# skyepurchase/MeatModeler

Measured on AMD Instinct MI355X. Metric: descriptor-match pairs/sec + BA residuals/sec, 500×1080p frames, 1/2/4/8 GPU, higher is better.
Workload: dtype u8/int32 (match), f64 (BA); 1 GPU; 500 frames 1920x1080, 4000 ORB kpts/frame, BF Hamming 2-NN + ratio, track linking, 2-view DLT, full BA (TRF, Schur, f64 MFMA Cholesky); frames=500, height=1080, width=1920, nfeatures=4000, parallelism=pairs/points x1

## Files before the change

include/meatmodeler.h:

```cpp
#ifndef MEATMODELER_H
#define MEATMODELER_H

#include <stddef.h>
#include <stdint.h>

#ifdef __cplusplus
extern "C" {
#endif

#define MM_OK 0
#define MM_ERR_ARG (-1)
#define MM_ERR_HIP (-2)
#define MM_ERR_WORKSPACE (-3)
#define MM_ERR_NUMERIC (-4)

typedef struct mm_ctx mm_ctx;

int mm_abi_version(void);
int mm_ctx_create(int device, void *hip_stream, mm_ctx **out);
void mm_ctx_destroy(mm_ctx *ctx);
const char *mm_last_error(mm_ctx *ctx);
int mm_ctx_sync(mm_ctx *ctx);
#define MM_CTL_CHOL_FORCE_ABANDON 1
#define MM_CTL_CHOL_LAST_PATH 2
#define MM_CTL_CHOL_RESERVED 3
#define MM_CTL_CU_COUNT 4
#define MM_CTL_CHOL_AVOID_FUSED 5
#define MM_CTL_LINK_LAST_VARIANT 6
#define MM_CTL_BATCH_LAST 7
long long mm_ctx_control(mm_ctx *ctx, int what, long long value);
int mm_timer_create(mm_ctx *ctx, void **timer_out);
int mm_timer_start(mm_ctx *ctx, void *timer);
int mm_timer_stop(mm_ctx *ctx, void *timer);
int mm_timer_elapsed_ms(mm_ctx *ctx, void *timer, float *ms_out);
void mm_timer_destroy(mm_ctx *ctx, void *timer);
int mm_profile_enable(mm_ctx *ctx, int on);
int mm_profile_select(mm_ctx *ctx, const char *name);
int mm_profile_report(mm_ctx *ctx, char *buf, size_t buf_len);

size_t mm_bf_workspace_bytes(int n_pairs, int nq_cap, int nt_cap);
int mm_bf_knn2_batched(mm_ctx *ctx, const uint8_t *q , const int32_t *nq , int nq_cap,
                       size_t q_set_stride, const uint8_t *t , const int32_t *nt , int nt_cap,
                       size_t t_set_stride, int n_pairs, int32_t *idx , int32_t *dist ,
                       void *ws , size_t ws_bytes);
int mm_bf_knn2_hamming(mm_ctx *ctx, const uint8_t *q , int nq, const uint8_t *t , int nt,
                       int32_t *idx , int32_t *dist , void *ws, size_t ws_bytes);
int mm_ratio_filter_batched(mm_ctx *ctx, const int32_t *idx , const int32_t *dist ,
                            const int32_t *nq , int nq_cap, int n_pairs, double threshold,
                            int32_t *pairs , int32_t *m_out );

typedef struct mm_orb_params {
    int32_t nfeatures;
    int32_t nlevels;
    int32_t edge_threshold;
    int32_t fast_threshold;
    float scale_factor;
    int32_t reserved;
} mm_orb_params;
size_t mm_orb_workspace_bytes(int batch, int height, int width, const mm_orb_params *prm);
int mm_orb_detect_compute(mm_ctx *ctx, const uint8_t *imgs , int batch, int height, int width, int stride,
                          const mm_orb_params *prm, const int8_t *pattern , void *ws , size_t ws_bytes,
                          float *kp_xy, int32_t *kp_meta, float *kp_resp, int32_t *kp_mom, uint8_t *desc,
                          int32_t *n_out);
int mm_orb_level_sizes(int height, int width, const mm_orb_params *prm, int32_t *lvl_w ,
                       int32_t *lvl_h , int32_t *lvl_n ,
                       float *lvl_scale );

int64_t mm_link_tracks_clip(int n_frames, int cap, const int32_t *kp_count, const float *kp_xy, int mcap,
                            const int32_t *match_count, const int32_t *matches, int64_t max_tracks,
                            int64_t max_obs, int64_t *track_ptr , int32_t *obs_frame,
                            int32_t *obs_kp, int64_t *n_obs_out);
size_t mm_link_workspace_bytes(int n_frames, int cap);
int mm_link_tracks_device(mm_ctx *ctx, int n_frames, int cap, const int32_t *kp_count, const float *kp_xy,
                          const int32_t *match_count, const int32_t *matches, void *ws, size_t ws_bytes,
                          int32_t *track_ptr, int32_t *obs_frame, int32_t *obs_kp, int64_t *counts );
int mm_flatten_offsets(mm_ctx *ctx, const int32_t *track_ptr, const int32_t *sel, int64_t n_sel, int64_t *out_ptr);
int mm_flatten_tracks(mm_ctx *ctx, const int32_t *track_ptr, const int32_t *obs_frame, const int32_t *obs_kp, const float *kp_xy,
                      int cap, const int32_t *sel , int t_lo, int64_t n_sel, const int64_t *out_ptr , int64_t n_obs,
                      int frame_offset, double *coords, int32_t *frame_indices, int32_t *point_indices);
int64_t mm_ba_build_pairs(int F, int P, int64_t O, const int32_t *fi, const int32_t *pi, const int32_t *pt_ptr,
                          const int32_t *pt_obs, const int32_t *cam_ptr, const int32_t *cam_obs, int span,
                          int64_t *seg_ptr, int32_t *pair_o, int32_t *pair_o2, int64_t max_pairs);
int mm_ba_build_index(int F, int P, int64_t O, const int32_t *fi, const int32_t *pi, int32_t *pt_ptr ,
                      int32_t *pt_obs , int32_t *cam_ptr , int32_t *cam_obs );

#define MM_VERIFY_TOO_FEW 1
#define MM_VERIFY_NO_MODEL 2
#define MM_VERIFY_WEAK 4
#define MM_VERIFY_MALFORMED 8
typedef struct mm_verify_params {
    int32_t n_hyp, min_matches, min_inliers, refit_iters;
    uint32_t seed, pair_base;
    int32_t on_fail, reserved;
    double threshold_px;
} mm_verify_params;
size_t mm_verify_workspace_bytes(int n_pairs, int n_hyp);
int mm_verify_matches(mm_ctx *ctx, const float *kp_xy , const int32_t *pairs ,
                      const int32_t *m , int n_pairs, int cap, const mm_verify_params *prm,
                      int32_t *pairs_out , int32_t *m_out , double *Fm ,
                      double *cost , int32_t *info , void *ws, size_t ws_bytes);

int mm_triangulate_dlt(mm_ctx *ctx, const double *proj , const int32_t *f0 , const int32_t *f1 ,
                       const double *x0 , const double *x1 , int64_t n,
                       double *X );
#define MM_TRI_BEHIND 1
#define MM_TRI_REPROJ 2
#define MM_TRI_PARALLAX 4
#define MM_TRI_DEGENERATE 8
typedef struct mm_tri_params {
    int32_t refine_iters, reserved;
    double max_reproj_px, max_cos_parallax, min_depth;
} mm_tri_params;
size_t mm_triangulate_tracks_workspace_bytes(int F);
int mm_triangulate_tracks(mm_ctx *ctx, const double *proj , int F, const int32_t *track_ptr , int64_t T,
                          const int32_t *obs_frame , const double *obs_xy , const mm_tri_params *prm,
                          double *X , double *quality , int32_t *flags , void *ws, size_t ws_bytes);

typedef struct mm_ba_problem {
    int32_t F, P;
    int64_t O;
    const double *K;
    const int32_t *fi, *pi;
    const double *obs;
    const int32_t *pt_ptr, *pt_obs;
    const int32_t *cam_ptr, *cam_obs;
    int32_t cam_span;
    int32_t reserved;
    int64_t n_seg;
    const int32_t *seg_ids;
    const int32_t *seg_chunk_ptr;
    int64_t n_chunks;
    const int32_t *chunk_seg;
    const int32_t *chunk_begin, *chunk_end;
    const int32_t *pair_o, *pair_o2;
    const int32_t *pair_p;
} mm_ba_problem;

int mm_ba_residual(mm_ctx *ctx, const mm_ba_problem *pb, const double *cams ,
                   const double *pts , double *res , double *cost2 ,
                   void *ws, size_t ws_bytes);
int mm_ba_jacobian(mm_ctx *ctx, const mm_ba_problem *pb, const double *cams, const double *pts, double *Jc,
                   double *Jp);
int mm_ba_normal_eq(mm_ctx *ctx, const mm_ba_problem *pb, const double *cams, const double *pts, double *B,
                    double *gc, double *C, double *gp);
int mm_ba_jvp(mm_ctx *ctx, const mm_ba_problem *pb, const double *cams, const double *pts, const double *wc,
              const double *wp, double *out);
size_t mm_ba_jvp_dots_workspace_bytes(const mm_ba_problem *pb);
int mm_ba_jvp_dots(mm_ctx *ctx, const mm_ba_problem *pb, const double *cams, const double *pts, const double *wc,
                   const double *wp, double *out, const double *other , double *rows ,
                   void *ws, size_t ws_bytes);
int mm_ba_schur(mm_ctx *ctx, const mm_ba_problem *pb, const double *cams, const double *pts, const double *Bd,
                const double *Cd, const double *gc, const double *gp, double *S, double *v, double *Cinv, void *ws,
                size_t ws_bytes);
size_t mm_ba_schur_workspace_bytes(const mm_ba_problem *pb);
int mm_ba_pairs_count(mm_ctx *ctx, const mm_ba_problem *pb, int32_t *cnt , int32_t *span_out );
int mm_ba_pairs_emit(mm_ctx *ctx, const mm_ba_problem *pb, const int64_t *offsets , int span,
                     int32_t *key , int32_t *pair_o , int32_t *pair_o2 );
size_t mm_multi_dot_workspace_bytes(void);
int mm_multi_dot(mm_ctx *ctx, int k, const double *const *a, const double *const *b, int64_t n, int64_t split,
                 double *out, void *ws, size_t ws_bytes);
int mm_trf_fused(mm_ctx *ctx, int op, const double *const *in, double *const *outv, const double *const *scalars,
                 double h0, double h1, int64_t n, int64_t split, double *out, void *ws, size_t ws_bytes);
int mm_trf_damping(mm_ctx *ctx, const double *gh2, const double *d11, double Delta, double min_damping, double *out);
size_t mm_ba_backsub_workspace_bytes(const mm_ba_problem *pb);
int mm_ba_backsub(mm_ctx *ctx, const mm_ba_problem *pb, const double *cams, const double *pts, const double *Cinv,
                  const double *gp, const double *dc , double *dp, void *ws , size_t ws_bytes);
int mm_ba_schur_solve(mm_ctx *ctx, const mm_ba_problem *pb, const double *cams, const double *pts, const double *Bd,
                      const double *Cd, const double *gc, const double *gp, double *S, double *v, double *Cinv,
                      int half_bandwidth, int32_t *info, void *ws_schur, size_t ws_schur_bytes, void *ws_chol,
                      size_t ws_chol_bytes, int n_slabs, int cams_per_slab, const int64_t *slab_seg_ptr,
                      const int64_t *slab_chunk_ptr);
int mm_ba_scale_update(mm_ctx *ctx, int F, int P, const double *B, const double *C, double *scale_inv , int first);
int mm_ba_damp(mm_ctx *ctx, int F, int P, const double *B, const double *C, const double *scale_inv, const double *reg ,
               double *Bd, double *Cd);
int mm_trf_step2d(mm_ctx *ctx, const double *r0, const double *d11, const double *r1, const double *r2, const double *r3,
                  const double *bs, const double *reg, const int32_t *info, double Delta, double *board );
typedef struct mm_trf_params {
    double ftol, xtol, gtol;
    double min_damping;
    int64_t max_nfev;
} mm_trf_params;
typedef struct mm_trf_row {
    int32_t iteration, nfev;
    double cost, reduction, step_norm, optimality;
} mm_trf_row;
typedef struct mm_trf_report {
    double cost0, cost, optimality, min_damping ;
    int32_t nfev, njev, status, iterations, log_rows;
    int32_t chol_fallbacks;
    int32_t collectives;
    int32_t reserved;
} mm_trf_report;
size_t mm_ba_trf_workspace_bytes(const mm_ba_problem *pb);
int mm_ba_trf(mm_ctx *ctx, const mm_ba_problem *pb, double *cams , double *pts ,
              const mm_trf_params *prm, mm_trf_report *report , mm_trf_row *log , int log_cap,
              void *ws , size_t ws_bytes);
typedef int (*mm_allreduce_fn)(void *user, double *buf , int64_t count);
typedef struct mm_dist {
    int32_t rank, world;
    int32_t half_bandwidth, band_exchange;
    mm_allreduce_fn allreduce;
    void *user;
} mm_dist;
size_t mm_ba_trf_dist_workspace_bytes(const mm_ba_problem *pb, int half_bandwidth);
int mm_ba_trf_dist(mm_ctx *ctx, const mm_ba_problem *pb, double *cams, double *pts, const mm_trf_params *prm,
                   mm_trf_report *report, mm_trf_row *log, int log_cap, void *ws, size_t ws_bytes, const mm_dist *dist);
size_t mm_ba_trf_batched_workspace_bytes(const mm_ba_problem *pb);
int mm_ba_trf_batched(mm_ctx *ctx, int n_prob, const mm_ba_problem *const *pbs, double *const *cams ,
                      double *const *pts , const mm_trf_params *prm, mm_trf_report *reports ,
                      void *const *ws , const size_t *ws_bytes, int32_t *solved_alone );
typedef struct mm_ba_fixed {
    int32_t F_fixed;
    int32_t reserved;
    const double *cams;
} mm_ba_fixed;
int mm_ba_residual_fixed(mm_ctx *ctx, const mm_ba_problem *pb, const mm_ba_fixed *fx, const double *cams ,
                         const double *pts , double *res , double *cost2 , void *ws,
                         size_t ws_bytes);
int mm_ba_normal_eq_fixed(mm_ctx *ctx, const mm_ba_problem *pb, const mm_ba_fixed *fx, const double *cams, const double *pts,
                          double *B, double *gc, double *C, double *gp);
size_t mm_ba_trf_fixed_workspace_bytes(const mm_ba_problem *pb, const mm_ba_fixed *fx);
int mm_ba_trf_fixed(mm_ctx *ctx, const mm_ba_problem *pb, const mm_ba_fixed *fx, double *cams ,
                    double *pts , const mm_trf_params *prm, mm_trf_report *report ,
                    mm_trf_row *log , int log_cap, void *ws , size_t ws_bytes);
size_t mm_chol_workspace_bytes(int n);
int mm_chol_solve_sym(mm_ctx *ctx, double *A , int n, double *b , int half_bandwidth, int both_triangles,
                      int32_t *info , void *ws, size_t ws_bytes);
int mm_chol_solve(mm_ctx *ctx, double *A , int n, double *b , int nrhs, int half_bandwidth,
                  int32_t *info , void *ws, size_t ws_bytes);

int mm_pyr_down(mm_ctx *ctx, const uint8_t *src , int w, int h, int src_pitch, uint8_t *dst , int dst_pitch);
int mm_lk_track(mm_ctx *ctx, const uint8_t *const *prev_levels, const uint8_t *const *next_levels, const int *w, const int *h,
                const int *pitch, int levels, const float *pts, int n, int win_w, int win_h, int max_count,
                double epsilon_sq, float *next_pts, uint8_t *status, float *err);
int mm_min_eig(mm_ctx *ctx, const uint8_t *img , int w, int h, int pitch, int block_size, double *eig );
int mm_corner_candidates(mm_ctx *ctx, const double *eig, int w, int h, double quality, unsigned long long *max_bits ,
                         long long *val_bits , int32_t *pos , int cap, int32_t *count );
int mm_gftt_select(const int32_t *pos , int64_t n, int w, int h, int max_corners, double min_distance,
                   float *out , int cap);
size_t mm_contrast_workspace_bytes(int batch, int w, int h, int tiles_x, int tiles_y);
int mm_increase_contrast(mm_ctx *ctx, const uint8_t *bgr, int batch, int w, int h, const uint16_t *gamma,
                         const uint16_t *cbrt_tab, const uint8_t *gamma_inv, double clip_limit, int tiles_x, int tiles_y,
                         uint8_t *out, uint8_t *grey , void *ws, size_t ws_bytes);
int mm_bgr_to_grey(mm_ctx *ctx, const uint8_t *bgr , size_t n_pixels, uint8_t *grey );
int mm_write_ply(const char *path, const double *xyz , int64_t n);

#ifdef __cplusplus
}
#endif
#endif
```

meatmodeler_amd/_lib.py:

```python
import ctypes as C
import os

_HERE = os.path.dirname(os.path.abspath(__file__))
LIB_PATH = os.path.join(_HERE, "libmeatmodeler_hip.so")

c_i32p = C.POINTER(C.c_int32)
c_i64p = C.POINTER(C.c_int64)
c_f32p = C.POINTER(C.c_float)
c_f64p = C.POINTER(C.c_double)
c_u8p = C.POINTER(C.c_uint8)
c_i8p = C.POINTER(C.c_int8)
vp = C.c_void_p


class MMError(RuntimeError):
    pass


class OrbParams(C.Structure):
    _fields_ = [("nfeatures", C.c_int32), ("nlevels", C.c_int32), ("edge_threshold", C.c_int32),
                ("fast_threshold", C.c_int32), ("scale_factor", C.c_float), ("reserved", C.c_int32)]


class BAProblem(C.Structure):
    _fields_ = [("F", C.c_int32), ("P", C.c_int32), ("O", C.c_int64), ("K", vp), ("fi", vp), ("pi", vp),
                ("obs", vp), ("pt_ptr", vp), ("pt_obs", vp), ("cam_ptr", vp), ("cam_obs", vp),
                ("cam_span", C.c_int32), ("reserved", C.c_int32), ("n_seg", C.c_int64), ("seg_ids", vp),
                ("seg_chunk_ptr", vp), ("n_chunks", C.c_int64), ("chunk_seg", vp), ("chunk_begin", vp),
                ("chunk_end", vp), ("pair_o", vp), ("pair_o2", vp), ("pair_p", vp)]


class BAFixed(C.Structure):
    _fields_ = [("F_fixed", C.c_int32), ("reserved", C.c_int32), ("cams", vp)]


class TrfParams(C.Structure):
    _fields_ = [("ftol", C.c_double), ("xtol", C.c_double), ("gtol", C.c_double), ("min_damping", C.c_double),
                ("max_nfev", C.c_int64)]


class TrfRow(C.Structure):
    _fields_ = [("iteration", C.c_int32), ("nfev", C.c_int32), ("cost", C.c_double), ("reduction", C.c_double),
                ("step_norm", C.c_double), ("optimality", C.c_double)]


class TriParams(C.Structure):
    _fields_ = [("refine_iters", C.c_int32), ("reserved", C.c_int32), ("max_reproj_px", C.c_double),
                ("max_cos_parallax", C.c_double), ("min_depth", C.c_double)]


class VerifyParams(C.Structure):
    _fields_ = [("n_hyp", C.c_int32), ("min_matches", C.c_int32), ("min_inliers", C.c_int32), ("refit_iters", C.c_int32),
                ("seed", C.c_uint32), ("pair_base", C.c_uint32), ("on_fail", C.c_int32), ("reserved", C.c_int32),
                ("threshold_px", C.c_double)]


ALLREDUCE_FN = C.CFUNCTYPE(C.c_int, vp, vp, C.c_int64)


class Dist(C.Structure):
    _fields_ = [("rank", C.c_int32), ("world", C.c_int32), ("half_bandwidth", C.c_int32), ("band_exchange", C.c_int32),
                ("allreduce", ALLREDUCE_FN), ("user", vp)]


class TrfReport(C.Structure):
    _fields_ = [("cost0", C.c_double), ("cost", C.c_double), ("optimality", C.c_double), ("min_damping", C.c_double),
                ("nfev", C.c_int32), ("njev", C.c_int32), ("status", C.c_int32), ("iterations", C.c_int32),
                ("log_rows", C.c_int32), ("chol_fallbacks", C.c_int32), ("collectives", C.c_int32), ("reserved", C.c_int32)]


SIGNATURES = {
    "mm_abi_version": (C.c_int, []),
    "mm_ctx_create": (C.c_int, [C.c_int, vp, C.POINTER(vp)]),
    "mm_ctx_destroy": (None, [vp]),
    "mm_ctx_control": (C.c_longlong, [vp, C.c_int, C.c_longlong]),
    "mm_last_error": (C.c_char_p, [vp]),
    "mm_ctx_sync": (C.c_int, [vp]),
    "mm_timer_create": (C.c_int, [vp, C.POINTER(vp)]),
    "mm_timer_start": (C.c_int, [vp, vp]),
    "mm_timer_stop": (C.c_int, [vp, vp]),
    "mm_timer_elapsed_ms": (C.c_int, [vp, vp, C.POINTER(C.c_float)]),
    "mm_timer_destroy": (None, [vp, vp]),
    "mm_profile_enable": (C.c_int, [vp, C.c_int]),
    "mm_profile_report": (C.c_int, [vp, C.c_char_p, C.c_size_t]),
    "mm_profile_select": (C.c_int, [vp, C.c_char_p]),
    "mm_bf_workspace_bytes": (C.c_size_t, [C.c_int, C.c_int, C.c_int]),
    "mm_bf_knn2_batched": (C.c_int, [vp, vp, vp, C.c_int, C.c_size_t, vp, vp, C.c_int, C.c_size_t, C.c_int, vp, vp,
                                     vp, C.c_size_t]),
    "mm_bf_knn2_hamming": (C.c_int, [vp, vp, C.c_int, vp, C.c_int, vp, vp, vp, C.c_size_t]),
    "mm_ratio_filter_batched": (C.c_int, [vp, vp, vp, vp, C.c_int, C.c_int, C.c_double, vp, vp]),
    "mm_orb_workspace_bytes": (C.c_size_t, [C.c_int, C.c_int, C.c_int, C.POINTER(OrbParams)]),
    "mm_orb_detect_compute": (C.c_int, [vp, vp, C.c_int, C.c_int, C.c_int, C.c_int, C.POINTER(OrbParams), vp, vp,
                                        C.c_size_t, vp, vp, vp, vp, vp, vp]),
    "mm_orb_level_sizes": (C.c_int, [C.c_int, C.c_int, C.POINTER(OrbParams), c_i32p, c_i32p, c_i32p, c_f32p]),
    "mm_link_tracks_clip": (C.c_int64, [C.c_int, C.c_int, c_i32p, c_f32p, C.c_int, c_i32p, c_i32p, C.c_int64,
                                        C.c_int64, c_i64p, c_i32p, c_i32p, c_i64p]),
    "mm_link_workspace_bytes": (C.c_size_t, [C.c_int, C.c_int]),
    "mm_link_tracks_device": (C.c_int, [vp, C.c_int, C.c_int, vp, vp, vp, vp, vp, C.c_size_t, vp, vp, vp, vp]),
    "mm_flatten_offsets": (C.c_int, [vp, vp, vp, C.c_int64, vp]),
    "mm_flatten_tracks": (C.c_int, [vp, vp, vp, vp, vp, C.c_int, vp, C.c_int, C.c_int64, vp, C.c_int64, C.c_int, vp, vp, vp]),
    "mm_ba_build_pairs": (C.c_int64, [C.c_int, C.c_int, C.c_int64, c_i32p, c_i32p, c_i32p, c_i32p, c_i32p, c_i32p, C.c_int,
                                      c_i64p, c_i32p, c_i32p, C.c_int64]),
    "mm_ba_build_index": (C.c_int, [C.c_int, C.c_int, C.c_int64, c_i32p, c_i32p, c_i32p, c_i32p, c_i32p, c_i32p]),
    "mm_verify_workspace_bytes": (C.c_size_t, [C.c_int, C.c_int]),
    "mm_verify_matches": (C.c_int, [vp, vp, vp, vp, C.c_int, C.c_int, C.POINTER(VerifyParams), vp, vp, vp, vp, vp, vp, C.c_size_t]),
    "mm_triangulate_dlt": (C.c_int, [vp, vp, vp, vp, vp, vp, C.c_int64, vp]),
    "mm_triangulate_tracks_workspace_bytes": (C.c_size_t, [C.c_int]),
    "mm_triangulate_tracks": (C.c_int, [vp, vp, C.c_int, vp, C.c_int64, vp, vp, C.POINTER(TriParams), vp, vp, vp, vp, C.c_size_t]),
    "mm_ba_residual": (C.c_int, [vp, C.POINTER(BAProblem), vp, vp, vp, vp, vp, C.c_size_t]),
    "mm_ba_jacobian": (C.c_int, [vp, C.POINTER(BAProblem), vp, vp, vp, vp]),
    "mm_ba_normal_eq": (C.c_int, [vp, C.POINTER(BAProblem), vp, vp, vp, vp, vp, vp]),
    "mm_ba_jvp": (C.c_int, [vp, C.POINTER(BAProblem), vp, vp, vp, vp, vp]),
    "mm_ba_schur": (C.c_int, [vp, C.POINTER(BAProblem), vp, vp, vp, vp, vp, vp, vp, vp, vp, vp, C.c_size_t]),
    "mm_ba_schur_workspace_bytes": (C.c_size_t, [C.POINTER(BAProblem)]),
    "mm_ba_pairs_count": (C.c_int, [vp, C.POINTER(BAProblem), vp, vp]),
    "mm_ba_pairs_emit": (C.c_int, [vp, C.POINTER(BAProblem), vp, C.c_int, vp, vp, vp]),
    "mm_ba_schur_solve": (C.c_int, [vp, C.POINTER(BAProblem), vp, vp, vp, vp, vp, vp, vp, vp, vp, C.c_int, vp, vp,
                                    C.c_size_t, vp, C.c_size_t, C.c_int, C.c_int, c_i64p, c_i64p]),
    "mm_multi_dot_workspace_bytes": (C.c_size_t, []),
    "mm_multi_dot": (C.c_int, [vp, C.c_int, C.POINTER(vp), C.POINTER(vp), C.c_int64, C.c_int64, vp, vp, C.c_size_t]),
    "mm_trf_fused": (C.c_int, [vp, C.c_int, C.POINTER(vp), C.POINTER(vp), C.POINTER(vp), C.c_double, C.c_double, C.c_int64,
                               C.c_int64, vp, vp, C.c_size_t]),
    "mm_trf_damping": (C.c_int, [vp, vp, vp, C.c_double, C.c_double, vp]),
    "mm_ba_backsub": (C.c_int, [vp, C.POINTER(BAProblem), vp, vp, vp, vp, vp, vp, vp, C.c_size_t]),
    "mm_ba_backsub_workspace_bytes": (C.c_size_t, [C.POINTER(BAProblem)]),
    "mm_chol_workspace_bytes": (C.c_size_t, [C.c_int]),
    "mm_chol_solve": (C.c_int, [vp, vp, C.c_int, vp, C.c_int, C.c_int, vp, vp, C.c_size_t]),
    "mm_ba_jvp_dots_workspace_bytes": (C.c_size_t, [C.POINTER(BAProblem)]),
    "mm_ba_jvp_dots": (C.c_int, [vp, C.POINTER(BAProblem), vp, vp, vp, vp, vp, vp, vp, vp, C.c_size_t]),
    "mm_ba_scale_update": (C.c_int, [vp, C.c_int, C.c_int, vp, vp, vp, C.c_int]),
    "mm_ba_damp": (C.c_int, [vp, C.c_int, C.c_int, vp, vp, vp, vp, vp, vp]),
    "mm_trf_step2d": (C.c_int, [vp, vp, vp, vp, vp, vp, vp, vp, vp, C.c_double, vp]),
    "mm_pyr_down": (C.c_int, [vp, vp, C.c_int, C.c_int, C.c_int, vp, C.c_int]),
    "mm_lk_track": (C.c_int, [vp, vp, vp, vp, vp, vp, C.c_int, vp, C.c_int, C.c_int, C.c_int, C.c_int, C.c_double, vp, vp, vp]),
    "mm_min_eig": (C.c_int, [vp, vp, C.c_int, C.c_int, C.c_int, C.c_int, vp]),
    "mm_corner_candidates": (C.c_int, [vp, vp, C.c_int, C.c_int, C.c_double, vp, vp, vp, C.c_int, vp]),
    "mm_gftt_select": (C.c_int, [vp, C.c_int64, C.c_int, C.c_int, C.c_int, C.c_double, vp, C.c_int]),
    "mm_contrast_workspace_bytes": (C.c_size_t, [C.c_int, C.c_int, C.c_int, C.c_int, C.c_int]),
    "mm_increase_contrast": (C.c_int, [vp, vp, C.c_int, C.c_int, C.c_int, vp, vp, vp, C.c_double, C.c_int, C.c_int, vp, vp, vp,
                                       C.c_size_t]),
    "mm_bgr_to_grey": (C.c_int, [vp, vp, C.c_size_t, vp]),
    "mm_write_ply": (C.c_int, [C.c_char_p, vp, C.c_int64]),
    "mm_chol_solve_sym": (C.c_int, [vp, vp, C.c_int, vp, C.c_int, C.c_int, vp, vp, C.c_size_t]),
    "mm_ba_trf_workspace_bytes": (C.c_size_t, [C.POINTER(BAProblem)]),
    "mm_ba_trf": (C.c_int, [vp, C.POINTER(BAProblem), vp, vp, C.POINTER(TrfParams), C.POINTER(TrfReport),
                            C.POINTER(TrfRow), C.c_int, vp, C.c_size_t]),
    "mm_ba_trf_batched_workspace_bytes": (C.c_size_t, [C.POINTER(BAProblem)]),
    "mm_ba_trf_batched": (C.c_int, [vp, C.c_int, C.POINTER(C.POINTER(BAProblem)), C.POINTER(vp), C.POINTER(vp),
                                    C.POINTER(TrfParams), C.POINTER(TrfReport), C.POINTER(vp), C.POINTER(C.c_size_t), c_i32p]),
    "mm_ba_residual_fixed": (C.c_int, [vp, C.POINTER(BAProblem), C.POINTER(BAFixed), vp, vp, vp, vp, vp, C.c_size_t]),
    "mm_ba_normal_eq_fixed": (C.c_int, [vp, C.POINTER(BAProblem), C.POINTER(BAFixed), vp, vp, vp, vp, vp, vp]),
    "mm_ba_trf_fixed_workspace_bytes": (C.c_size_t, [C.POINTER(BAProblem), C.POINTER(BAFixed)]),
    "mm_ba_trf_fixed": (C.c_int, [vp, C.POINTER(BAProblem), C.POINTER(BAFixed), vp, vp, C.POINTER(TrfParams),
                                  C.POINTER(TrfReport), C.POINTER(TrfRow), C.c_int, vp, C.c_size_t]),
    "mm_ba_trf_dist_workspace_bytes": (C.c_size_t, [C.POINTER(BAProblem), C.c_int]),
    "mm_ba_trf_dist": (C.c_int, [vp, C.POINTER(BAProblem), vp, vp, C.POINTER(TrfParams), C.POINTER(TrfReport),
                                 C.POINTER(TrfRow), C.c_int, vp, C.c_size_t, C.POINTER(Dist)]),
}


def _load():
    if not os.path.exists(LIB_PATH):
        raise ImportError(
            f"{LIB_PATH} is missing: the HIP extension has not been built "
            "(make -C meatmodeler_amd/csrc).  meatmodeler_amd has no CPU fallback.")
    lib = C.CDLL(LIB_PATH)
    for name, (res, args) in SIGNATURES.items():
        fn = getattr(lib, name)
        fn.restype = res
        fn.argtypes = args
    return lib


lib = _load()


def ptr(t):
    if t is None:
        return None
    if hasattr(t, "data_ptr"):
        return t.data_ptr()
    return t.ctypes.data


class Context:

    def __init__(self, device=None, stream=None):
        import torch
        if not torch.cuda.is_available():
            raise MMError("meatmodeler_amd needs an AMD GPU (torch.cuda.is_available() is False); "
                          "there is no CPU path")
        if device is None:
            device = torch.cuda.current_device()
        self.device = torch.device("cuda", device if isinstance(device, int) else device.index or 0)
        self.stream = stream if stream is not None else torch.cuda.current_stream(self.device)
        h = vp()
        rc = lib.mm_ctx_create(self.device.index, vp(self.stream.cuda_stream), C.byref(h))
        if rc != 0:
            raise MMError(f"mm_ctx_create failed ({rc})")
        self.h = h

    def check(self, rc, what=""):
        if rc != 0:
            msg = lib.mm_last_error(self.h)
            raise MMError(f"{what} failed ({rc}): {msg.decode() if msg else ''}")

    def sync(self):
        self.check(lib.mm_ctx_sync(self.h), "mm_ctx_sync")

    CTL_CHOL_FORCE_ABANDON, CTL_CHOL_LAST_PATH, CTL_CHOL_RESERVED, CTL_CU_COUNT, CTL_CHOL_AVOID_FUSED = 1, 2, 3, 4, 5
    CTL_LINK_LAST_VARIANT = 6
    CTL_BATCH_LAST = 7

    def control(self, what, value=0):
        r = int(lib.mm_ctx_control(self.h, int(what), int(value)))
        if r < -1 or (r == -1 and what not in (self.CTL_CHOL_LAST_PATH, self.CTL_LINK_LAST_VARIANT, self.CTL_BATCH_LAST)):
            self.check(r, "mm_ctx_control")
        return r

    def profile(self, level, only=None):
        if only is not None:
            self.check(lib.mm_profile_select(self.h, only.encode()), "mm_profile_select")
        self.check(lib.mm_profile_enable(self.h, int(level)), "mm_profile_enable")

    def profile_report(self):
        buf = C.create_string_buffer(1 << 16)
        n = lib.mm_profile_report(self.h, buf, len(buf))
        if n < 0:
            self.check(n, "mm_profile_report")
        out = {}
        for line in buf.value.decode().splitlines():
            name, cnt, ms = line.split()
            out[name] = (int(cnt), float(ms))
        return out

    def __del__(self):
        try:
            if getattr(self, "h", None):
                lib.mm_ctx_destroy(self.h)
                self.h = None
        except Exception:
            pass


class Timer:

    def __init__(self, ctx):
        self.ctx = ctx
        self.t = vp()
        ctx.check(lib.mm_timer_create(ctx.h, C.byref(self.t)), "mm_timer_create")

    def start(self):
        self.ctx.check(lib.mm_timer_start(self.ctx.h, self.t), "mm_timer_start")

    def stop(self):
        self.ctx.check(lib.mm_timer_stop(self.ctx.h, self.t), "mm_timer_stop")

    def elapsed_ms(self):
        ms = C.c_float()
        self.ctx.check(lib.mm_timer_elapsed_ms(self.ctx.h, self.t, C.byref(ms)), "mm_timer_elapsed_ms")
        return ms.value

    def __del__(self):
        try:
            lib.mm_timer_destroy(self.ctx.h, self.t)
        except Exception:
            pass


_default_ctx = {}


def default_context():
    import torch
    key = (torch.cuda.current_device(), torch.cuda.current_stream().cuda_stream)
    c = _default_ctx.get(key)
    if c is None:
        c = _default_ctx[key] = Context()
    return c
```

meatmodeler_amd/csrc/bf_match.hip:

```cpp
#include "mm_common.h"
#include <cstdlib>
#include <type_traits>

namespace {

constexpr int BF_THREADS = 256;
constexpr uint32_t BF_NONE = 0xFFFFFFFFu;
constexpr int BF_IDX_BITS = 20;

__device__ __forceinline__ uint32_t bcnt_acc(uint32_t x, uint32_t acc) {
    uint32_t r;
    asm("v_bcnt_u32_b32 %0, %1, %2" : "=v"(r) : "v"(x), "v"(acc));
    return r;
}

__device__ __forceinline__ uint32_t ham256(const uint32_t (&a)[8], const uint4 &t0, const uint4 &t1) {
    uint32_t d = bcnt_acc(a[0] ^ t0.x, 0u);
    d = bcnt_acc(a[1] ^ t0.y, d);
    d = bcnt_acc(a[2] ^ t0.z, d);
    d = bcnt_acc(a[3] ^ t0.w, d);
    d = bcnt_acc(a[4] ^ t1.x, d);
    d = bcnt_acc(a[5] ^ t1.y, d);
    d = bcnt_acc(a[6] ^ t1.z, d);
    d = bcnt_acc(a[7] ^ t1.w, d);
    return d;
}

__device__ __forceinline__ void top2_insert(uint32_t key, uint32_t &b0, uint32_t &b1) {
    uint32_t hi = max(b0, key);
    b0 = min(b0, key);
    b1 = min(b1, hi);
}

template <int BF_QPL, int BF_UNROLL>
__global__ __launch_bounds__(BF_THREADS) void bf_knn2_kernel(
    const uint8_t *__restrict__ q, const int32_t *__restrict__ nq_dev, int nq_cap, size_t q_stride,
    const uint8_t *__restrict__ t, const int32_t *__restrict__ nt_dev, int nt_cap, size_t t_stride, int n_splits,
    uint32_t *__restrict__ part, int32_t *__restrict__ idx, int32_t *__restrict__ dist) {
    const int pair = blockIdx.z;
    const int split = blockIdx.y;
    int nq = nq_dev ? min(nq_dev[pair], nq_cap) : nq_cap;
    int nt = nt_dev ? min(nt_dev[pair], nt_cap) : nt_cap;
    constexpr int BF_QTILE = BF_THREADS * BF_QPL;
    const int qbase = blockIdx.x * BF_QTILE;
    if (qbase >= nq) return;

    uint32_t qa[BF_QPL][8];
    const uint8_t *qp = q + (size_t)pair * q_stride;
#pragma unroll
    for (int u = 0; u < BF_QPL; ++u) {
        int qi = qbase + u * BF_THREADS + threadIdx.x;
        uint4 lo = make_uint4(0, 0, 0, 0), hi = lo;
        if (qi < nq) {
            const uint4 *p = reinterpret_cast<const uint4 *>(qp + (size_t)qi * 32);
            lo = p[0];
            hi = p[1];
        }
        qa[u][0] = lo.x; qa[u][1] = lo.y; qa[u][2] = lo.z; qa[u][3] = lo.w;
        qa[u][4] = hi.x; qa[u][5] = hi.y; qa[u][6] = hi.z; qa[u][7] = hi.w;
    }

    int chunk = (nt + n_splits - 1) / n_splits;
    chunk = (chunk + BF_UNROLL - 1) / BF_UNROLL * BF_UNROLL;
    const int j0 = split * chunk;
    const int j1 = min(nt, j0 + chunk);

    uint32_t b0[BF_QPL], b1[BF_QPL];
#pragma unroll
    for (int u = 0; u < BF_QPL; ++u) b0[u] = b1[u] = BF_NONE;

    const uint4 *__restrict__ tp = reinterpret_cast<const uint4 *>(t + (size_t)pair * t_stride);
    int j = j0;
    for (; j + BF_UNROLL <= j1; j += BF_UNROLL) {
        uint4 tv[2 * BF_UNROLL];
#pragma unroll
        for (int k = 0; k < 2 * BF_UNROLL; ++k) tv[k] = tp[2 * j + k];
#pragma unroll
        for (int k = 0; k < BF_UNROLL; ++k) {
#pragma unroll
            for (int u = 0; u < BF_QPL; ++u) {
                uint32_t d = ham256(qa[u], tv[2 * k], tv[2 * k + 1]);
                top2_insert((d << BF_IDX_BITS) | (uint32_t)(j + k), b0[u], b1[u]);
            }
        }
    }
    for (; j < j1; ++j) {
        uint4 t0 = tp[2 * j], t1 = tp[2 * j + 1];
#pragma unroll
        for (int u = 0; u < BF_QPL; ++u) {
            uint32_t d = ham256(qa[u], t0, t1);
            top2_insert((d << BF_IDX_BITS) | (uint32_t)j, b0[u], b1[u]);
        }
    }

#pragma unroll
    for (int u = 0; u < BF_QPL; ++u) {
        int qi = qbase + u * BF_THREADS + threadIdx.x;
        if (qi >= nq) continue;
        if (n_splits == 1) {
            size_t o = ((size_t)pair * nq_cap + qi) * 2;
            idx[o] = b0[u] == BF_NONE ? -1 : (int32_t)(b0[u] & ((1u << BF_IDX_BITS) - 1));
            idx[o + 1] = b1[u] == BF_NONE ? -1 : (int32_t)(b1[u] & ((1u << BF_IDX_BITS) - 1));
            dist[o] = b0[u] == BF_NONE ? -1 : (int32_t)(b0[u] >> BF_IDX_BITS);
            dist[o + 1] = b1[u] == BF_NONE ? -1 : (int32_t)(b1[u] >> BF_IDX_BITS);
        } else {
            size_t o = (((size_t)pair * n_splits + split) * nq_cap + qi) * 2;
            part[o] = b0[u];
            part[o + 1] = b1[u];
        }
    }
}

constexpr int BF_TCHUNK = 128;

__device__ __forceinline__ void top2_insert_med3(uint32_t key, uint32_t &b0, uint32_t &b1) {
    uint32_t m;
    asm("v_med3_u32 %0, %1, %2, %3" : "=v"(m) : "v"(b0), "v"(b1), "v"(key));
    b0 = min(b0, key);
    b1 = m;
}

template <int BF_QPL, int TCH = BF_TCHUNK>
__global__ __launch_bounds__(BF_THREADS) void bf_knn2_lds_kernel(
    const uint8_t *__restrict__ q, const int32_t *__restrict__ nq_dev, int nq_cap, size_t q_stride,
    const uint8_t *__restrict__ t, const int32_t *__restrict__ nt_dev, int nt_cap, size_t t_stride, int n_splits,
    uint32_t *__restrict__ part, int32_t *__restrict__ idx, int32_t *__restrict__ dist) {
    constexpr int NST = TCH / 128;
    __shared__ uint4 tl[2][TCH * 2];
    const int pair = blockIdx.z;
    const int split = blockIdx.y;
    int nq = nq_dev ? min(nq_dev[pair], nq_cap) : nq_cap;
    int nt = nt_dev ? min(nt_dev[pair], nt_cap) : nt_cap;
    constexpr int BF_QTILE = BF_THREADS * BF_QPL;
    const int qbase = blockIdx.x * BF_QTILE;
    if (qbase >= nq) return;

    uint32_t qa[BF_QPL][8];
    const uint8_t *qp = q + (size_t)pair * q_stride;
#pragma unroll
    for (int u = 0; u < BF_QPL; ++u) {
        int qi = qbase + u * BF_THREADS + threadIdx.x;
        uint4 lo = make_uint4(0, 0, 0, 0), hi = lo;
        if (qi < nq) {
            const uint4 *p = reinterpret_cast<const uint4 *>(qp + (size_t)qi * 32);
            lo = p[0];
            hi = p[1];
        }
        qa[u][0] = lo.x; qa[u][1] = lo.y; qa[u][2] = lo.z; qa[u][3] = lo.w;
        qa[u][4] = hi.x; qa[u][5] = hi.y; qa[u][6] = hi.z; qa[u][7] = hi.w;
    }
    int chunk = (nt + n_splits - 1) / n_splits;
    chunk = (chunk + 3) & ~3;
    const int j0 = split * chunk;
    const int j1 = min(nt, j0 + chunk);
    uint32_t b0[BF_QPL], b1[BF_QPL];
#pragma unroll
    for (int u = 0; u < BF_QPL; ++u) b0[u] = b1[u] = BF_NONE;

    const uint4 *__restrict__ tp = reinterpret_cast<const uint4 *>(t + (size_t)pair * t_stride);
    uint4 stage[NST];
#pragma unroll
    for (int z = 0; z < NST; ++z) {
        const int e = 2 * j0 + z * BF_THREADS + (int)threadIdx.x;
        stage[z] = e < 2 * j1 ? tp[e] : make_uint4(0, 0, 0, 0);
        tl[0][z * BF_THREADS + threadIdx.x] = stage[z];
    }
    __syncthreads();
    int buf = 0;
    for (int c0 = j0; c0 < j1; c0 += TCH) {
        const int cn = min(TCH, j1 - c0);
        const int nxt = c0 + TCH;
        if (nxt < j1) {
#pragma unroll
            for (int z = 0; z < NST; ++z) {
                const int e = 2 * nxt + z * BF_THREADS + (int)threadIdx.x;
                stage[z] = e < 2 * j1 ? tp[e] : make_uint4(0, 0, 0, 0);
            }
        }
        const uint4 *tb = tl[buf];
        int k = 0;
        for (; k + 4 <= cn; k += 4) {
            uint4 tv[8];
#pragma unroll
            for (int r = 0; r < 8; ++r) tv[r] = tb[2 * k + r];
            uint32_t d[4][BF_QPL];
            bool hit = false;
#pragma unroll
            for (int u = 0; u < BF_QPL; ++u) {
#pragma unroll
                for (int r = 0; r < 4; ++r) d[r][u] = ham256(qa[u], tv[2 * r], tv[2 * r + 1]);
                const uint32_t m = min(min(d[0][u], d[1][u]), min(d[2][u], d[3][u]));
                hit |= m < (b1[u] >> BF_IDX_BITS);
            }
            if (__builtin_amdgcn_ballot_w64(hit) != 0) {
#pragma unroll
                for (int r = 0; r < 4; ++r) {
#pragma unroll
                    for (int u = 0; u < BF_QPL; ++u)
                        top2_insert_med3((d[r][u] << BF_IDX_BITS) | (uint32_t)(c0 + k + r), b0[u], b1[u]);
                }
            }
        }
        for (; k < cn; ++k) {
            const uint4 t0 = tb[2 * k], t1 = tb[2 * k + 1];
#pragma unroll
            for (int u = 0; u < BF_QPL; ++u) {
                uint32_t d = ham256(qa[u], t0, t1);
                top2_insert_med3((d << BF_IDX_BITS) | (uint32_t)(c0 + k), b0[u], b1[u]);
            }
        }
        if (nxt < j1) {
#pragma unroll
            for (int z = 0; z < NST; ++z) tl[buf ^ 1][z * BF_THREADS + threadIdx.x] = stage[z];
            __syncthreads();
            buf ^= 1;
        }
    }
#pragma unroll
    for (int u = 0; u < BF_QPL; ++u) {
        int qi = qbase + u * BF_THREADS + threadIdx.x;
        if (qi >= nq) continue;
        if (n_splits == 1) {
            size_t o = ((size_t)pair * nq_cap + qi) * 2;
            idx[o] = b0[u] == BF_NONE ? -1 : (int32_t)(b0[u] & ((1u << BF_IDX_BITS) - 1));
            idx[o + 1] = b1[u] == BF_NONE ? -1 : (int32_t)(b1[u] & ((1u << BF_IDX_BITS) - 1));
            dist[o] = b0[u] == BF_NONE ? -1 : (int32_t)(b0[u] >> BF_IDX_BITS);
            dist[o + 1] = b1[u] == BF_NONE ? -1 : (int32_t)(b1[u] >> BF_IDX_BITS);
        } else {
            size_t o = (((size_t)pair * n_splits + split) * nq_cap + qi) * 2;
            part[o] = b0[u];
            part[o + 1] = b1[u];
        }
    }
}

__global__ __launch_bounds__(256) void bf_merge_kernel(const uint32_t *__restrict__ part,
                                                       const int32_t *__restrict__ nq_dev, int nq_cap, int n_splits,
                                                       int32_t *__restrict__ idx, int32_t *__restrict__ dist) {
    const int pair = blockIdx.y;
    const int qi = blockIdx.x * blockDim.x + threadIdx.x;
    int nq = nq_dev ? min(nq_dev[pair], nq_cap) : nq_cap;
    if (qi >= nq) return;
    uint32_t b0 = BF_NONE, b1 = BF_NONE;
    for (int s = 0; s < n_splits; ++s) {
        size_t o = (((size_t)pair * n_splits + s) * nq_cap + qi) * 2;
        top2_insert(part[o], b0, b1);
        top2_insert(part[o + 1], b0, b1);
    }
    size_t o = ((size_t)pair * nq_cap + qi) * 2;
    idx[o] = b0 == BF_NONE ? -1 : (int32_t)(b0 & ((1u << BF_IDX_BITS) - 1));
    idx[o + 1] = b1 == BF_NONE ? -1 : (int32_t)(b1 & ((1u << BF_IDX_BITS) - 1));
    dist[o] = b0 == BF_NONE ? -1 : (int32_t)(b0 >> BF_IDX_BITS);
    dist[o + 1] = b1 == BF_NONE ? -1 : (int32_t)(b1 >> BF_IDX_BITS);
}

__global__ __launch_bounds__(256) void ratio_filter_kernel(const int32_t *__restrict__ idx,
                                                           const int32_t *__restrict__ dist,
                                                           const int32_t *__restrict__ nq_dev, int nq_cap,
                                                           double threshold, int32_t *__restrict__ pairs,
                                                           int32_t *__restrict__ m_out) {
    __shared__ int wave_cnt[4];
    __shared__ int base_s;
    const int pair = blockIdx.x;
    int nq = nq_dev ? min(nq_dev[pair], nq_cap) : nq_cap;
    const int lane = threadIdx.x & 63, wave = threadIdx.x >> 6;
    if (threadIdx.x == 0) base_s = 0;
    __syncthreads();
    for (int q0 = 0; q0 < nq; q0 += 256) {
        int qi = q0 + threadIdx.x;
        bool keep = false;
        int ti = -1;
        if (qi < nq) {
            size_t o = ((size_t)pair * nq_cap + qi) * 2;
            int d0 = dist[o], d1 = dist[o + 1];
            ti = idx[o];
            keep = (d0 >= 0) && (d1 >= 0) && ((double)d0 < threshold * (double)d1);
        }
        unsigned long long m = __ballot(keep);
        int before = __builtin_popcountll(m & ((1ull << lane) - 1ull));
        if (lane == 0) wave_cnt[wave] = __builtin_popcountll(m);
        __syncthreads();
        int off = base_s;
        for (int w = 0; w < wave; ++w) off += wave_cnt[w];
        if (keep) {
            size_t o = ((size_t)pair * nq_cap + (off + before)) * 2;
            pairs[o] = qi;
            pairs[o + 1] = ti;
        }
        __syncthreads();
        if (threadIdx.x == 0) base_s += wave_cnt[0] + wave_cnt[1] + wave_cnt[2] + wave_cnt[3];
        __syncthreads();
    }
    if (threadIdx.x == 0) m_out[pair] = base_s;
}

typedef int bf_v4i __attribute__((ext_vector_type(4)));
typedef int bf_v16i __attribute__((ext_vector_type(16)));
constexpr int MF_TT = 32;
constexpr int MF_PITCH = 272;
constexpr int MF_SEG = 128;

__device__ __forceinline__ uint32_t bf_expand4(uint32_t nib) {
    const uint32_t x = (nib * 0x00204081u) & 0x01010101u;
    return ((x ^ 0x01010101u) * 0xFFu) | x;
}
__device__ __forceinline__ bf_v4i bf_expand16(uint32_t bits) {
    bf_v4i r;
    r[0] = (int)bf_expand4(bits & 15u);
    r[1] = (int)bf_expand4((bits >> 4) & 15u);
    r[2] = (int)bf_expand4((bits >> 8) & 15u);
    r[3] = (int)bf_expand4((bits >> 12) & 15u);
    return r;
}

__global__ __launch_bounds__(256) void bf_expand_kernel(const uint8_t *__restrict__ t, int nt_cap, size_t t_stride, int ntp,
                                                        int n_pairs, uint8_t *__restrict__ out) {
    const size_t g = (size_t)blockIdx.x * 256 + threadIdx.x;
    const size_t total = (size_t)n_pairs * ntp * 16;
    if (g >= total) return;
    const int chunk = (int)(g & 15);
    const size_t rowg = g >> 4;
    const int row = (int)(rowg % ntp), pair = (int)(rowg / ntp);
    uint32_t bits = 0;
    if (row < nt_cap) bits = reinterpret_cast<const uint16_t *>(t + (size_t)pair * t_stride + (size_t)row * 32)[chunk];
    reinterpret_cast<bf_v4i *>(out)[g] = bf_expand16(bits);
}

__device__ __forceinline__ uint32_t bf_pk_lo16(uint32_t hi_src, uint32_t lo_src) {
    return __builtin_amdgcn_perm(hi_src, lo_src, 0x05040100u);
}
typedef unsigned short bf_u16x2 __attribute__((ext_vector_type(2)));
__device__ __forceinline__ uint32_t bf_pk_mad(uint32_t a, uint32_t b, uint32_t c) {
    const bf_u16x2 r = __builtin_bit_cast(bf_u16x2, a) * __builtin_bit_cast(bf_u16x2, b) + __builtin_bit_cast(bf_u16x2, c);
    return __builtin_bit_cast(uint32_t, r);
}
__device__ __forceinline__ void bf_pk_top2(uint32_t key, uint32_t &b0, uint32_t &b1) {
    const bf_u16x2 k = __builtin_bit_cast(bf_u16x2, key), x0 = __builtin_bit_cast(bf_u16x2, b0), x1 = __builtin_bit_cast(bf_u16x2, b1);
    const bf_u16x2 hi = __builtin_elementwise_max(x0, k);
    b0 = __builtin_bit_cast(uint32_t, __builtin_elementwise_min(x0, k));
    b1 = __builtin_bit_cast(uint32_t, __builtin_elementwise_min(x1, hi));
}

__global__ __launch_bounds__(BF_THREADS) void bf_knn2_mfma_kernel(
    const uint8_t *__restrict__ q, const int32_t *__restrict__ nq_dev, int nq_cap, size_t q_stride,
    const uint8_t *__restrict__ tx, const int32_t *__restrict__ nt_dev, int nt_cap, int ntp,
    int32_t *__restrict__ idx, int32_t *__restrict__ dist) {
    __shared__ __attribute__((aligned(16))) uint8_t tile[2][MF_TT][MF_PITCH];
    const int pair = blockIdx.z;
    const int nq = nq_dev ? min(nq_dev[pair], nq_cap) : nq_cap;
    const int nt = nt_dev ? min(nt_dev[pair], nt_cap) : nt_cap;
    const int qbase = blockIdx.x * BF_THREADS;
    if (qbase >= nq) return;
    const int lane = threadIdx.x & 63, wv = threadIdx.x >> 6;
    const int c = lane & 31, h = lane >> 5;
    bf_v4i B[2][8];
    const uint8_t *qp = q + (size_t)pair * q_stride;
#pragma unroll
    for (int u = 0; u < 2; ++u) {
        const int qi = qbase + 64 * wv + 32 * u + c;
        uint4 lo = make_uint4(0, 0, 0, 0), hi = lo;
        if (qi < nq) {
            const uint4 *p = reinterpret_cast<const uint4 *>(qp + (size_t)qi * 32);
            lo = p[0];
            hi = p[1];
        }
        const uint32_t w[8] = {lo.x, lo.y, lo.z, lo.w, hi.x, hi.y, hi.z, hi.w};
#pragma unroll
        for (int j = 0; j < 8; ++j) B[u][j] = bf_expand16((w[j] >> (16 * h)) & 0xFFFFu);
    }
    uint32_t s0[2][8], s1[2][8];
#pragma unroll
    for (int u = 0; u < 2; ++u)
#pragma unroll
        for (int p = 0; p < 8; ++p) s0[u][p] = s1[u][p] = 0xFFFFFFFFu;
    uint32_t g0[2] = {BF_NONE, BF_NONE}, g1[2] = {BF_NONE, BF_NONE};
    const int ntiles = (nt + MF_TT - 1) / MF_TT;
    const uint8_t *txp = tx + (size_t)pair * ntp * 256;
    const int e0 = threadIdx.x, e1 = threadIdx.x + 256;
    bf_v4i a0, a1, b0_, b1_, c0_, c1_;
    auto fetch = [&](int tt, auto set) __attribute__((always_inline)) {
        constexpr int S = decltype(set)::value;
        if (tt < ntiles) {
            const bf_v4i *src = reinterpret_cast<const bf_v4i *>(txp + (size_t)tt * MF_TT * 256);
            const bf_v4i v0 = src[e0], v1 = src[e1];
            if constexpr (S == 0) { a0 = v0; a1 = v1; }
            if constexpr (S == 1) { b0_ = v0; b1_ = v1; }
            if constexpr (S == 2) { c0_ = v0; c1_ = v1; }
        }
    };
    auto commit = [&](int buf, auto set) __attribute__((always_inline)) {
        constexpr int S = decltype(set)::value;
        bf_v4i *d0 = reinterpret_cast<bf_v4i *>(&tile[buf][e0 >> 4][(e0 & 15) * 16]);
        bf_v4i *d1 = reinterpret_cast<bf_v4i *>(&tile[buf][e1 >> 4][(e1 & 15) * 16]);
        if constexpr (S == 0) { *d0 = a0; *d1 = a1; }
        if constexpr (S == 1) { *d0 = b0_; *d1 = b1_; }
        if constexpr (S == 2) { *d0 = c0_; *d1 = c1_; }
    };
    auto fold = [&](int seg) __attribute__((always_inline)) {
#pragma unroll
        for (int u = 0; u < 2; ++u)
#pragma unroll
            for (int p = 0; p < 8; ++p) {
                const int m = 8 * (p >> 1) + 4 * h + 2 * (p & 1);
#pragma unroll
                for (int x = 0; x < 2; ++x) {
#pragma unroll
                    for (int k = 0; k < 2; ++k) {
                        const uint32_t key16 = ((k == 0 ? s0[u][p] : s1[u][p]) >> (16 * x)) & 0xFFFFu;
                        if (key16 != 0xFFFFu) {
                            const uint32_t d = key16 >> 7, tno = key16 & 127u;
                            top2_insert((d << 16) | (uint32_t)((seg * MF_SEG + (int)tno) * MF_TT + m + x), g0[u], g1[u]);
                        }
                    }
                }
                s0[u][p] = s1[u][p] = 0xFFFFFFFFu;
            }
    };
    auto tile_step = [&](int tt, auto partial_tag) __attribute__((always_inline)) {
        constexpr bool PARTIAL = decltype(partial_tag)::value;
        const int buf = tt & 1;
        bf_v16i acc0 = {0, 0, 0, 0, 0, 0, 0, 0, 0, 0, 0, 0, 0, 0, 0, 0}, acc1 = acc0;
        bf_v4i A[8];
#pragma unroll
        for (int j = 0; j < 8; ++j) A[j] = *reinterpret_cast<const bf_v4i *>(&tile[buf][c][32 * j + 16 * h]);
        const uint32_t tno = (uint32_t)(tt & (MF_SEG - 1));
        const uint32_t base = (16384u + tno) * 0x00010001u;
        auto keys = [&](const bf_v16i &acc, int u, int p) __attribute__((always_inline)) {
            uint32_t k = bf_pk_mad(bf_pk_lo16((uint32_t)acc[2 * p + 1], (uint32_t)acc[2 * p]), 0xFFC0FFC0u, base);
            if constexpr (PARTIAL) {
                const int m = tt * MF_TT + 8 * (p >> 1) + 4 * h + 2 * (p & 1);
                k |= (m >= nt ? 0x0000FFFFu : 0u) | (m + 1 >= nt ? 0xFFFF0000u : 0u);
            }
            bf_pk_top2(k, s0[u][p], s1[u][p]);
        };
#pragma unroll
        for (int j = 0; j < 8; ++j) acc0 = __builtin_amdgcn_mfma_i32_32x32x32_i8(A[j], B[0][j], acc0, 0, 0, 0);
        __builtin_amdgcn_sched_barrier(0);
#pragma unroll
        for (int j = 0; j < 8; ++j) {
            acc1 = __builtin_amdgcn_mfma_i32_32x32x32_i8(A[j], B[1][j], acc1, 0, 0, 0);
            keys(acc0, 0, j);
            __builtin_amdgcn_sched_barrier(0);
        }
#pragma unroll
        for (int p = 0; p < 8; ++p) keys(acc1, 1, p);
    };
    using I0 = std::integral_constant<int, 0>;
    using I1 = std::integral_constant<int, 1>;
    using I2 = std::integral_constant<int, 2>;
    fetch(0, I0{});
    fetch(1, I1{});
    fetch(2, I2{});
    if (ntiles > 0) commit(0, I0{});
    fetch(3, I0{});
    __syncthreads();
    const int nfull = nt / MF_TT;
    auto iteration = [&](int tt, auto next_set) __attribute__((always_inline)) {
        tile_step(tt, std::false_type{});
        if ((tt & (MF_SEG - 1)) == MF_SEG - 1) fold(tt / MF_SEG);
        if (tt + 1 < ntiles) commit((tt & 1) ^ 1, next_set);
        fetch(tt + 4, next_set);
        __syncthreads();
    };
    int tt = 0;
    for (; tt + 3 <= nfull; tt += 3) {
        iteration(tt, I1{});
        iteration(tt + 1, I2{});
        iteration(tt + 2, I0{});
    }
    if (tt < nfull) {
        iteration(tt, I1{});
        if (tt + 1 < nfull) iteration(tt + 1, I2{});
    }
    if (nfull < ntiles) tile_step(nfull, std::true_type{});
    if (ntiles > 0) fold((ntiles - 1) / MF_SEG);
#pragma unroll
    for (int u = 0; u < 2; ++u) {
        const uint32_t o0 = __shfl_xor(g0[u], 32, 64), o1 = __shfl_xor(g1[u], 32, 64);
        top2_insert(o0, g0[u], g1[u]);
        top2_insert(o1, g0[u], g1[u]);
        const int qi = qbase + 64 * wv + 32 * u + c;
        if (h == 0 && qi < nq) {
            const size_t o = ((size_t)pair * nq_cap + qi) * 2;
            idx[o] = g0[u] == BF_NONE ? -1 : (int32_t)(g0[u] & 0xFFFFu);
            idx[o + 1] = g1[u] == BF_NONE ? -1 : (int32_t)(g1[u] & 0xFFFFu);
            dist[o] = g0[u] == BF_NONE ? -1 : (int32_t)(g0[u] >> 16);
            dist[o + 1] = g1[u] == BF_NONE ? -1 : (int32_t)(g1[u] >> 16);
        }
    }
}

typedef int bf_v8i __attribute__((ext_vector_type(8)));
typedef float bf_v16f __attribute__((ext_vector_type(16)));
constexpr int F4_PITCH = 144;

__device__ __forceinline__ uint32_t bf_fp4x8(uint32_t byte) {
    uint32_t x = byte;
    x = (x | (x << 12)) & 0x000F000Fu;
    x = (x | (x << 6)) & 0x03030303u;
    x = (x | (x << 3)) & 0x11111111u;
    return 0xAAAAAAAAu ^ (x << 3);
}
__device__ __forceinline__ bf_v4i bf_fp4x32(uint32_t bits) {
    bf_v4i r;
    r[0] = (int)bf_fp4x8(bits & 255u);
    r[1] = (int)bf_fp4x8((bits >> 8) & 255u);
    r[2] = (int)bf_fp4x8((bits >> 16) & 255u);
    r[3] = (int)bf_fp4x8(bits >> 24);
    return r;
}

__global__ __launch_bounds__(256) void bf_expand_fp4_kernel(const uint8_t *__restrict__ t, int nt_cap, size_t t_stride, int ntp,
                                                            int n_pairs, uint8_t *__restrict__ out) {
    const size_t g = (size_t)blockIdx.x * 256 + threadIdx.x;
    const size_t total = (size_t)n_pairs * ntp * 8;
    if (g >= total) return;
    const int chunk = (int)(g & 7);
    const size_t rowg = g >> 3;
    const int row = (int)(rowg % ntp), pair = (int)(rowg / ntp);
    uint32_t bits = 0;
    if (row < nt_cap) bits = reinterpret_cast<const uint32_t *>(t + (size_t)pair * t_stride + (size_t)row * 32)[chunk];
    reinterpret_cast<bf_v4i *>(out)[g] = bf_fp4x32(bits);
}

__global__ __launch_bounds__(BF_THREADS, 3) void bf_knn2_fp4_kernel(
    const uint8_t *__restrict__ q, const int32_t *__restrict__ nq_dev, int nq_cap, size_t q_stride,
    const uint8_t *__restrict__ tx, const int32_t *__restrict__ nt_dev, int nt_cap, int ntp,
    int32_t *__restrict__ idx, int32_t *__restrict__ dist) {
    __shared__ __attribute__((aligned(16))) uint8_t tile[2][MF_TT][F4_PITCH];
    const int pair = blockIdx.z;
    const int nq = nq_dev ? min(nq_dev[pair], nq_cap) : nq_cap;
    const int nt = nt_dev ? min(nt_dev[pair], nt_cap) : nt_cap;
    const int qbase = blockIdx.x * BF_THREADS;
    if (qbase >= nq) return;
    const int lane = threadIdx.x & 63, wv = threadIdx.x >> 6;
    const int c = lane & 31, h = lane >> 5;
    bf_v8i B[2][4];
    const uint8_t *qp = q + (size_t)pair * q_stride;
#pragma unroll
    for (int u = 0; u < 2; ++u) {
        const int qi = qbase + 64 * wv + 32 * u + c;
        uint4 lo = make_uint4(0, 0, 0, 0), hi = lo;
        if (qi < nq) {
            const uint4 *p = reinterpret_cast<const uint4 *>(qp + (size_t)qi * 32);
            lo = p[0];
            hi = p[1];
        }
        const uint32_t w[8] = {lo.x, lo.y, lo.z, lo.w, hi.x, hi.y, hi.z, hi.w};
#pragma unroll
        for (int j = 0; j < 4; ++j) {
            const bf_v4i e = bf_fp4x32(~(h ? w[2 * j + 1] : w[2 * j]));
            B[u][j] = bf_v8i{e[0], e[1], e[2], e[3], 0, 0, 0, 0};
        }
    }
    uint32_t s0[2][8], s1[2][8];
#pragma unroll
    for (int u = 0; u < 2; ++u)
#pragma unroll
        for (int p = 0; p < 8; ++p) s0[u][p] = s1[u][p] = 0xFFFFFFFFu;
    uint32_t g0[2] = {BF_NONE, BF_NONE}, g1[2] = {BF_NONE, BF_NONE};
    const int ntiles = (nt + MF_TT - 1) / MF_TT;
    const uint8_t *txp = tx + (size_t)pair * ntp * 128;
    const int e0 = threadIdx.x;
    bf_v4i ra, rb, rc;
    auto fetch = [&](int tt, auto set) __attribute__((always_inline)) {
        constexpr int S = decltype(set)::value;
        if (tt < ntiles) {
            const bf_v4i v = reinterpret_cast<const bf_v4i *>(txp + (size_t)tt * MF_TT * 128)[e0];
            if constexpr (S == 0) ra = v;
            if constexpr (S == 1) rb = v;
            if constexpr (S == 2) rc = v;
        }
    };
    auto commit = [&](int buf, auto set) __attribute__((always_inline)) {
        constexpr int S = decltype(set)::value;
        bf_v4i *d = reinterpret_cast<bf_v4i *>(&tile[buf][e0 >> 3][(e0 & 7) * 16]);
        if constexpr (S == 0) *d = ra;
        if constexpr (S == 1) *d = rb;
        if constexpr (S == 2) *d = rc;
    };
    auto fold = [&](int seg) __attribute__((always_inline)) {
#pragma unroll
        for (int u = 0; u < 2; ++u)
#pragma unroll
            for (int p = 0; p < 8; ++p) {
                const int m = 8 * (p >> 1) + 4 * h + 2 * (p & 1);
#pragma unroll
                for (int x = 0; x < 2; ++x) {
#pragma unroll
                    for (int k = 0; k < 2; ++k) {
                        const uint32_t key16 = ((k == 0 ? s0[u][p] : s1[u][p]) >> (16 * x)) & 0xFFFFu;
                        if (key16 != 0xFFFFu) {
                            const uint32_t d = key16 >> 7, tno = key16 & 127u;
                            top2_insert((d << 16) | (uint32_t)((seg * MF_SEG + (int)tno) * MF_TT + m + x), g0[u], g1[u]);
                        }
                    }
                }
                s0[u][p] = s1[u][p] = 0xFFFFFFFFu;
            }
    };
    auto keys = [&](const bf_v16f &acc, int u, int p, int dead_from) __attribute__((always_inline)) {
        const float f_hi = acc[2 * p + 1], f_lo = acc[2 * p];
        uint32_t k = bf_pk_lo16(__float_as_uint(f_hi), __float_as_uint(f_lo));
        if (dead_from >= 0) {
            const int m = 8 * (p >> 1) + 4 * h + 2 * (p & 1);
            k |= (m >= dead_from ? 0x0000FFFFu : 0u) | (m + 1 >= dead_from ? 0xFFFF0000u : 0u);
        }
        bf_pk_top2(k, s0[u][p], s1[u][p]);
    };
    bf_v16f acc1_prev;
    bool pending = false;
    auto tile_step = [&](int tt, auto first_tag) __attribute__((always_inline)) {
        constexpr bool HAVE_PREV = !decltype(first_tag)::value;
        const int buf = tt & 1;
        const uint32_t tno = (uint32_t)(tt & (MF_SEG - 1));
        const float init = 12582912.0f + 16384.0f + (float)tno;
        bf_v16f acc0 = {init, init, init, init, init, init, init, init, init, init, init, init, init, init, init, init};
        bf_v16f acc1 = acc0;
        bf_v8i A[4];
#pragma unroll
        for (int j = 0; j < 4; ++j) {
            const bf_v4i a = *reinterpret_cast<const bf_v4i *>(&tile[buf][c][32 * j + 16 * h]);
            A[j] = bf_v8i{a[0], a[1], a[2], a[3], 0, 0, 0, 0};
        }
#pragma unroll
        for (int j = 0; j < 4; ++j) {
            acc0 = __builtin_amdgcn_mfma_scale_f32_32x32x64_f8f6f4(A[j], B[0][j], acc0, 4, 4, 0, 133, 0, 127);
            if constexpr (HAVE_PREV) {
                keys(acc1_prev, 1, 2 * j, -1);
                keys(acc1_prev, 1, 2 * j + 1, -1);
            }
            __builtin_amdgcn_sched_barrier(0);
        }
        if (HAVE_PREV && ((tt - 1) & (MF_SEG - 1)) == MF_SEG - 1) fold((tt - 1) / MF_SEG);
#pragma unroll
        for (int j = 0; j < 4; ++j) {
            acc1 = __builtin_amdgcn_mfma_scale_f32_32x32x64_f8f6f4(A[j], B[1][j], acc1, 4, 4, 0, 133, 0, 127);
            keys(acc0, 0, 2 * j, -1);
            keys(acc0, 0, 2 * j + 1, -1);
            __builtin_amdgcn_sched_barrier(0);
        }
        acc1_prev = acc1;
    };
    using I0 = std::integral_constant<int, 0>;
    using I1 = std::integral_constant<int, 1>;
    using I2 = std::integral_constant<int, 2>;
    fetch(0, I0{});
    fetch(1, I1{});
    fetch(2, I2{});
    if (ntiles > 0) commit(0, I0{});
    fetch(3, I0{});
    __syncthreads();
    const int nfull = nt / MF_TT;
    auto iteration = [&](int tt, auto next_set, auto first_tag) __attribute__((always_inline)) {
        tile_step(tt, first_tag);
        if (tt + 1 < ntiles) commit((tt & 1) ^ 1, next_set);
        fetch(tt + 4, next_set);
        __syncthreads();
    };
    int tt = 0;
    if (nfull > 0) {
        iteration(0, I1{}, std::true_type{});
        pending = true;
        tt = 1;
        if (tt < nfull) { iteration(tt, I2{}, std::false_type{}); ++tt; }
        if (tt < nfull) { iteration(tt, I0{}, std::false_type{}); ++tt; }
    }
    for (; tt + 3 <= nfull; tt += 3) {
        iteration(tt, I1{}, std::false_type{});
        iteration(tt + 1, I2{}, std::false_type{});
        iteration(tt + 2, I0{}, std::false_type{});
    }
    if (tt < nfull) {
        iteration(tt, I1{}, std::false_type{});
        if (tt + 1 < nfull) iteration(tt + 1, I2{}, std::false_type{});
    }
    if (pending) {
#pragma unroll
        for (int p = 0; p < 8; ++p) keys(acc1_prev, 1, p, -1);
        if (((nfull - 1) & (MF_SEG - 1)) == MF_SEG - 1) fold((nfull - 1) / MF_SEG);
    }
    if (nfull < ntiles) {
        const int buf = nfull & 1;
        const float init = 12582912.0f + 16384.0f + (float)(nfull & (MF_SEG - 1));
        bf_v16f acc0 = {init, init, init, init, init, init, init, init, init, init, init, init, init, init, init, init};
        bf_v16f acc1 = acc0;
#pragma unroll
        for (int j = 0; j < 4; ++j) {
            const bf_v4i a = *reinterpret_cast<const bf_v4i *>(&tile[buf][c][32 * j + 16 * h]);
            const bf_v8i A = bf_v8i{a[0], a[1], a[2], a[3], 0, 0, 0, 0};
            acc0 = __builtin_amdgcn_mfma_scale_f32_32x32x64_f8f6f4(A, B[0][j], acc0, 4, 4, 0, 133, 0, 127);
            acc1 = __builtin_amdgcn_mfma_scale_f32_32x32x64_f8f6f4(A, B[1][j], acc1, 4, 4, 0, 133, 0, 127);
        }
        const int dead_from = nt - nfull * MF_TT;
#pragma unroll
        for (int p = 0; p < 8; ++p) {
            keys(acc0, 0, p, dead_from);
            keys(acc1, 1, p, dead_from);
        }
    }
    if (ntiles > 0) fold((ntiles - 1) / MF_SEG);
#pragma unroll
    for (int u = 0; u < 2; ++u) {
        const uint32_t o0 = __shfl_xor(g0[u], 32, 64), o1 = __shfl_xor(g1[u], 32, 64);
        top2_insert(o0, g0[u], g1[u]);
        top2_insert(o1, g0[u], g1[u]);
        const int qi = qbase + 64 * wv + 32 * u + c;
        if (h == 0 && qi < nq) {
            const size_t o = ((size_t)pair * nq_cap + qi) * 2;
            idx[o] = g0[u] == BF_NONE ? -1 : (int32_t)(g0[u] & 0xFFFFu);
            idx[o + 1] = g1[u] == BF_NONE ? -1 : (int32_t)(g1[u] & 0xFFFFu);
            dist[o] = g0[u] == BF_NONE ? -1 : (int32_t)(g0[u] >> 16);
            dist[o + 1] = g1[u] == BF_NONE ? -1 : (int32_t)(g1[u] >> 16);
        }
    }
}


struct F4mState {
    uint32_t m[5], last, n0, n1, key;
};
template <bool PARTIAL>
__device__ __forceinline__ void f4m_chunk0(const bf_v16f &acc, F4mState &st, int h, int dead_from) {
    uint32_t v[16];
#pragma unroll
    for (int i = 0; i < 16; ++i) {
        const float f = acc[i];
        v[i] = __float_as_uint(f);
        if constexpr (PARTIAL) {
            const int m = 8 * (i >> 2) + 4 * h + (i & 3);
            if (m >= dead_from) v[i] = 0xFFFFFFFFu;
        }
    }
#pragma unroll
    for (int g = 0; g < 5; ++g) st.m[g] = min(min(v[3 * g], v[3 * g + 1]), v[3 * g + 2]);
    st.last = v[15];
}
__device__ __forceinline__ void f4m_chunk1(F4mState &st) {
    st.n0 = min(min(st.m[0], st.m[1]), st.m[2]);
    st.n1 = min(min(st.m[3], st.m[4]), st.last);
    st.n0 = min(st.n0, st.n1);
}
template <bool PARTIAL>
__device__ __forceinline__ void f4m_chunk2(F4mState &st, uint32_t tile32) {
    const uint32_t m = st.n0;
    uint32_t k = ((m & 0x003FFFE0u) << 11) + tile32;
    k = (m & 31u) | k;
    if constexpr (PARTIAL) k = m == 0xFFFFFFFFu ? BF_NONE : k;
    st.key = k;
}
__device__ __forceinline__ void f4m_update(uint32_t k, uint32_t &b0, uint32_t &b1) {
    asm("v_med3_u32 %0, %1, %2, %3" : "=v"(b1) : "v"(b0), "v"(b1), "v"(k));
    b0 = min(b0, k);
}

#ifdef MM_BF_CLOCK
__device__ long long g_bf_clock[2 * 4096];
#endif
template <int WAVES, bool PIPE>
__global__ __launch_bounds__(BF_THREADS, WAVES) void bf_knn2_fp4min_kernel(
    const uint8_t *__restrict__ q, const int32_t *__restrict__ nq_dev, int nq_cap, size_t q_stride,
    const uint8_t *__restrict__ tx, const uint8_t *__restrict__ tpk, size_t t_stride, const int32_t *__restrict__ nt_dev,
    int nt_cap, int ntp, int32_t *__restrict__ idx, int32_t *__restrict__ dist, int qtiles, int n_pairs) {
    __shared__ __attribute__((aligned(16))) uint8_t tile[3][MF_TT][F4_PITCH];
    const int xcd = blockIdx.x & 7, slot = blockIdx.x >> 3;
    const int grp = slot / qtiles;
    const int pair = grp * 8 + xcd;
    if (pair >= n_pairs) return;
    const int nq = nq_dev ? min(nq_dev[pair], nq_cap) : nq_cap;
    const int nt = nt_dev ? min(nt_dev[pair], nt_cap) : nt_cap;
    const int qbase = (slot - grp * qtiles) * BF_THREADS;
    if (qbase >= nq) return;
    const int lane = threadIdx.x & 63, wv = threadIdx.x >> 6;
    const int c = lane & 31, h = lane >> 5;
#ifdef MM_BF_CLOCK
    const long long clk_t0 = __builtin_readcyclecounter();
    const unsigned long long clk_r0 = __builtin_amdgcn_s_memrealtime();
#endif
    bf_v4i B4[2][4];
    const uint8_t *qp = q + (size_t)pair * q_stride;
#pragma unroll
    for (int u = 0; u < 2; ++u) {
        const int qi = qbase + 64 * wv + 32 * u + c;
        uint4 lo = make_uint4(0, 0, 0, 0), hi = lo;
        if (qi < nq) {
            const uint4 *p = reinterpret_cast<const uint4 *>(qp + (size_t)qi * 32);
            lo = p[0];
            hi = p[1];
        }
        const uint32_t w[8] = {lo.x, lo.y, lo.z, lo.w, hi.x, hi.y, hi.z, hi.w};
#pragma unroll
        for (int j = 0; j < 4; ++j) {
            const bf_v4i e = bf_fp4x32(~(h ? w[2 * j + 1] : w[2 * j]));
            B4[u][j] = e;
        }
    }
    bf_v16f cinit;
#pragma unroll
    for (int i = 0; i < 16; ++i) cinit[i] = 12582912.0f + 262144.0f + (float)(8 * (i >> 2) + 4 * h + (i & 3));
    uint32_t b0[2] = {BF_NONE, BF_NONE}, b1[2] = {BF_NONE, BF_NONE};
    const int ntiles = (nt + MF_TT - 1) / MF_TT;
    const uint8_t *txp = tx + (size_t)pair * ntp * 128;
    const int e0 = threadIdx.x;
    bf_v4i ra, rb, rc;
    auto fetch = [&](int tt, auto set) __attribute__((always_inline)) {
        constexpr int S = decltype(set)::value;
        if (tt < ntiles) {
            const bf_v4i v = reinterpret_cast<const bf_v4i *>(txp + (size_t)tt * MF_TT * 128)[e0];
            if constexpr (S == 0) ra = v;
            if constexpr (S == 1) rb = v;
            if constexpr (S == 2) rc = v;
        }
    };
    auto commit = [&](int buf, auto set) __attribute__((always_inline)) {
        constexpr int S = decltype(set)::value;
        bf_v4i *d = reinterpret_cast<bf_v4i *>(&tile[buf][e0 >> 3][(e0 & 7) * 16]);
        if constexpr (S == 0) *d = ra;
        if constexpr (S == 1) *d = rb;
        if constexpr (S == 2) *d = rc;
    };
    bf_v16f acc1_prev;
    bf_v4i A4[4];
    auto read_a = [&](int buf, int j) __attribute__((always_inline)) {
        A4[j] = *reinterpret_cast<const bf_v4i *>(&tile[buf][c][32 * j + 16 * h]);
    };
#define F4M_A(j) (bf_v8i{A4[j][0], A4[j][1], A4[j][2], A4[j][3], 0, 0, 0, 0})
#define F4M_B(u, j) (bf_v8i{B4[u][j][0], B4[u][j][1], B4[u][j][2], B4[u][j][3], 0, 0, 0, 0})
    const bool wave_active = __builtin_amdgcn_readfirstlane(qbase + 64 * wv) < nq;
    auto tile_step = [&](int tt, auto first_tag, int nxt, bool have_next) __attribute__((always_inline)) {
        constexpr bool HAVE_PREV = !decltype(first_tag)::value;
        if (!wave_active) return;
        if constexpr (!PIPE) {
#pragma unroll
            for (int j = 0; j < 4; ++j) read_a((nxt + 2) % 3, j);
        }
        F4mState st;
        bf_v16f acc0 = __builtin_amdgcn_mfma_scale_f32_32x32x64_f8f6f4(F4M_A(0), F4M_B(0, 0), cinit, 4, 4, 0, 137, 0, 127);
        if constexpr (HAVE_PREV) f4m_chunk0<false>(acc1_prev, st, h, 0);
        __builtin_amdgcn_sched_barrier(0);
        acc0 = __builtin_amdgcn_mfma_scale_f32_32x32x64_f8f6f4(F4M_A(1), F4M_B(0, 1), acc0, 4, 4, 0, 137, 0, 127);
        if constexpr (HAVE_PREV) f4m_chunk1(st);
        __builtin_amdgcn_sched_barrier(0);
        acc0 = __builtin_amdgcn_mfma_scale_f32_32x32x64_f8f6f4(F4M_A(2), F4M_B(0, 2), acc0, 4, 4, 0, 137, 0, 127);
        if constexpr (HAVE_PREV) f4m_chunk2<false>(st, (uint32_t)(tt - 1) * MF_TT);
        __builtin_amdgcn_sched_barrier(0);
        acc0 = __builtin_amdgcn_mfma_scale_f32_32x32x64_f8f6f4(F4M_A(3), F4M_B(0, 3), acc0, 4, 4, 0, 137, 0, 127);
        if constexpr (HAVE_PREV) f4m_update(st.key, b0[1], b1[1]);
        __builtin_amdgcn_sched_barrier(0);
        bf_v16f acc1 = __builtin_amdgcn_mfma_scale_f32_32x32x64_f8f6f4(F4M_A(0), F4M_B(1, 0), cinit, 4, 4, 0, 137, 0, 127);
        if (PIPE && have_next) read_a(nxt, 0);
        f4m_chunk0<false>(acc0, st, h, 0);
        __builtin_amdgcn_sched_barrier(0);
        acc1 = __builtin_amdgcn_mfma_scale_f32_32x32x64_f8f6f4(F4M_A(1), F4M_B(1, 1), acc1, 4, 4, 0, 137, 0, 127);
        if (PIPE && have_next) read_a(nxt, 1);
        f4m_chunk1(st);
        __builtin_amdgcn_sched_barrier(0);
        acc1 = __builtin_amdgcn_mfma_scale_f32_32x32x64_f8f6f4(F4M_A(2), F4M_B(1, 2), acc1, 4, 4, 0, 137, 0, 127);
        if (PIPE && have_next) read_a(nxt, 2);
        f4m_chunk2<false>(st, (uint32_t)tt * MF_TT);
        __builtin_amdgcn_sched_barrier(0);
        acc1 = __builtin_amdgcn_mfma_scale_f32_32x32x64_f8f6f4(F4M_A(3), F4M_B(1, 3), acc1, 4, 4, 0, 137, 0, 127);
        if (PIPE && have_next) read_a(nxt, 3);
        f4m_update(st.key, b0[0], b1[0]);
        __builtin_amdgcn_sched_barrier(0);
        acc1_prev = acc1;
    };
    using I0 = std::integral_constant<int, 0>;
    using I1 = std::integral_constant<int, 1>;
    using I2 = std::integral_constant<int, 2>;
    fetch(0, I0{});
    fetch(1, I1{});
    fetch(2, I2{});
    if (ntiles > 0) commit(0, I0{});
    fetch(3, I0{});
    if (ntiles > 1) commit(1, I1{});
    fetch(4, I1{});
    __syncthreads();
    if constexpr (PIPE) {
#pragma unroll
        for (int j = 0; j < 4; ++j) read_a(0, j);
    }
    const int nfull = nt / MF_TT;
    auto iteration = [&](int tt, auto cur_tag, auto first_tag) __attribute__((always_inline)) {
        constexpr int CUR = decltype(cur_tag)::value, NXT = (CUR + 1) % 3, C2 = (CUR + 2) % 3;
        tile_step(tt, first_tag, NXT, tt + 1 < ntiles);
        if (tt + 2 < ntiles) commit(C2, std::integral_constant<int, C2>{});
        fetch(tt + 5, std::integral_constant<int, C2>{});
        __syncthreads();
    };
    int tt = 0;
    if (nfull > 0) {
        iteration(0, I0{}, std::true_type{});
        tt = 1;
        if (tt < nfull) { iteration(tt, I1{}, std::false_type{}); ++tt; }
        if (tt < nfull) { iteration(tt, I2{}, std::false_type{}); ++tt; }
    }
    for (; tt + 3 <= nfull; tt += 3) {
        iteration(tt, I0{}, std::false_type{});
        iteration(tt + 1, I1{}, std::false_type{});
        iteration(tt + 2, I2{}, std::false_type{});
    }
    if (tt < nfull) {
        iteration(tt, I0{}, std::false_type{});
        if (tt + 1 < nfull) iteration(tt + 1, I1{}, std::false_type{});
    }
    auto book = [&](const bf_v16f &acc, uint32_t tile32, int u, auto partial_tag, int dead_from) __attribute__((always_inline)) {
        constexpr bool PARTIAL = decltype(partial_tag)::value;
        F4mState st;
        f4m_chunk0<PARTIAL>(acc, st, h, dead_from);
        f4m_chunk1(st);
        f4m_chunk2<PARTIAL>(st, tile32);
        f4m_update(st.key, b0[u], b1[u]);
    };
    if (!wave_active) return;
    if (nfull > 0) book(acc1_prev, (uint32_t)(nfull - 1) * MF_TT, 1, std::false_type{}, 0);
    if (nfull < ntiles) {
        bf_v16f acc0 = cinit, acc1 = cinit;
#pragma unroll
        for (int j = 0; j < 4; ++j) {
            if constexpr (!PIPE) read_a(nfull % 3, j);
            acc0 = __builtin_amdgcn_mfma_scale_f32_32x32x64_f8f6f4(F4M_A(j), F4M_B(0, j), acc0, 4, 4, 0, 137, 0, 127);
            acc1 = __builtin_amdgcn_mfma_scale_f32_32x32x64_f8f6f4(F4M_A(j), F4M_B(1, j), acc1, 4, 4, 0, 137, 0, 127);
        }
        const int dead_from = nt - nfull * MF_TT;
        book(acc0, (uint32_t)nfull * MF_TT, 0, std::true_type{}, dead_from);
        book(acc1, (uint32_t)nfull * MF_TT, 1, std::true_type{}, dead_from);
    }
    const uint8_t *tp = tpk + (size_t)pair * t_stride;
#pragma unroll
    for (int u = 0; u < 2; ++u) {
        const int qi = qbase + 64 * wv + 32 * u + c;
        {
            const uint4 *p = reinterpret_cast<const uint4 *>(qp + (size_t)min(qi, nq - 1) * 32);
            const uint4 lo = p[0], hi = p[1];
            const uint32_t a[8] = {lo.x, lo.y, lo.z, lo.w, hi.x, hi.y, hi.z, hi.w};
            const bool have = b0[u] != BF_NONE;
            const uint32_t best_idx = have ? (b0[u] & 0xFFFFu) : 0u, t0 = best_idx & ~31u;
            const uint32_t last = (uint32_t)max(nt - 1, 0);
            uint32_t c2 = BF_NONE;
#pragma unroll
            for (int part = 0; part < 4; ++part) {
                uint4 r0[4], r1[4];
#pragma unroll
                for (int i = 0; i < 4; ++i) {
                    const int ii = 4 * part + i;
                    const uint32_t ti = t0 + (uint32_t)(8 * (ii >> 2) + 4 * h + (ii & 3));
                    const uint4 *r = reinterpret_cast<const uint4 *>(tp + (size_t)min(ti, last) * 32);
                    r0[i] = r[0];
                    r1[i] = r[1];
                }
#pragma unroll
                for (int i = 0; i < 4; ++i) {
                    const int ii = 4 * part + i;
                    const uint32_t ti = t0 + (uint32_t)(8 * (ii >> 2) + 4 * h + (ii & 3));
                    const uint32_t key = (ham256(a, r0[i], r1[i]) << 22) | ti;
                    c2 = (have && ti != best_idx && ti < (uint32_t)nt) ? min(c2, key) : c2;
                }
            }
            b1[u] = min(b1[u], c2);
        }
        const uint32_t o0 = __shfl_xor(b0[u], 32, 64), o1 = __shfl_xor(b1[u], 32, 64);
        top2_insert(o0, b0[u], b1[u]);
        top2_insert(o1, b0[u], b1[u]);
        if (h == 0 && qi < nq) {
            const size_t o = ((size_t)pair * nq_cap + qi) * 2;
            idx[o] = b0[u] == BF_NONE ? -1 : (int32_t)(b0[u] & 0xFFFFu);
            idx[o + 1] = b1[u] == BF_NONE ? -1 : (int32_t)(b1[u] & 0xFFFFu);
            dist[o] = b0[u] == BF_NONE ? -1 : (int32_t)(b0[u] >> 22);
            dist[o + 1] = b1[u] == BF_NONE ? -1 : (int32_t)(b1[u] >> 22);
        }
    }
#ifdef MM_BF_CLOCK
    if (threadIdx.x == 0) {
        const unsigned w = blockIdx.x & 4095u;
        g_bf_clock[2 * w] = __builtin_readcyclecounter() - clk_t0;
        g_bf_clock[2 * w + 1] = (long long)(__builtin_amdgcn_s_memrealtime() - clk_r0);
    }
#endif
}

#undef F4M_B
#undef F4M_A
int bf_variant(int n_pairs, int nq_cap) {
    const char *e = getenv("MM_BF_VARIANT");
    const int forced = e ? atoi(e) : 0;
    if (forced) return forced;
    return 314;
}

bool bf_use_mfma(int n_pairs, int nq_cap, int nt_cap) {
    const int v = bf_variant(n_pairs, nq_cap);
    return (v == 200 || v == 300 || v == 310 || v == 314) && nt_cap >= 64 && nt_cap < 65536;
}
int bf_ntp(int nt_cap) { return (nt_cap + MF_TT - 1) / MF_TT * MF_TT; }

int bf_choose_splits(int n_pairs, int nq_cap, int nt_cap) {
    if (bf_use_mfma(n_pairs, nq_cap, nt_cap)) return 1;
    int var = bf_variant(n_pairs, nq_cap);
    if (var == 200 || var >= 300) var = 114;
    const int BF_QTILE = BF_THREADS * ((var / 10) % 10);
    long waves = (long)n_pairs * ((nq_cap + BF_QTILE - 1) / BF_QTILE) * (BF_THREADS / 64);
    if (waves <= 0) return 1;
    long s = (2048 + waves - 1) / waves;
    long smax = (nt_cap + 127) / 128;
    if (s > smax) s = smax;
    if (s > 64) s = 64;
    if (s < 1) s = 1;
    return (int)s;
}

}

#ifdef MM_BF_CLOCK
extern "C" int mm_debug_bf_clock(long long *host ) {
    return (int)hipMemcpyFromSymbol(host, HIP_SYMBOL(g_bf_clock), sizeof(g_bf_clock));
}
#endif

extern "C" {

size_t mm_bf_workspace_bytes(int n_pairs, int nq_cap, int nt_cap) {
    if (n_pairs > 0 && nq_cap > 0 && bf_use_mfma(n_pairs, nq_cap, nt_cap))
        return mm_align_up((size_t)n_pairs * bf_ntp(nt_cap) * (bf_variant(n_pairs, nq_cap) >= 300 ? 128 : 256), 256);
    int s = bf_choose_splits(n_pairs, nq_cap, nt_cap);
    if (s == 1) return 256;
    return mm_align_up((size_t)n_pairs * s * nq_cap * 2 * sizeof(uint32_t), 256);
}

int mm_bf_knn2_batched(mm_ctx *ctx, const uint8_t *q, const int32_t *nq, int nq_cap, size_t q_set_stride,
                       const uint8_t *t, const int32_t *nt, int nt_cap, size_t t_set_stride, int n_pairs,
                       int32_t *idx, int32_t *dist, void *ws, size_t ws_bytes) {
    if (!ctx) return MM_ERR_ARG;
    if (n_pairs == 0 || nq_cap == 0) return MM_OK;
    if (!q || (!t && nt_cap > 0) || !idx || !dist || n_pairs < 0 || nq_cap < 0 || nt_cap < 0)
        return mm_fail(ctx, MM_ERR_ARG, "mm_bf_knn2_batched: bad argument");
    if (nt_cap >= (1 << BF_IDX_BITS)) return mm_fail(ctx, MM_ERR_ARG, "mm_bf_knn2_batched: nt_cap must be < 2^20");
    if (((uintptr_t)q | (uintptr_t)t | q_set_stride | t_set_stride) & 15)
        return mm_fail(ctx, MM_ERR_ARG, "mm_bf_knn2_batched: descriptors must be 16-byte aligned");
    if (n_pairs > 65535) return mm_fail(ctx, MM_ERR_ARG, "mm_bf_knn2_batched: at most 65535 pairs per call");
    int s = bf_choose_splits(n_pairs, nq_cap, nt_cap);
    if (s > 1 && (!ws || ws_bytes < mm_bf_workspace_bytes(n_pairs, nq_cap, nt_cap)))
        return mm_fail(ctx, MM_ERR_WORKSPACE, "mm_bf_knn2_batched: workspace too small");
    if (bf_use_mfma(n_pairs, nq_cap, nt_cap)) {
        if (!ws || ws_bytes < mm_bf_workspace_bytes(n_pairs, nq_cap, nt_cap) || ((uintptr_t)ws & 15))
            return mm_fail(ctx, MM_ERR_WORKSPACE, "mm_bf_knn2_batched: workspace too small or misaligned");
        const int ntp = bf_ntp(nt_cap);
        const dim3 grid((nq_cap + BF_THREADS - 1) / BF_THREADS, 1, n_pairs);
        if (bf_variant(n_pairs, nq_cap) >= 300) {
            const size_t chunks = (size_t)n_pairs * ntp * 8;
            MM_LAUNCH(ctx, "bf_expand_kernel", bf_expand_fp4_kernel, dim3((unsigned)((chunks + 255) / 256)), dim3(256), 0, t, nt_cap,
                      t_set_stride, ntp, n_pairs, (uint8_t *)ws);
            const int qtiles = (int)grid.x;
            const dim3 grid_x(8u * (unsigned)((n_pairs + 7) / 8) * grid.x);
            if (bf_variant(n_pairs, nq_cap) == 310) {
                MM_LAUNCH(ctx, "bf_knn2_fp4min_kernel", (bf_knn2_fp4min_kernel<3, true>), grid_x, dim3(BF_THREADS), 0, q, nq, nq_cap, q_set_stride,
                          (const uint8_t *)ws, t, t_set_stride, nt, nt_cap, ntp, idx, dist, qtiles, n_pairs);
                return MM_OK;
            }
            if (bf_variant(n_pairs, nq_cap) == 314) {
                MM_LAUNCH(ctx, "bf_knn2_fp4min_kernel", (bf_knn2_fp4min_kernel<4, false>), grid_x, dim3(BF_THREADS), 0, q, nq, nq_cap, q_set_stride,
                          (const uint8_t *)ws, t, t_set_stride, nt, nt_cap, ntp, idx, dist, qtiles, n_pairs);
                return MM_OK;
            }
            MM_LAUNCH(ctx, "bf_knn2_fp4_kernel", bf_knn2_fp4_kernel, grid, dim3(BF_THREADS), 0, q, nq, nq_cap, q_set_stride,
                      (const uint8_t *)ws, nt, nt_cap, ntp, idx, dist);
            return MM_OK;
        }
        const size_t chunks = (size_t)n_pairs * ntp * 16;
        MM_LAUNCH(ctx, "bf_expand_kernel", bf_expand_kernel, dim3((unsigned)((chunks + 255) / 256)), dim3(256), 0, t, nt_cap,
                  t_set_stride, ntp, n_pairs, (uint8_t *)ws);
        MM_LAUNCH(ctx, "bf_knn2_mfma_kernel", bf_knn2_mfma_kernel, grid, dim3(BF_THREADS), 0, q, nq, nq_cap, q_set_stride,
                  (const uint8_t *)ws, nt, nt_cap, ntp, idx, dist);
        return MM_OK;
    }
    int var = bf_variant(n_pairs, nq_cap);
    if (var == 200 || var >= 300) var = 114;
    const int qtile = BF_THREADS * ((var / 10) % 10);
    dim3 grid((nq_cap + qtile - 1) / qtile, s, n_pairs);
#define BF_GO(Q, U)                                                                                              \
    MM_LAUNCH(ctx, "bf_knn2_kernel", (bf_knn2_kernel<Q, U>), grid, dim3(BF_THREADS), 0, q, nq, nq_cap, q_set_stride, t, \
              nt, nt_cap, t_set_stride, s, (uint32_t *)ws, idx, dist)
    switch (var) {
        case 14: BF_GO(1, 4); break;
        case 18: BF_GO(1, 8); break;
        case 24: BF_GO(2, 4); break;
        case 28: BF_GO(2, 8); break;
        case 34: BF_GO(3, 4); break;
        case 44: BF_GO(4, 4); break;
        case 48: BF_GO(4, 8); break;
#define BF_GO_LDS(Q)                                                                                             \
    MM_LAUNCH(ctx, "bf_knn2_lds_kernel", (bf_knn2_lds_kernel<Q>), grid, dim3(BF_THREADS), 0, q, nq, nq_cap, q_set_stride, t, \
              nt, nt_cap, t_set_stride, s, (uint32_t *)ws, idx, dist)
        case 114: BF_GO_LDS(1); break;
        case 115:
            MM_LAUNCH(ctx, "bf_knn2_lds_kernel", (bf_knn2_lds_kernel<1, 512>), grid, dim3(BF_THREADS), 0, q, nq, nq_cap, q_set_stride,
                      t, nt, nt_cap, t_set_stride, s, (uint32_t *)ws, idx, dist);
            break;
        case 125:
            MM_LAUNCH(ctx, "bf_knn2_lds_kernel", (bf_knn2_lds_kernel<2, 512>), grid, dim3(BF_THREADS), 0, q, nq, nq_cap, q_set_stride,
                      t, nt, nt_cap, t_set_stride, s, (uint32_t *)ws, idx, dist);
            break;
        case 124: BF_GO_LDS(2); break;
        case 134: BF_GO_LDS(3); break;
        case 144: BF_GO_LDS(4); break;
#undef BF_GO_LDS
        default: return mm_fail(ctx, MM_ERR_ARG, "mm_bf_knn2_batched: unknown MM_BF_VARIANT %d", var);
    }
#undef BF_GO
    if (s > 1) {
        dim3 g2((nq_cap + 255) / 256, n_pairs);
        MM_LAUNCH(ctx, "bf_merge_kernel", bf_merge_kernel, g2, dim3(256), 0, (const uint32_t *)ws, nq, nq_cap, s, idx, dist);
    }
    return MM_OK;
}

int mm_bf_knn2_hamming(mm_ctx *ctx, const uint8_t *q, int nq, const uint8_t *t, int nt, int32_t *idx, int32_t *dist,
                       void *ws, size_t ws_bytes) {
    return mm_bf_knn2_batched(ctx, q, nullptr, nq, 0, t, nullptr, nt, 0, 1, idx, dist, ws, ws_bytes);
}

int mm_ratio_filter_batched(mm_ctx *ctx, const int32_t *idx, const int32_t *dist, const int32_t *nq, int nq_cap,
                            int n_pairs, double threshold, int32_t *pairs, int32_t *m_out) {
    if (!ctx) return MM_ERR_ARG;
    if (n_pairs == 0) return MM_OK;
    if (!idx || !dist || !pairs || !m_out || n_pairs < 0 || nq_cap < 0)
        return mm_fail(ctx, MM_ERR_ARG, "mm_ratio_filter_batched: bad argument");
    MM_LAUNCH(ctx, "ratio_filter_kernel", ratio_filter_kernel, dim3(n_pairs), dim3(256), 0, idx, dist, nq, nq_cap, threshold, pairs, m_out);
    return MM_OK;
}

}
```

meatmodeler_amd/ops.py:

```python
import ctypes as C
import math
import os

import numpy as np
import torch

from . import _lib
from ._lib import lib, ptr, vp, OrbParams, BAProblem, default_context


def _i32(t):
    assert t.dtype == torch.int32 and t.is_contiguous()
    return t



def bf_knn2_batched(q, t, nq=None, nt=None, ctx=None):
    ctx = ctx or default_context()
    assert q.dtype == torch.uint8 and t.dtype == torch.uint8 and q.shape[-1] == 32 and t.shape[-1] == 32
    assert q.stride(-1) == 1 and q.stride(-2) == 32 and t.stride(-1) == 1 and t.stride(-2) == 32
    n_pairs, nq_cap, nt_cap = q.shape[0], q.shape[1], t.shape[1]
    assert t.shape[0] == n_pairs
    both = torch.full((2, n_pairs, nq_cap, 2), -1, dtype=torch.int32, device=q.device)
    idx, dist = both[0], both[1]
    if n_pairs == 0 or nq_cap == 0:
        return idx, dist
    wsb = lib.mm_bf_workspace_bytes(n_pairs, nq_cap, nt_cap)
    ws = torch.empty(wsb, dtype=torch.uint8, device=q.device)
    qs = q.stride(0) if n_pairs > 1 else 0
    ts = t.stride(0) if n_pairs > 1 else 0
    ctx.check(lib.mm_bf_knn2_batched(ctx.h, ptr(q), ptr(nq), nq_cap, qs, ptr(t), ptr(nt), nt_cap, ts, n_pairs,
                                     ptr(idx), ptr(dist), ptr(ws), wsb), "mm_bf_knn2_batched")
    return idx, dist


def bf_knn2(q, t, ctx=None):
    ctx = ctx or default_context()
    assert q.dtype == torch.uint8 and t.dtype == torch.uint8 and q.is_contiguous() and t.is_contiguous()
    nq, nt = q.shape[0], t.shape[0]
    idx = torch.full((nq, 2), -1, dtype=torch.int32, device=q.device)
    dist = torch.full((nq, 2), -1, dtype=torch.int32, device=q.device)
    if nq == 0:
        return idx, dist
    wsb = lib.mm_bf_workspace_bytes(1, nq, nt)
    ws = torch.empty(wsb, dtype=torch.uint8, device=q.device)
    ctx.check(lib.mm_bf_knn2_hamming(ctx.h, ptr(q), nq, ptr(t), nt, ptr(idx), ptr(dist), ptr(ws), wsb),
              "mm_bf_knn2_hamming")
    return idx, dist


def ratio_filter_batched(idx, dist, threshold=0.75, nq=None, ctx=None):
    ctx = ctx or default_context()
    n_pairs, nq_cap = idx.shape[0], idx.shape[1]
    pairs = torch.full((n_pairs, nq_cap, 2), -1, dtype=torch.int32, device=idx.device)
    m = torch.zeros(n_pairs, dtype=torch.int32, device=idx.device)
    if n_pairs == 0:
        return pairs, m
    ctx.check(lib.mm_ratio_filter_batched(ctx.h, ptr(_i32(idx)), ptr(_i32(dist)), ptr(nq), nq_cap, n_pairs,
                                          float(threshold), ptr(pairs), ptr(m)), "mm_ratio_filter_batched")
    return pairs, m


VERIFY_TOO_FEW, VERIFY_NO_MODEL, VERIFY_WEAK, VERIFY_MALFORMED = 1, 2, 4, 8


def verify_matches(kp_xy, pairs, m, n_hyp=256, threshold_px=2.0, min_matches=16, min_inliers=16, refit_iters=2, seed=0,
                   pair_base=0, on_fail="keep", ctx=None):
    if on_fail not in ("keep", "drop"):
        raise ValueError("verify_matches: on_fail must be 'keep' or 'drop'")
    if not 1 <= int(n_hyp) <= 4096:
        raise ValueError("verify_matches: n_hyp must be in 1 .. 4096")
    if not float(threshold_px) >= 0:
        raise ValueError("verify_matches: threshold_px must not be negative")
    if not 0 <= int(refit_iters) <= 1000 or int(min_inliers) < 0:
        raise ValueError("verify_matches: refit_iters must be in 0 .. 1000 and min_inliers not negative")
    if pairs.dim() != 3 or pairs.shape[2] != 2 or kp_xy.dim() != 3 or tuple(kp_xy.shape) != (pairs.shape[0] + 1, pairs.shape[1], 2) \
            or tuple(m.shape) != (pairs.shape[0],):
        raise ValueError("verify_matches: kp_xy [n_pairs+1, cap, 2], pairs [n_pairs, cap, 2] and m [n_pairs] expected")
    ctx = ctx or default_context()
    d = pairs.device
    n_pairs, cap = pairs.shape[0], pairs.shape[1]
    pairs_out = torch.full((n_pairs, cap, 2), -1, dtype=torch.int32, device=d)
    m_out = torch.zeros(n_pairs, dtype=torch.int32, device=d)
    F = torch.full((n_pairs, 9), math.nan, dtype=torch.float64, device=d)
    cost = torch.full((n_pairs,), math.nan, dtype=torch.float64, device=d)
    info = torch.zeros((n_pairs, 4), dtype=torch.int32, device=d)
    if n_pairs == 0 or cap == 0:
        return pairs_out, m_out, F, cost, info
    prm = _lib.VerifyParams(int(n_hyp), int(min_matches), int(min_inliers), int(refit_iters), int(seed) & 0xFFFFFFFF,
                            int(pair_base) & 0xFFFFFFFF, 1 if on_fail == "drop" else 0, 0, float(threshold_px))
    wsb = lib.mm_verify_workspace_bytes(n_pairs, int(n_hyp))
    ws = torch.empty(wsb, dtype=torch.uint8, device=d)
    assert kp_xy.dtype == torch.float32
    ctx.check(lib.mm_verify_matches(ctx.h, ptr(kp_xy.contiguous()), ptr(_i32(pairs.contiguous())), ptr(_i32(m.contiguous())),
                                    n_pairs, cap, C.byref(prm), ptr(pairs_out), ptr(m_out), ptr(F), ptr(cost), ptr(info),
                                    ptr(ws), wsb), "mm_verify_matches")
    return pairs_out, m_out, F, cost, info



def orb_params(nfeatures, nlevels=8, scale_factor=1.2, edge_threshold=31, fast_threshold=20):
    return OrbParams(int(nfeatures), int(nlevels), int(edge_threshold), int(fast_threshold), float(scale_factor), 0)


def orb_level_sizes(H, W, prm):
    L = prm.nlevels
    w = (C.c_int32 * L)()
    h = (C.c_int32 * L)()
    n = (C.c_int32 * L)()
    s = (C.c_float * L)()
    rc = lib.mm_orb_level_sizes(H, W, C.byref(prm), w, h, n, s)
    if rc != 0:
        raise _lib.MMError(f"mm_orb_level_sizes failed ({rc})")
    return np.array(w), np.array(h), np.array(n), np.array(s, np.float32)


class OrbWorkspace:

    def __init__(self, batch, H, W, prm, device, pattern):
        self.batch, self.H, self.W, self.prm = batch, H, W, prm
        nb = lib.mm_orb_workspace_bytes(batch, H, W, C.byref(prm))
        if nb == 0:
            raise _lib.MMError("mm_orb_workspace_bytes: unsupported geometry")
        self.nbytes = nb
        self.ws = torch.empty(nb, dtype=torch.uint8, device=device)
        self.pattern = torch.as_tensor(np.ascontiguousarray(pattern, np.int8)).to(device)
        cap = prm.nfeatures
        self.xy = torch.zeros((batch, cap, 2), dtype=torch.float32, device=device)
        self.meta = torch.zeros((batch, cap, 4), dtype=torch.int32, device=device)
        self.resp = torch.zeros((batch, cap), dtype=torch.float32, device=device)
        self.mom = torch.zeros((batch, cap, 2), dtype=torch.int32, device=device)
        self.desc = torch.zeros((batch, cap, 32), dtype=torch.uint8, device=device)
        self.n = torch.zeros(batch, dtype=torch.int32, device=device)


def orb_detect_compute(imgs, wsp, ctx=None, out=None):
    ctx = ctx or default_context()
    assert imgs.dtype == torch.uint8 and imgs.dim() == 3 and imgs.stride(2) == 1
    B, H, W = imgs.shape
    assert B <= wsp.batch and H == wsp.H and W == wsp.W and imgs.stride(0) == H * imgs.stride(1)
    xy, meta, resp, mom, desc, n = out if out is not None else (wsp.xy, wsp.meta, wsp.resp, wsp.mom, wsp.desc, wsp.n)
    ctx.check(lib.mm_orb_detect_compute(ctx.h, ptr(imgs), B, H, W, imgs.stride(1), C.byref(wsp.prm), ptr(wsp.pattern),
                                        ptr(wsp.ws), wsp.nbytes, ptr(xy), ptr(meta), ptr(resp), ptr(mom), ptr(desc),
                                        ptr(n)), "mm_orb_detect_compute")
    return xy, meta, resp, mom, desc, n



def triangulate_dlt(proj, f0, f1, x0, x1, ctx=None):
    ctx = ctx or default_context()
    n = f0.shape[0]
    X = torch.empty((n, 3), dtype=torch.float64, device=proj.device)
    if n:
        lim = torch.stack([f0.min(), f1.min(), f0.max(), f1.max()]).tolist()
        if min(lim[:2]) < 0 or max(lim[2:]) >= proj.shape[0]:
            raise IndexError("triangulate_dlt: frame index outside the projection table")
        ctx.check(lib.mm_triangulate_dlt(ctx.h, ptr(proj.contiguous()), ptr(_i32(f0)), ptr(_i32(f1)),
                                         ptr(x0.contiguous()), ptr(x1.contiguous()), n, ptr(X)), "mm_triangulate_dlt")
    return X


TRI_BEHIND, TRI_REPROJ, TRI_PARALLAX, TRI_DEGENERATE = 1, 2, 4, 8


def triangulate_tracks(proj, track_ptr, obs_frame, obs_xy, refine_iters=8, max_reproj_px=math.inf, min_angle_deg=0,
                       min_depth=-math.inf, ctx=None):
    if proj.dim() != 3 or tuple(proj.shape[1:]) != (3, 4):
        raise ValueError("triangulate_tracks: proj must be [F,3,4]")
    if not 0 <= int(refine_iters) <= 1000:
        raise ValueError("triangulate_tracks: refine_iters must be in 0 .. 1000")
    if not min_angle_deg >= 0:
        raise ValueError("triangulate_tracks: min_angle_deg must not be negative")
    ctx = ctx or default_context()
    d = proj.device
    F = proj.shape[0]
    tp = _i32(track_ptr.to(torch.int32).contiguous())
    of_ = _i32(obs_frame.to(torch.int32).contiguous())
    xy = obs_xy.to(torch.float64).contiguous()
    T, O = tp.numel() - 1, of_.numel()
    if T < 0 or xy.shape != (O, 2):
        raise ValueError("triangulate_tracks: track_ptr [T+1], obs_frame [O] and obs_xy [O,2] expected")
    X = torch.empty((T, 3), dtype=torch.float64, device=d)
    quality = torch.empty((T, 4), dtype=torch.float64, device=d)
    flags = torch.empty(T, dtype=torch.int32, device=d)
    if T == 0:
        return X, quality, flags
    lim = [tp[0], tp[-1], (tp[1:] - tp[:-1]).min()] + ([of_.min(), of_.max()] if O else [])
    lim = torch.stack([v.long() for v in lim]).tolist()
    if lim[0] < 0 or lim[1] > O or lim[2] < 0:
        raise ValueError("triangulate_tracks: track_ptr is not a CSR over the observations")
    if O and (lim[3] < 0 or lim[4] >= F):
        raise IndexError("triangulate_tracks: frame index outside the projection table")
    max_cos = math.cos(math.radians(min_angle_deg)) if min_angle_deg > 0 else 2.0
    prm = _lib.TriParams(int(refine_iters), 0, float(max_reproj_px), max_cos, float(min_depth))
    ws = torch.empty(max(lib.mm_triangulate_tracks_workspace_bytes(F), 256), dtype=torch.uint8, device=d)
    if O == 0:
        of_ = torch.zeros(1, dtype=torch.int32, device=d)
        xy = torch.zeros((1, 2), dtype=torch.float64, device=d)
    ctx.check(lib.mm_triangulate_tracks(ctx.h, ptr(proj.to(torch.float64).contiguous()), F, ptr(tp), T, ptr(of_), ptr(xy),
                                        C.byref(prm), ptr(X), ptr(quality), ptr(flags), ptr(ws), ws.numel()),
              "mm_triangulate_tracks")
    return X, quality, flags



def link_tracks_device(kp_count, kp_xy, match_count, matches, ctx=None):
    ctx = ctx or default_context()
    F, cap = kp_xy.shape[0], kp_xy.shape[1]
    d = kp_xy.device
    npairs = max(F - 1, 0)
    if matches.shape[0] != npairs or (npairs and matches.shape[1] != cap) or match_count.shape[0] != npairs:
        raise ValueError("link_tracks_device: matches must be [F-1, cap, 2] with match_count [F-1]")
    track_ptr = torch.empty(npairs * cap + 1, dtype=torch.int32, device=d)
    obs_frame = torch.empty(max(2 * npairs * cap, 1), dtype=torch.int32, device=d)
    obs_kp = torch.empty_like(obs_frame)
    counts = torch.zeros(3, dtype=torch.int64, device=d)
    wsb = lib.mm_link_workspace_bytes(F, cap)
    ws = torch.empty(max(wsb, 256), dtype=torch.uint8, device=d)
    ctx.check(lib.mm_link_tracks_device(ctx.h, F, cap, ptr(_i32(kp_count)), ptr(kp_xy.contiguous()),
                                        ptr(_i32(match_count)), ptr(_i32(matches)), ptr(ws), ws.numel(), ptr(track_ptr),
                                        ptr(obs_frame), ptr(obs_kp), ptr(counts)), "mm_link_tracks_device")
    nt, no, bad = (int(v) for v in counts.cpu())
    return track_ptr[:nt + 1], obs_frame[:no], obs_kp[:no], bool(bad)


def flatten_tracks(track_ptr, obs_frame, obs_kp, kp_xy, sel=None, t_lo=0, n_sel=None, frame_offset=0, ctx=None):
    ctx = ctx or default_context()
    d = kp_xy.device
    cap = kp_xy.shape[1]
    tp = track_ptr.to(torch.int32).contiguous()
    T = tp.numel() - 1
    out_ptr = None
    if sel is None:
        n_sel = T - t_lo if n_sel is None else int(n_sel)
        if n_sel < 0 or t_lo < 0 or t_lo + n_sel > T:
            raise ValueError("flatten_tracks: range outside the track list")
        n_obs = int((tp[t_lo + n_sel] - tp[t_lo]).item()) if n_sel else 0
        sel_t = None
    else:
        sel_t = sel.to(torch.int32).contiguous()
        n_sel = sel_t.numel()
        out_ptr = torch.empty(n_sel + 1, dtype=torch.int64, device=d)
        ctx.check(lib.mm_flatten_offsets(ctx.h, ptr(tp), ptr(sel_t) if n_sel else None, n_sel, ptr(out_ptr)), "mm_flatten_offsets")
        n_obs = int(out_ptr[n_sel].item())
    coords = torch.empty((n_obs, 2), dtype=torch.float64, device=d)
    fi = torch.empty(n_obs, dtype=torch.int32, device=d)
    pi = torch.empty(n_obs, dtype=torch.int32, device=d)
    if n_obs:
        ctx.check(lib.mm_flatten_tracks(ctx.h, ptr(tp), ptr(obs_frame.to(torch.int32).contiguous()), ptr(obs_kp.to(torch.int32).contiguous()),
                                        ptr(kp_xy.contiguous()), cap,
                                        ptr(sel_t) if sel_t is not None else None, int(t_lo), n_sel,
                                        ptr(out_ptr) if out_ptr is not None else None, n_obs, int(frame_offset), ptr(coords),
                                        ptr(fi), ptr(pi)), "mm_flatten_tracks")
    return coords, fi, pi



def ba_build_index(F, P, fi, pi):
    fi = np.ascontiguousarray(fi, np.int32)
    pi = np.ascontiguousarray(pi, np.int32)
    O = fi.size
    pt_ptr = np.zeros(P + 1, np.int32)
    cam_ptr = np.zeros(F + 1, np.int32)
    pt_obs = np.zeros(max(O, 1), np.int32)
    cam_obs = np.zeros(max(O, 1), np.int32)
    i32p = _lib.c_i32p
    rc = lib.mm_ba_build_index(F, P, O, fi.ctypes.data_as(i32p), pi.ctypes.data_as(i32p), pt_ptr.ctypes.data_as(i32p),
                               pt_obs.ctypes.data_as(i32p), cam_ptr.ctypes.data_as(i32p), cam_obs.ctypes.data_as(i32p))
    if rc != 0:
        raise ValueError(f"mm_ba_build_index failed ({rc}): frame/point index out of range")
    return pt_ptr, pt_obs[:O], cam_ptr, cam_obs[:O]


class BADevice:

    def __init__(self, K, fi, pi, obs, F, P, device, ctx=None, pairs=True, max_band_span=192, fixed_cams=None):
        self.ctx = ctx or default_context()
        self._mdot = None
        dev = device
        self.device = dev
        self.F, self.P, self.O = int(F), int(P), int(len(fi))
        F, P, O = self.F, self.P, self.O

        def to_dev(a, dtype):
            if isinstance(a, torch.Tensor):
                return a.to(device=dev, dtype=dtype).contiguous()
            return torch.as_tensor(np.ascontiguousarray(a)).to(device=dev, dtype=dtype).contiguous()

        self.K = to_dev(np.asarray(K, np.float64).reshape(9), torch.float64)
        self.fi = to_dev(fi, torch.int32).reshape(-1)
        self.pi = to_dev(pi, torch.int32).reshape(-1)
        self.obs = to_dev(obs, torch.float64).reshape(-1, 2)
        self.fixed_cams, self.F_fixed, self.fx = None, 0, None
        if fixed_cams is not None:
            assert (isinstance(fixed_cams, torch.Tensor) and fixed_cams.dtype == torch.float64 and fixed_cams.device == dev
                    and fixed_cams.dim() == 2 and fixed_cams.shape[1] == 6), "fixed_cams: [F_fixed, 6] f64 device tensor"
            self.F_fixed = int(fixed_cams.shape[0])
            if self.F_fixed:
                self.fixed_cams = fixed_cams.contiguous()
                self.fx = _lib.BAFixed(self.F_fixed, 0, ptr(self.fixed_cams))
        F_all = F + self.F_fixed
        i64 = dict(dtype=torch.int64, device=dev)
        if O:
            lim = torch.stack([self.fi.min(), self.fi.max(), self.pi.min(), self.pi.max(),
                               (self.pi[1:] >= self.pi[:-1]).all().to(torch.int32)]).tolist()
            if lim[0] < 0 or lim[1] >= F_all or lim[2] < 0 or lim[3] >= P:
                raise ValueError("frame / point index out of range")
            point_major = bool(lim[4])
        else:
            point_major = True
        if point_major:
            self.pt_obs = torch.arange(O, dtype=torch.int32, device=dev)
        else:
            self.pt_obs = torch.sort(self.pi, stable=True)[1].to(torch.int32)
        self.pt_ptr = torch.zeros(P + 1, dtype=torch.int32, device=dev)
        self.cam_ptr = torch.zeros(F + 1, dtype=torch.int32, device=dev)
        if O and self.F_fixed:
            self.pt_ptr[1:] = torch.cumsum(torch.bincount(self.pi, minlength=P), 0).to(torch.int32)
            self.cam_ptr[1:] = torch.cumsum(torch.bincount(self.fi, minlength=F_all)[:F], 0).to(torch.int32)
            n_free = int(self.cam_ptr[-1].item())
            self.cam_obs = torch.sort(self.fi, stable=True)[1][:n_free].to(torch.int32).contiguous()
        elif O:
            self.pt_ptr[1:] = torch.cumsum(torch.bincount(self.pi, minlength=P), 0).to(torch.int32)
            self.cam_ptr[1:] = torch.cumsum(torch.bincount(self.fi, minlength=F), 0).to(torch.int32)
            self.cam_obs = torch.sort(self.fi, stable=True)[1].to(torch.int32)
        else:
            self.cam_obs = torch.zeros(0, dtype=torch.int32, device=dev)
        self.cam_span = 0
        self.max_band_span = int(max_band_span)
        self.slabs = None
        self.overlap = os.environ.get("MM_SCHUR_OVERLAP", "0") != "0"
        self.pb = BAProblem(F, P, O, ptr(self.K), ptr(self.fi), ptr(self.pi), ptr(self.obs),
                            ptr(self.pt_ptr), ptr(self.pt_obs), ptr(self.cam_ptr), ptr(self.cam_obs),
                            0, 0, 0, None, None, 0, None, None, None, None, None, None)
        self.n_pairs = 0
        pair_pb, free_idx, O_pairs = self.pb, None, O
        if O and self.F_fixed:
            free_idx = torch.nonzero(self.fi < F).reshape(-1)
            O_pairs = int(free_idx.numel())
            fi_f, pi_f = self.fi[free_idx].contiguous(), self.pi[free_idx].contiguous()
            pt_ptr_f = torch.zeros(P + 1, dtype=torch.int32, device=dev)
            pt_ptr_f[1:] = torch.cumsum(torch.bincount(pi_f, minlength=P), 0).to(torch.int32)
            pt_obs_f = (torch.arange(O_pairs, dtype=torch.int32, device=dev) if point_major
                        else torch.sort(pi_f, stable=True)[1].to(torch.int32))
            self._pair_src = (fi_f, pi_f, pt_ptr_f, pt_obs_f)
            pair_pb = BAProblem(F, P, O_pairs, ptr(self.K), ptr(fi_f), ptr(pi_f), ptr(self.obs), ptr(pt_ptr_f),
                                ptr(pt_obs_f), ptr(self.cam_ptr), ptr(self.cam_obs),
                                0, 0, 0, None, None, 0, None, None, None, None, None, None)
        if O_pairs:
            cnt = torch.empty(O_pairs, dtype=torch.int32, device=dev)
            span_t = torch.zeros(1, dtype=torch.int32, device=dev)
            self.ctx.check(lib.mm_ba_pairs_count(self.ctx.h, C.byref(pair_pb), ptr(cnt), ptr(span_t)),
                           "mm_ba_pairs_count")
            offs = torch.cumsum(cnt, 0, dtype=torch.int64)
            span, n = torch.stack([span_t[0].to(torch.int64), offs[-1]]).tolist()
            self.cam_span = int(span)
            self.pb.cam_span = self.cam_span
            if pairs and self.cam_span <= max_band_span and self.cam_span < F and F * (self.cam_span + 1) < 2 ** 31:
                key = torch.empty(n, dtype=torch.int32, device=dev)
                po = torch.empty(n, dtype=torch.int32, device=dev)
                po2 = torch.empty(n, dtype=torch.int32, device=dev)
                offs_ex = (offs - cnt).contiguous()
                self.ctx.check(lib.mm_ba_pairs_emit(self.ctx.h, C.byref(pair_pb), ptr(offs_ex), self.cam_span, ptr(key),
                                                    ptr(po), ptr(po2)), "mm_ba_pairs_emit")
                key_s, perm = torch.sort(key, stable=True)
                self.pair_o, self.pair_o2 = po[perm].contiguous(), po2[perm].contiguous()
                if free_idx is not None:
                    self.pair_o = free_idx[self.pair_o.long()].to(torch.int32).contiguous()
                    self.pair_o2 = free_idx[self.pair_o2.long()].to(torch.int32).contiguous()
                seg_ids, counts = torch.unique_consecutive(key_s, return_counts=True)
                seg_hi = torch.cumsum(counts, 0)
                seg_lo = seg_hi - counts
                CH = max(64, int(os.environ.get("MM_SCHUR_CHUNK", "512")) // 64 * 64)
                cntc = (counts + (CH - 1)) // CH
                first_hi = torch.cumsum(cntc, 0)
                first = first_hi - cntc
                nchunks = int(first_hi[-1].item())
                chunk_seg = torch.repeat_interleave(torch.arange(len(seg_ids), **i64), cntc, output_size=nchunks)
                chunk_begin = seg_lo[chunk_seg] + CH * (torch.arange(nchunks, **i64) - first[chunk_seg])
                chunk_end = torch.minimum(chunk_begin + CH, seg_hi[chunk_seg])
                i32 = lambda t: t.to(torch.int32).contiguous()
                self.seg_ids = i32(seg_ids)
                self.seg_chunk_ptr = i32(torch.cat([first, first_hi[-1:]]))
                self.chunk_seg, self.chunk_begin, self.chunk_end = i32(chunk_seg), i32(chunk_begin), i32(chunk_end)
                self.n_pairs = int(n)
                self.pb.n_seg = len(seg_ids)
                self.pb.n_chunks = nchunks
                self.pb.seg_ids, self.pb.seg_chunk_ptr = ptr(self.seg_ids), ptr(self.seg_chunk_ptr)
                self.pb.chunk_seg, self.pb.chunk_begin, self.pb.chunk_end = ptr(self.chunk_seg), ptr(self.chunk_begin), ptr(self.chunk_end)
                self.pb.pair_o, self.pb.pair_o2 = ptr(self.pair_o), ptr(self.pair_o2)
                self.pair_p = self.pi[self.pair_o.long()].contiguous()
                self.pb.pair_p = ptr(self.pair_p)
                n_slabs = 8
                cps = -(-F // n_slabs)
                if cps >= 16:
                    seg_cam = seg_ids.to(torch.int64) // (self.cam_span + 1)
                    bounds = torch.arange(n_slabs + 1, **i64) * cps
                    sseg = torch.searchsorted(seg_cam, bounds)
                    schunk = torch.cat([first, first_hi[-1:]])[sseg]
                    self.slabs = (n_slabs, cps, np.ascontiguousarray(sseg.cpu().numpy(), np.int64),
                                  np.ascontiguousarray(schunk.cpu().numpy(), np.int64))
        self._ws = torch.empty(2048 * 8, dtype=torch.uint8, device=dev)
        self._cost2 = torch.zeros(1, dtype=torch.float64, device=dev)
        self._S = None
        self._schur_ws = None
        self._chol_ws = None

    def residual(self, cams, pts, want_res=False, cost_out=None):
        res = torch.empty((self.O, 2), dtype=torch.float64, device=self.device) if want_res else None
        cost2 = cost_out if cost_out is not None else torch.empty(1, dtype=torch.float64, device=self.device)
        if self.fx is not None:
            self.ctx.check(lib.mm_ba_residual_fixed(self.ctx.h, C.byref(self.pb), C.byref(self.fx), ptr(cams), ptr(pts),
                                                    ptr(res), ptr(cost2), ptr(self._ws), self._ws.numel()),
                           "mm_ba_residual_fixed")
            return cost2, res
        self.ctx.check(lib.mm_ba_residual(self.ctx.h, C.byref(self.pb), ptr(cams), ptr(pts), ptr(res), ptr(cost2),
                                          ptr(self._ws), self._ws.numel()), "mm_ba_residual")
        return cost2, res

    def _no_fixed(self, what):
        if self.fx is not None:
            raise NotImplementedError(f"BADevice.{what}: no fixed-camera form (residual, normal_eq and trf_solve have one)")

    def jacobian(self, cams, pts):
        self._no_fixed("jacobian")
        Jc = torch.empty((self.O, 2, 6), dtype=torch.float64, device=self.device)
        Jp = torch.empty((self.O, 2, 3), dtype=torch.float64, device=self.device)
        self.ctx.check(lib.mm_ba_jacobian(self.ctx.h, C.byref(self.pb), ptr(cams), ptr(pts), ptr(Jc), ptr(Jp)),
                       "mm_ba_jacobian")
        return Jc, Jp

    def normal_eq(self, cams, pts, want_cams=True, want_pts=True, out=None):
        d = self.device
        if out is not None:
            B, gc, Cb, gp = out
            for t_ in out:
                assert t_ is None or (t_.dtype == torch.float64 and t_.is_contiguous())
        else:
            B = torch.empty((self.F, 6, 6), dtype=torch.float64, device=d) if want_cams else None
            gc = torch.empty((self.F, 6), dtype=torch.float64, device=d) if want_cams else None
            Cb = torch.empty((self.P, 6), dtype=torch.float64, device=d) if want_pts else None
            gp = torch.empty((self.P, 3), dtype=torch.float64, device=d) if want_pts else None
        if self.fx is not None:
            self.ctx.check(lib.mm_ba_normal_eq_fixed(self.ctx.h, C.byref(self.pb), C.byref(self.fx), ptr(cams), ptr(pts),
                                                     ptr(B), ptr(gc), ptr(Cb), ptr(gp)), "mm_ba_normal_eq_fixed")
            return B, gc, Cb, gp
        self.ctx.check(lib.mm_ba_normal_eq(self.ctx.h, C.byref(self.pb), ptr(cams), ptr(pts), ptr(B), ptr(gc), ptr(Cb),
                                           ptr(gp)), "mm_ba_normal_eq")
        return B, gc, Cb, gp

    def jvp(self, cams, pts, wc, wp):
        self._no_fixed("jvp")
        out = torch.empty((self.O, 2), dtype=torch.float64, device=self.device)
        self.ctx.check(lib.mm_ba_jvp(self.ctx.h, C.byref(self.pb), ptr(cams), ptr(pts), ptr(wc), ptr(wp), ptr(out)),
                       "mm_ba_jvp")
        return out

    def jvp_dots(self, cams, pts, wc, wp, other=None):
        self._no_fixed("jvp_dots")
        out = torch.empty((self.O, 2), dtype=torch.float64, device=self.device)
        rows = torch.empty((2, 3), dtype=torch.float64, device=self.device)
        if getattr(self, "_jvp_ws", None) is None:
            self._jvp_ws = torch.zeros(lib.mm_ba_jvp_dots_workspace_bytes(C.byref(self.pb)), dtype=torch.uint8,
                                       device=self.device)
        self.ctx.check(lib.mm_ba_jvp_dots(self.ctx.h, C.byref(self.pb), ptr(cams), ptr(pts), ptr(wc), ptr(wp), ptr(out),
                                          ptr(other), ptr(rows), ptr(self._jvp_ws), self._jvp_ws.numel()), "mm_ba_jvp_dots")
        return out, rows

    def schur(self, cams, pts, Bd, Cd, gc, gp):
        self._no_fixed("schur")
        n = 6 * self.F
        if self._S is None:
            self._alloc_S(n)
        S = self._S
        v = torch.empty(n, dtype=torch.float64, device=self.device)
        Cinv = torch.empty((self.P, 6), dtype=torch.float64, device=self.device)
        if self._schur_ws is None:
            nb = lib.mm_ba_schur_workspace_bytes(C.byref(self.pb))
            self._schur_ws = torch.empty(max(nb, 256), dtype=torch.uint8, device=self.device)
        self.ctx.check(lib.mm_ba_schur(self.ctx.h, C.byref(self.pb), ptr(cams), ptr(pts), ptr(Bd), ptr(Cd), ptr(gc),
                                       ptr(gp), ptr(S), ptr(v), ptr(Cinv), ptr(self._schur_ws),
                                       self._schur_ws.numel()), "mm_ba_schur")
        return S, v, Cinv

    def _alloc_S(self, n):
        self._S_storage = torch.zeros(2 * n * n, dtype=torch.float64, device=self.device)
        self._S = self._S_storage[:n * n].view(n, n)

    def band_view(self, half_bandwidth):
        n = 6 * self.F
        hb = int(min(half_bandwidth, n - 1))
        return torch.as_strided(self._S_storage, (n, hb + 1), (n + 1, n))

    def schur_solve(self, cams, pts, Bd, Cd, gc, gp, half_bandwidth):
        self._no_fixed("schur_solve")
        n = 6 * self.F
        if self._S is None:
            self._alloc_S(n)
        v = torch.empty(n, dtype=torch.float64, device=self.device)
        Cinv = torch.empty((self.P, 6), dtype=torch.float64, device=self.device)
        info = torch.zeros(1, dtype=torch.int32, device=self.device)
        if self._schur_ws is None:
            nb = lib.mm_ba_schur_workspace_bytes(C.byref(self.pb))
            self._schur_ws = torch.empty(max(nb, 256), dtype=torch.uint8, device=self.device)
        if self._chol_ws is None:
            self._chol_ws = torch.empty(lib.mm_chol_workspace_bytes(n), dtype=torch.uint8, device=self.device)
        hb = int(min(half_bandwidth, n))
        if self.slabs is not None and self.overlap:
            ns, cps, sseg, schunk = self.slabs
            a_seg, a_chunk = sseg.ctypes.data_as(_lib.c_i64p), schunk.ctypes.data_as(_lib.c_i64p)
        else:
            ns, cps, a_seg, a_chunk = 0, 0, None, None
        self.ctx.check(lib.mm_ba_schur_solve(self.ctx.h, C.byref(self.pb), ptr(cams), ptr(pts), ptr(Bd), ptr(Cd), ptr(gc),
                                             ptr(gp), ptr(self._S), ptr(v), ptr(Cinv), hb, ptr(info), ptr(self._schur_ws),
                                             self._schur_ws.numel(), ptr(self._chol_ws), self._chol_ws.numel(), ns, cps,
                                             a_seg, a_chunk), "mm_ba_schur_solve")
        return info, v, Cinv

    def multi_dot(self, pairs, split=0):
        if self._mdot is None:
            self._mdot = MultiDot(self.device, self.ctx)
        return self._mdot(pairs, split)

    _FUSED_ROWS = (2, 3, 2, 6, 0, 0)

    def trf_fused(self, op, ins, outs, scalars=(), h0=0.0, h1=0.0, split=0):
        if self._mdot is None:
            self._mdot = MultiDot(self.device, self.ctx)
        ws = self._mdot.ws
        n = outs[0].numel()
        for t in list(ins) + list(outs) + list(scalars):
            assert t.dtype == torch.float64 and t.is_contiguous()
        pin = (C.c_void_p * len(ins))(*[t.data_ptr() for t in ins])
        pout = (C.c_void_p * len(outs))(*[t.data_ptr() for t in outs])
        psc = (C.c_void_p * max(len(scalars), 1))(*[t.data_ptr() for t in scalars]) if scalars else None
        rows = self._FUSED_ROWS[op]
        if n == 0:
            return torch.zeros((max(rows, 1), 3), dtype=torch.float64, device=self.device)
        res = torch.empty((max(rows, 1), 3), dtype=torch.float64, device=self.device)
        self.ctx.check(lib.mm_trf_fused(self.ctx.h, op, pin, pout, psc, float(h0), float(h1), n, int(split), ptr(res), ptr(ws),
                                        ws.numel()), "mm_trf_fused")
        return res

    def trf_step2d(self, r0, d11, r1, r2, r3, bs, reg, info, Delta, board):
        self.ctx.check(lib.mm_trf_step2d(self.ctx.h, ptr(r0), ptr(d11), ptr(r1), ptr(r2), ptr(r3), ptr(bs), ptr(reg),
                                         ptr(info), float(Delta), ptr(board)), "mm_trf_step2d")

    def trf_damping(self, gh2, d11, Delta, min_damping):
        return trf_damping(gh2, d11, Delta, min_damping, self.ctx)

    def chol_solve(self, S, v, half_bandwidth=None):
        return chol_solve(S, v, self.ctx, half_bandwidth=half_bandwidth)

    def scale_update(self, B, Cb, si, first):
        self.ctx.check(lib.mm_ba_scale_update(self.ctx.h, self.F, self.P, ptr(B), ptr(Cb), ptr(si), 1 if first else 0),
                       "mm_ba_scale_update")
        return si

    def damp(self, B, Cb, si, reg, Bd, Cd):
        assert reg.dtype == torch.float64 and reg.numel() == 1
        self.ctx.check(lib.mm_ba_damp(self.ctx.h, self.F, self.P, ptr(B), ptr(Cb), ptr(si), ptr(reg), ptr(Bd), ptr(Cd)),
                       "mm_ba_damp")
        return Bd, Cd

    def chol_solve_sym(self, S, v, half_bandwidth, both_triangles):
        return chol_solve_sym(S, v, self.ctx, half_bandwidth, both_triangles)

    def trf_solve(self, cams, pts, ftol, xtol, gtol, max_nfev=None, min_damping=1e-9, log_cap=0):
        for t in (cams, pts):
            assert t.dtype == torch.float64 and t.is_contiguous() and t.device == self.device
        if getattr(self, "_trf_ws", None) is None:
            nb = (lib.mm_ba_trf_fixed_workspace_bytes(C.byref(self.pb), C.byref(self.fx)) if self.fx is not None
                  else lib.mm_ba_trf_workspace_bytes(C.byref(self.pb)))
            self._trf_ws = torch.empty(nb, dtype=torch.uint8, device=self.device)
        prm = _lib.TrfParams(ftol, xtol, gtol, min_damping, int(max_nfev) if max_nfev else 0)
        rep = _lib.TrfReport()
        log = (_lib.TrfRow * max(log_cap, 1))()
        if self.fx is not None:
            name = "mm_ba_trf_fixed"
            rc = lib.mm_ba_trf_fixed(self.ctx.h, C.byref(self.pb), C.byref(self.fx), ptr(cams), ptr(pts), C.byref(prm),
                                     C.byref(rep), log, int(log_cap), ptr(self._trf_ws), self._trf_ws.numel())
        else:
            name = "mm_ba_trf"
            rc = lib.mm_ba_trf(self.ctx.h, C.byref(self.pb), ptr(cams), ptr(pts), C.byref(prm), C.byref(rep), log,
                               int(log_cap), ptr(self._trf_ws), self._trf_ws.numel())
        if rc and rep.status == -2:
            raise ValueError("Residuals are not finite in the initial point.")
        self.ctx.check(rc, name)
        rows = [(r.iteration, r.nfev, r.cost, r.reduction, r.step_norm, r.optimality)
                for r in log[:min(rep.log_rows, log_cap)]]
        return rep, rows

    def trf_solve_dist(self, cams, pts, ftol, xtol, gtol, allreduce, half_bandwidth, band_exchange, max_nfev=None,
                       min_damping=1e-9, log_cap=0):
        self._no_fixed("trf_solve_dist")
        for t in (cams, pts):
            assert t.dtype == torch.float64 and t.is_contiguous() and t.device == self.device
        need = lib.mm_ba_trf_dist_workspace_bytes(C.byref(self.pb), int(half_bandwidth))
        if getattr(self, "_trf_ws_dist", None) is None or self._trf_ws_dist.numel() < need:
            self._trf_ws_dist = torch.empty(need, dtype=torch.uint8, device=self.device)
        ws = self._trf_ws_dist
        base = ws.data_ptr()
        err = []

        def _cb(user, buf, count):
            try:
                off = int(buf) - base
                with torch.cuda.stream(self.ctx.stream):
                    allreduce(ws[off:off + 8 * int(count)].view(torch.float64))
                return 0
            except BaseException as e:
                err.append(e)
                return 1
        cb = _lib.ALLREDUCE_FN(_cb)
        d = _lib.Dist(int(getattr(allreduce, "rank", 0)), int(getattr(allreduce, "world_size", 1)), int(half_bandwidth),
                      1 if band_exchange else 0, cb, None)
        prm = _lib.TrfParams(ftol, xtol, gtol, min_damping, int(max_nfev) if max_nfev else 0)
        rep = _lib.TrfReport()
        log = (_lib.TrfRow * max(log_cap, 1))()
        rc = lib.mm_ba_trf_dist(self.ctx.h, C.byref(self.pb), ptr(cams), ptr(pts), C.byref(prm), C.byref(rep), log,
                                int(log_cap), ptr(ws), ws.numel(), C.byref(d))
        if err:
            raise err[0]
        if rc and rep.status == -2:
            raise ValueError("Residuals are not finite in the initial point.")
        self.ctx.check(rc, "mm_ba_trf_dist")
        rows = [(r.iteration, r.nfev, r.cost, r.reduction, r.step_norm, r.optimality)
                for r in log[:min(rep.log_rows, log_cap)]]
        return rep, rows

    def backsub(self, cams, pts, Cinv, gp, dc):
        self._no_fixed("backsub")
        dp = torch.empty((self.P, 3), dtype=torch.float64, device=self.device)
        if getattr(self, "_backsub_ws", None) is None:
            self._backsub_ws = torch.empty(lib.mm_ba_backsub_workspace_bytes(C.byref(self.pb)), dtype=torch.uint8,
                                           device=self.device)
        self.ctx.check(lib.mm_ba_backsub(self.ctx.h, C.byref(self.pb), ptr(cams), ptr(pts), ptr(Cinv), ptr(gp), ptr(dc),
                                         ptr(dp), ptr(self._backsub_ws), self._backsub_ws.numel()), "mm_ba_backsub")
        return dp


def trf_solve_batched(problems, cams_list, pts_list, ftol, xtol, gtol, max_nfev=None, min_damping=1e-9, ctx=None):
    n = len(problems)
    if n == 0:
        return [], []
    ctx = ctx or problems[0].ctx
    dev = problems[0].device
    pbs = (C.POINTER(_lib.BAProblem) * n)()
    cams_p, pts_p, ws_p = (C.c_void_p * n)(), (C.c_void_p * n)(), (C.c_void_p * n)()
    ws_b = (C.c_size_t * n)()
    keep = []
    for k, (pb, cm, pt) in enumerate(zip(problems, cams_list, pts_list)):
        for t in (cm, pt):
            assert t.dtype == torch.float64 and t.is_contiguous() and t.device == dev
        assert pb.device == dev
        need = lib.mm_ba_trf_batched_workspace_bytes(C.byref(pb.pb))
        if getattr(pb, "_trf_ws", None) is None or pb._trf_ws.numel() < need:
            pb._trf_ws = torch.empty(need, dtype=torch.uint8, device=dev)
        pbs[k] = C.pointer(pb.pb)
        cams_p[k], pts_p[k], ws_p[k], ws_b[k] = cm.data_ptr(), pt.data_ptr(), pb._trf_ws.data_ptr(), pb._trf_ws.numel()
        keep.append(pb._trf_ws)
    prm = _lib.TrfParams(ftol, xtol, gtol, min_damping, int(max_nfev) if max_nfev else 0)
    reps = (_lib.TrfReport * n)()
    alone = (C.c_int32 * n)()
    rc = lib.mm_ba_trf_batched(ctx.h, n, pbs, cams_p, pts_p, C.byref(prm), reps, ws_p, ws_b, alone)
    if rc and any(r.status == -2 for r in reps):
        raise ValueError("Residuals are not finite in the initial point.")
    ctx.check(rc, "mm_ba_trf_batched")
    return list(reps), [bool(a) for a in alone]


class MultiDot:

    def __init__(self, device, ctx=None):
        self.ctx = ctx or default_context()
        self.ws = torch.zeros(lib.mm_multi_dot_workspace_bytes(), dtype=torch.uint8, device=device)

    def __call__(self, pairs, split=0):
        out_all = []
        for i0 in range(0, len(pairs), 8):
            chunk = pairs[i0:i0 + 8]
            k = len(chunk)
            n = chunk[0][0].numel()
            if n == 0:
                out_all.append(torch.zeros((k, 3), dtype=torch.float64, device=self.ws.device))
                continue
            for a, b in chunk:
                assert a.dtype == torch.float64 and b.dtype == torch.float64 and a.is_contiguous() and b.is_contiguous()
                assert a.numel() == n and b.numel() == n
            pa = (C.c_void_p * k)(*[a.data_ptr() for a, _ in chunk])
            pb_ = (C.c_void_p * k)(*[b.data_ptr() for _, b in chunk])
            out = torch.empty((k, 3), dtype=torch.float64, device=self.ws.device)
            self.ctx.check(lib.mm_multi_dot(self.ctx.h, k, pa, pb_, n, int(split), ptr(out), ptr(self.ws), self.ws.numel()),
                           "mm_multi_dot")
            out_all.append(out)
        return out_all[0] if len(out_all) == 1 else torch.cat(out_all)


def trf_damping(gh2, d11, Delta, min_damping, ctx=None):
    ctx = ctx or default_context()
    out = torch.empty(2, dtype=torch.float64, device=gh2.device)
    ctx.check(lib.mm_trf_damping(ctx.h, ptr(gh2), ptr(d11), float(Delta), float(min_damping), ptr(out)), "mm_trf_damping")
    return out


def chol_solve(A, b, ctx=None, half_bandwidth=None):
    ctx = ctx or default_context()
    n = A.shape[0]
    assert A.dtype == torch.float64 and A.is_contiguous() and b.is_contiguous() and b.shape[-1] == n
    nrhs = 1 if b.dim() == 1 else b.shape[0]
    info = torch.zeros(1, dtype=torch.int32, device=A.device)
    wsb = lib.mm_chol_workspace_bytes(n)
    ws = torch.empty(wsb, dtype=torch.uint8, device=A.device)
    hb = n if half_bandwidth is None else int(min(half_bandwidth, n))
    ctx.check(lib.mm_chol_solve(ctx.h, ptr(A), n, ptr(b), nrhs, hb, ptr(info), ptr(ws), wsb), "mm_chol_solve")
    return info


def chol_solve_sym(A, b, ctx=None, half_bandwidth=None, both_triangles=True):
    ctx = ctx or default_context()
    n = A.shape[0]
    assert A.dtype == torch.float64 and A.is_contiguous() and b.is_contiguous() and b.dim() == 1 and b.shape[0] == n
    info = torch.zeros(1, dtype=torch.int32, device=A.device)
    wsb = lib.mm_chol_workspace_bytes(n)
    ws = torch.empty(wsb, dtype=torch.uint8, device=A.device)
    hb = n if half_bandwidth is None else int(min(half_bandwidth, n))
    ctx.check(lib.mm_chol_solve_sym(ctx.h, ptr(A), n, ptr(b), hb, 1 if both_triangles else 0, ptr(info), ptr(ws), wsb),
              "mm_chol_solve_sym")
    return info



def pyramid(img, max_level, ctx=None):
    ctx = ctx or default_context()
    assert img.dtype == torch.uint8 and img.dim() == 2 and img.is_contiguous()
    levels = [img]
    for _ in range(int(max_level)):
        s = levels[-1]
        h, w = s.shape
        d = torch.empty(((h + 1) // 2, (w + 1) // 2), dtype=torch.uint8, device=s.device)
        ctx.check(lib.mm_pyr_down(ctx.h, ptr(s), w, h, s.stride(0), ptr(d), d.stride(0)), "mm_pyr_down")
        levels.append(d)
    return levels


def lk_track(prev_levels, next_levels, pts, win=(21, 21), max_count=30, epsilon=0.01, ctx=None):
    ctx = ctx or default_context()
    L = len(prev_levels)
    assert len(next_levels) == L and pts.dtype == torch.float32 and pts.is_contiguous() and pts.shape[-1] == 2
    n = pts.shape[0]
    d = pts.device
    out = torch.empty((n, 2), dtype=torch.float32, device=d)
    st = torch.empty(n, dtype=torch.uint8, device=d)
    err = torch.empty(n, dtype=torch.float32, device=d)
    if n == 0:
        return out, st, err
    arr_p = (C.c_void_p * L)(*[t.data_ptr() for t in prev_levels])
    arr_n = (C.c_void_p * L)(*[t.data_ptr() for t in next_levels])
    ws = (C.c_int * L)(*[t.shape[1] for t in prev_levels])
    hs = (C.c_int * L)(*[t.shape[0] for t in prev_levels])
    ps = (C.c_int * L)(*[t.stride(0) for t in prev_levels])
    for a, b in zip(prev_levels, next_levels):
        assert a.shape == b.shape and a.stride(0) == b.stride(0)
    eps = min(max(float(epsilon), 0.0), 10.0) ** 2
    ctx.check(lib.mm_lk_track(ctx.h, arr_p, arr_n, ws, hs, ps, L, ptr(pts), n, int(win[0]), int(win[1]),
                              min(max(int(max_count), 0), 100), eps, ptr(out), ptr(st), ptr(err)), "mm_lk_track")
    return out, st, err


def min_eig(img, block_size=3, ctx=None):
    ctx = ctx or default_context()
    assert img.dtype == torch.uint8 and img.dim() == 2 and img.stride(1) == 1
    h, w = img.shape
    eig = torch.empty((h, w), dtype=torch.float64, device=img.device)
    ctx.check(lib.mm_min_eig(ctx.h, ptr(img), w, h, img.stride(0), int(block_size), ptr(eig)), "mm_min_eig")
    return eig


def good_features(img, max_corners, quality, min_distance, block_size=3, ctx=None):
    ctx = ctx or default_context()
    h, w = img.shape
    if h < 3 or w < 3:
        return np.zeros((0, 2), np.float32)
    eig = min_eig(img, block_size, ctx)
    cap = h * w
    d = img.device
    mx = torch.zeros(1, dtype=torch.int64, device=d)
    vb = torch.empty(cap, dtype=torch.int64, device=d)
    pos = torch.empty(cap, dtype=torch.int32, device=d)
    cnt = torch.zeros(1, dtype=torch.int32, device=d)
    ctx.check(lib.mm_corner_candidates(ctx.h, ptr(eig), w, h, float(quality), ptr(mx), ptr(vb), ptr(pos), cap, ptr(cnt)),
              "mm_corner_candidates")
    n = min(int(cnt.item()), cap)
    if n == 0:
        return np.zeros((0, 2), np.float32)
    pos_s, o1 = torch.sort(pos[:n], stable=True)
    _, o2 = torch.sort(vb[:n][o1], descending=True, stable=True)
    pos_h = np.ascontiguousarray(pos_s[o2].cpu().numpy(), np.int32)
    out_cap = int(max_corners) if max_corners and max_corners > 0 else n
    out = np.zeros((max(out_cap, 1), 2), np.float32)
    m = lib.mm_gftt_select(pos_h.ctypes.data_as(C.c_void_p), n, w, h, int(max_corners or 0), float(min_distance),
                           out.ctypes.data_as(C.c_void_p), out_cap)
    if m < 0:
        raise _lib.MMError(f"mm_gftt_select failed ({m})")
    return out[:m]


_LAB_TABLES = {}


def increase_contrast(bgr, clip_limit=3.5, tiles=(8, 8), want_grey=False, ctx=None):
# ... 25 lines not shown
```

meatmodeler_amd/pipeline.py:

```python
import ctypes as C
import queue
import time
from concurrent.futures import ThreadPoolExecutor

import numpy as np
import torch

from . import _lib, ops, parallel
from ._lib import lib, default_context, c_i32p, c_i64p, c_f32p, MMError
from .bundleAdjuster import SchurTRF, frameParameters
from .orb_pattern import brief_pattern


VERIFY_KEYS = ("n_hyp", "threshold_px", "min_matches", "min_inliers", "refit_iters", "seed", "on_fail")


def verify_options(verify):
    if verify is None:
        return None
    if not isinstance(verify, dict):
        raise ValueError("verify must be None or a dict of " + ", ".join(VERIFY_KEYS))
    unknown = set(verify) - set(VERIFY_KEYS)
    if unknown:
        raise ValueError(f"verify takes {', '.join(VERIFY_KEYS)}; not {sorted(unknown)}")
    return dict(verify)


class ClipPipeline:
    def __init__(self, height, width, nfeatures, batch=32, ratio=0.75, device=None, ctx=None, nlevels=8):
        self.ctx = ctx or default_context()
        self.device = device or self.ctx.device
        self.H, self.W = height, width
        self.prm = ops.orb_params(nfeatures, nlevels=nlevels)
        self.cap = nfeatures
        self.batch = batch
        self.ratio = ratio
        self.wsp = ops.OrbWorkspace(batch, height, width, self.prm, self.device, brief_pattern())
        self.scales = ops.orb_level_sizes(height, width, self.prm)[3]

    def detect(self, frames):
        F = frames.shape[0]
        d = self.device
        out = dict(xy=torch.zeros((F, self.cap, 2), dtype=torch.float32, device=d),
                   meta=torch.zeros((F, self.cap, 4), dtype=torch.int32, device=d),
                   resp=torch.zeros((F, self.cap), dtype=torch.float32, device=d),
                   mom=torch.zeros((F, self.cap, 2), dtype=torch.int32, device=d),
                   desc=torch.zeros((F, self.cap, 32), dtype=torch.uint8, device=d),
                   n=torch.zeros(F, dtype=torch.int32, device=d))
        for b0 in range(0, F, self.batch):
            b1 = min(F, b0 + self.batch)
            ops.orb_detect_compute(frames[b0:b1], self.wsp, self.ctx,
                                   out=(out["xy"][b0:b1], out["meta"][b0:b1], out["resp"][b0:b1], out["mom"][b0:b1],
                                        out["desc"][b0:b1], out["n"][b0:b1]))
        return out

    def match(self, det, pair_lo=0, pair_hi=None):
        F = det["desc"].shape[0]
        if pair_hi is None:
            pair_hi = F - 1
        npairs = max(pair_hi - pair_lo, 0)
        desc, n = det["desc"], det["n"]
        if npairs == 0:
            return (torch.zeros((0, self.cap, 2), dtype=torch.int32, device=self.device),
                    torch.zeros(0, dtype=torch.int32, device=self.device))
        q = desc[pair_lo:pair_hi]
        t = desc[pair_lo + 1:pair_hi + 1]
        idx, dist = ops.bf_knn2_batched(q, t, n[pair_lo:pair_hi].contiguous(), n[pair_lo + 1:pair_hi + 1].contiguous(),
                                        self.ctx)
        return ops.ratio_filter_batched(idx, dist, self.ratio, n[pair_lo:pair_hi].contiguous(), self.ctx)

    def verify(self, det, pairs, m, pair_lo=0, **params):
        n = pairs.shape[0]
        return ops.verify_matches(det["xy"][:n + 1], pairs, m, pair_base=pair_lo, ctx=self.ctx, **params)

    def link(self, kp_count, kp_xy, match_count, matches):
        kp_count = np.ascontiguousarray(kp_count, np.int32)
        kp_xy = np.ascontiguousarray(kp_xy, np.float32)
        match_count = np.ascontiguousarray(match_count, np.int32)
        matches = np.ascontiguousarray(matches, np.int32)
        F = len(kp_count)
        cap = kp_xy.shape[1] if kp_xy.ndim == 3 else 0
        mcap = matches.shape[1] if matches.ndim == 3 else 0
        total = int(match_count.sum())
        track_ptr = np.zeros(total + 2, np.int64)
        obs_frame = np.zeros(2 * total + 2, np.int32)
        obs_kp = np.zeros(2 * total + 2, np.int32)
        n_obs = C.c_int64(0)
        nt = lib.mm_link_tracks_clip(F, cap, kp_count.ctypes.data_as(c_i32p), kp_xy.ctypes.data_as(c_f32p), mcap,
                                     match_count.ctypes.data_as(c_i32p), matches.ctypes.data_as(c_i32p), total + 1,
                                     2 * total + 1, track_ptr.ctypes.data_as(c_i64p), obs_frame.ctypes.data_as(c_i32p),
                                     obs_kp.ctypes.data_as(c_i32p), C.byref(n_obs))
        if nt < 0:
            raise MMError(f"mm_link_tracks_clip failed ({nt})")
        return track_ptr[:nt + 1], obs_frame[:n_obs.value], obs_kp[:n_obs.value]

    def triangulate(self, track_ptr, obs_frame, obs_kp, kp_xy_dev, projections):
        d = self.device
        track_ptr, obs_frame, obs_kp = (t if torch.is_tensor(t) else torch.as_tensor(np.ascontiguousarray(t)).to(d)
                                        for t in (track_ptr, obs_frame, obs_kp))
        T = track_ptr.shape[0] - 1
        if T <= 0:
            return torch.zeros((0, 3), dtype=torch.float64, device=d)
        first = track_ptr[:-1].long()
        last = track_ptr[1:].long() - 1
        f0, f1 = obs_frame[first].int(), obs_frame[last].int()
        x0 = kp_xy_dev[f0.long(), obs_kp[first].long()].to(torch.float64)
        x1 = kp_xy_dev[f1.long(), obs_kp[last].long()].to(torch.float64)
        proj = torch.as_tensor(np.ascontiguousarray(projections, np.float64)).to(d)
        return ops.triangulate_dlt(proj, f0.contiguous(), f1.contiguous(), x0, x1, self.ctx)

    def triangulate_multi_view(self, track_ptr, obs_frame, obs_kp, kp_xy_dev, projections, **thresholds):
        coords, of_, _ = ops.flatten_tracks(track_ptr, obs_frame, obs_kp, kp_xy_dev, ctx=self.ctx)
        proj = torch.as_tensor(np.ascontiguousarray(projections, np.float64)).to(self.device)
        return ops.triangulate_tracks(proj, track_ptr, of_, coords, ctx=self.ctx, **thresholds)

    @staticmethod
    def flatten(track_ptr, obs_frame, obs_kp, kp_xy_host):
        lens = np.diff(track_ptr).astype(np.int64)
        pi = np.repeat(np.arange(len(lens), dtype=np.int32), lens)
        coords = kp_xy_host[obs_frame, obs_kp].astype(np.float64)
        return coords, obs_frame.astype(np.int32), pi

    @staticmethod
    def window_selection(first_frame, last_frame, lo, hi, n_frames):
        inside = (first_frame >= lo) & (last_frame < hi)
        if hi >= n_frames:
            return inside
        return inside & (last_frame <= hi - 2)

    @staticmethod
    def window_selection_anchored(first_frame, last_frame, lo, hi, n_frames):
        del first_frame
        sel = (last_frame >= lo) & (last_frame < hi)
        if hi >= n_frames:
            return sel
        return sel & (last_frame <= hi - 2)

    def adjust_windows(self, out, K, extrinsics, window=50, stride=25, ftol=1e-4, verbose=0, timers=None, dist=None,
                       order="sequential", streams=1, batched=False, max_nfev=None, boundary="inside"):
        d = self.device
        world = dist.get_world_size() if dist is not None else 1
        rank = dist.get_rank() if dist is not None else 0
        if order not in ("sequential", "wavefront"):
            raise ValueError("order must be 'sequential' or 'wavefront'")
        if boundary not in ("inside", "anchored"):
            raise ValueError("boundary must be 'inside' or 'anchored'")
        if boundary == "anchored":
            if order != "sequential" or batched or int(streams) > 1 or dist is not None:
                raise ValueError("boundary='anchored' needs order='sequential' on one rank and one stream (no batched): "
                                 "its windows read the cameras earlier windows settled")
            return self._adjust_windows_anchored(out, K, extrinsics, window, stride, ftol, verbose, timers, max_nfev)
        allreduce = parallel.AllReduce() if world > 1 else None
        if order == "wavefront":
            return self._adjust_windows_wavefront(out, K, extrinsics, window, stride, ftol, verbose, timers, allreduce,
                                                  world, rank, streams, batched, max_nfev)
        F = int(np.asarray(extrinsics).shape[0])
        tp, of_, ok = out["track_ptr_dev"], out["obs_frame_dev"], out["obs_kp_dev"]
        xy = out["xy_dev"]
        T = tp.shape[0] - 1
        with np.errstate(all="ignore"):
            cams = torch.as_tensor(frameParameters(np.asarray(extrinsics, float)[:, :3, :]).reshape(F, 6)).to(d)
        pts = out["points0"].clone()
        stats = []
        if T == 0:
            return dict(cams=cams, points=pts, windows=stats)
        tp64 = tp.long()
        first_f, last_f = of_[tp64[:-1]], of_[tp64[1:] - 1]
        lens_all = tp64[1:] - tp64[:-1]
        window = max(2, min(int(window), F))
        his = list(range(window, F, max(1, int(stride)))) + [F]
        t0 = time.perf_counter()
        for hi in his:
            lo = max(0, hi - window)
            sel = torch.nonzero(self.window_selection(first_f, last_f, lo, hi, F)).reshape(-1)
            P = int(sel.numel())
            if P == 0:
                continue
            lens = lens_all[sel]
            P_all, p_lo, p_hi = P, 0, P
            if world > 1 and P >= 4 * world:
                cum = torch.cat([torch.zeros(1, dtype=torch.int64, device=d), torch.cumsum(lens, 0)])
                bounds = parallel.split_by_weight(cum, world)
                p_lo, p_hi = bounds[rank], bounds[rank + 1]
                sel_all, sel = sel, sel[p_lo:p_hi]
                lens = lens[p_lo:p_hi]
                P = p_hi - p_lo
            sharded = world > 1 and P_all >= 4 * world
            coords, fi, pi = ops.flatten_tracks(tp, of_, ok, xy, sel=sel, frame_offset=lo, ctx=self.ctx)
            O = int(fi.numel())
            pb = ops.BADevice(K, fi, pi, coords, hi - lo, P, d, self.ctx)
            res = SchurTRF(pb, allreduce=allreduce if sharded else None).solve(
                cams[lo:hi].contiguous(), pts[sel].contiguous(), ftol=ftol, max_nfev=max_nfev, verbose=verbose if rank == 0 else 0)
            cams[lo:hi] = res.cams
            if sharded:
                buf = torch.zeros((P_all, 3), dtype=torch.float64, device=d)
                buf[p_lo:p_hi] = res.pts
                allreduce(buf)
                pts[sel_all] = buf
                O_all = torch.tensor([float(O)], dtype=torch.float64, device=d)
                allreduce(O_all)
                O = int(O_all.item())
            else:
                pts[sel] = res.pts
            stats.append(dict(lo=lo, hi=hi, points=P_all, observations=O, nfev=res.nfev, cost=res.cost,
                              status=res.status))
        self.ctx.sync()
        if timers is not None:
            timers["ba_windows"] = timers.get("ba_windows", 0.0) + (time.perf_counter() - t0) * 1e3
        return dict(cams=cams, points=pts, windows=stats)

    def _adjust_windows_anchored(self, out, K, extrinsics, window, stride, ftol, verbose, timers, max_nfev):
        d = self.device
        F = int(np.asarray(extrinsics).shape[0])
        tp, of_, ok = out["track_ptr_dev"], out["obs_frame_dev"], out["obs_kp_dev"]
        xy = out["xy_dev"]
        T = tp.shape[0] - 1
        with np.errstate(all="ignore"):
            cams = torch.as_tensor(frameParameters(np.asarray(extrinsics, float)[:, :3, :]).reshape(F, 6)).to(d)
        pts = out["points0"].clone()
        stats = []
        if T == 0:
            return dict(cams=cams, points=pts, windows=stats)
        tp64 = tp.long()
        first_f, last_f = of_[tp64[:-1]], of_[tp64[1:] - 1]
        window = max(2, min(int(window), F))
        his = list(range(window, F, max(1, int(stride)))) + [F]
        t0 = time.perf_counter()
        for hi in his:
            lo = max(0, hi - window)
            W = hi - lo
            sel = torch.nonzero(self.window_selection_anchored(first_f, last_f, lo, hi, F)).reshape(-1)
            P = int(sel.numel())
            if P == 0:
                continue
            coords, fi, pi = ops.flatten_tracks(tp, of_, ok, xy, sel=sel, frame_offset=lo, ctx=self.ctx)
            O = int(fi.numel())
            n_fixed = 0
            if lo > 0:
                fi = torch.where(fi < 0, fi + (lo + W), fi).contiguous()
                n_fixed = int(torch.unique(fi[fi >= W]).numel())
                pb = ops.BADevice(K, fi, pi, coords, W, P, d, self.ctx, fixed_cams=cams[:lo].clone())
            else:
                pb = ops.BADevice(K, fi, pi, coords, W, P, d, self.ctx)
            res = SchurTRF(pb).solve(cams[lo:hi].contiguous(), pts[sel].contiguous(), ftol=ftol, max_nfev=max_nfev,
                                     verbose=verbose)
            cams[lo:hi] = res.cams
            pts[sel] = res.pts
            stats.append(dict(lo=lo, hi=hi, points=P, observations=O, fixed_cameras=n_fixed, nfev=res.nfev, cost=res.cost,
                              status=res.status))
        self.ctx.sync()
        if timers is not None:
            timers["ba_windows"] = timers.get("ba_windows", 0.0) + (time.perf_counter() - t0) * 1e3
        return dict(cams=cams, points=pts, windows=stats)

    def _window_problem(self, out, first_f, last_f, lens_all, tp64, lo, hi, F, ctx=None):
        d = self.device
        of_, ok, xy = out["obs_frame_dev"], out["obs_kp_dev"], out["xy_dev"]
        sel = torch.nonzero(self.window_selection(first_f, last_f, lo, hi, F)).reshape(-1)
        P = int(sel.numel())
        if P == 0:
            return sel, None, None, None, 0, 0
        coords, fi, pi = ops.flatten_tracks(out["track_ptr_dev"], of_, ok, xy, sel=sel, frame_offset=lo, ctx=ctx or self.ctx)
        return sel, fi, pi, coords, P, int(fi.numel())

    def _adjust_windows_wavefront(self, out, K, extrinsics, window, stride, ftol, verbose, timers, allreduce, world, rank,
                                  streams=1, batched=False, max_nfev=None):
        d = self.device
        F = int(np.asarray(extrinsics).shape[0])
        tp, of_ = out["track_ptr_dev"], out["obs_frame_dev"]
        T = tp.shape[0] - 1
        with np.errstate(all="ignore"):
            cams = torch.as_tensor(frameParameters(np.asarray(extrinsics, float)[:, :3, :]).reshape(F, 6)).to(d)
        pts = out["points0"].clone()
        if T == 0:
            return dict(cams=cams, points=pts, windows=[])
        tp64 = tp.long()
        first_f, last_f = of_[tp64[:-1]], of_[tp64[1:] - 1]
        lens_all = tp64[1:] - tp64[:-1]
        window = max(2, min(int(window), F))
        his = list(range(window, F, max(1, int(stride)))) + [F]
        wins = [(max(0, hi - window), hi) for hi in his]
        colour_end, colours = [], []
        for lo, hi in wins:
            c = next((k for k, e in enumerate(colour_end) if e <= lo), len(colour_end))
            if c == len(colour_end):
                colour_end.append(hi)
            else:
                colour_end[c] = hi
            colours.append(c)
        t0 = time.perf_counter()
        table = torch.zeros((len(wins), 5), dtype=torch.float64, device=d)
        n_streams = max(1, int(streams))
        slots = queue.SimpleQueue()
        if n_streams > 1:
            for _ in range(n_streams):
                st = torch.cuda.Stream(device=d)
                slots.put((st, _lib.Context(d, st)))

        def solve_window(k, ctx, cams, pts, cams_upd, cam_mask, pts_upd, pt_mask):
            lo, hi = wins[k]
            sel, fi, pi, coords, P, O = self._window_problem(out, first_f, last_f, lens_all, tp64, lo, hi, F, ctx)
            if P == 0:
                return
            pb = ops.BADevice(K, fi, pi, coords, hi - lo, P, d, ctx)
            res = SchurTRF(pb).solve(cams[lo:hi].contiguous(), pts[sel].contiguous(), ftol=ftol, max_nfev=max_nfev,
                                     verbose=verbose if rank == 0 and n_streams == 1 else 0)
            cams_upd[lo:hi] = res.cams
            cam_mask[lo:hi] = 1.0
            pts_upd[sel] = res.pts
            pt_mask[sel] = 1.0
            table[k] = torch.tensor([P, O, res.nfev, res.status, res.cost], dtype=torch.float64, device=d)

        def solve_window_on_slot(k, *state):
            slot = slots.get()
            try:
                with torch.cuda.stream(slot[0]):
                    solve_window(k, slot[1], *state)
                    slot[0].synchronize()
            finally:
                slots.put(slot)

        for c in range(len(colour_end)):
            mine = [k for j, k in enumerate(k for k, cc in enumerate(colours) if cc == c) if j % world == rank]
            cams_upd, pts_upd = torch.zeros_like(cams), torch.zeros_like(pts)
            cam_mask = torch.zeros(F, dtype=torch.float64, device=d)
            pt_mask = torch.zeros(T, dtype=torch.float64, device=d)
            state = (cams, pts, cams_upd, cam_mask, pts_upd, pt_mask)
            if batched and len(mine) > 1:
                items = []
                for k in mine:
                    lo, hi = wins[k]
                    sel, fi, pi, coords, P, O = self._window_problem(out, first_f, last_f, lens_all, tp64, lo, hi, F)
                    if P == 0:
                        continue
                    pb = ops.BADevice(K, fi, pi, coords, hi - lo, P, d, self.ctx)
                    items.append((k, sel, pb, cams[lo:hi].contiguous(), pts[sel].contiguous(), P, O))
                reps, _ = ops.trf_solve_batched([it[2] for it in items], [it[3] for it in items], [it[4] for it in items],
                                                ftol, 1e-8, 1e-8, max_nfev=max_nfev, ctx=self.ctx)
                rows, ks = [], []
                for (k, sel, pb, cw, pw, P, O), rep in zip(items, reps):
                    lo, hi = wins[k]
                    cams_upd[lo:hi] = cw
                    cam_mask[lo:hi] = 1.0
                    pts_upd[sel] = pw
                    pt_mask[sel] = 1.0
                    rows.append([P, O, rep.nfev, rep.status, rep.cost])
                    ks.append(k)
                if ks:
                    table[torch.tensor(ks, device=d)] = torch.tensor(rows, dtype=torch.float64, device=d)
            elif n_streams > 1 and len(mine) > 1:
                torch.cuda.current_stream(d).synchronize()
                with ThreadPoolExecutor(max_workers=n_streams) as pool:
                    for f_ in [pool.submit(solve_window_on_slot, k, *state) for k in mine]:
                        f_.result()
            else:
                for k in mine:
                    solve_window(k, self.ctx, *state)
            if allreduce is not None:
                for t_ in (cams_upd, cam_mask, pts_upd, pt_mask):
                    allreduce(t_)
            cams = torch.where(cam_mask[:, None] > 0, cams_upd, cams)
            pts = torch.where(pt_mask[:, None] > 0, pts_upd, pts)
        if allreduce is not None:
            allreduce(table)
        self.ctx.sync()
        if timers is not None:
            timers["ba_windows"] = timers.get("ba_windows", 0.0) + (time.perf_counter() - t0) * 1e3
        tab = table.cpu().numpy()
        stats = [dict(lo=wins[k][0], hi=wins[k][1], points=int(r[0]), observations=int(r[1]), nfev=int(r[2]), status=int(r[3]),
                      cost=float(r[4]), colour=colours[k]) for k, r in enumerate(tab) if r[0] > 0]
        return dict(cams=cams, points=pts, windows=stats)

# ... 133 lines not shown
```

Baseline: 8556 billion descriptor pairs/s (match stage).

## Fuse brute-force kNN with ratio filter and build BA index natively on GPU

Matching now calls a single fused kernel that does the Hamming 2-NN search and the ratio test together. This avoids writing and re-reading the intermediate idx/dist arrays and saves one launch. Separately, a native HIP index builder using rocprim sorts, scans and run-length encoding replaces the torch-based BA index construction, which cuts host-side torch op overhead. Together these add a large amount of new native code and a second matching path that has to stay in agreement with the old two-step one.

```diff
diff --git a/include/meatmodeler.h b/include/meatmodeler.h
--- a/include/meatmodeler.h
+++ b/include/meatmodeler.h
@@ -48,6 +48,12 @@
 int mm_ratio_filter_batched(mm_ctx *ctx, const int32_t *idx , const int32_t *dist ,
                             const int32_t *nq , int nq_cap, int n_pairs, double threshold,
                             int32_t *pairs , int32_t *m_out );
+size_t mm_bf_match_ratio_workspace_bytes(int n_pairs, int nq_cap, int nt_cap);
+int mm_bf_match_ratio_batched(mm_ctx *ctx, const uint8_t *q , const int32_t *nq , int nq_cap,
+                              size_t q_set_stride, const uint8_t *t , const int32_t *nt , int nt_cap,
+                              size_t t_set_stride, int n_pairs, double threshold,
+                              int32_t *pairs , int32_t *m_out ,
+                              void *ws , size_t ws_bytes);
 
 typedef struct mm_orb_params {
     int32_t nfeatures;
@@ -156,6 +162,22 @@
 int mm_ba_pairs_count(mm_ctx *ctx, const mm_ba_problem *pb, int32_t *cnt , int32_t *span_out );
 int mm_ba_pairs_emit(mm_ctx *ctx, const mm_ba_problem *pb, const int64_t *offsets , int span,
                      int32_t *key , int32_t *pair_o , int32_t *pair_o2 );
+typedef struct mm_ba_index {
+    int32_t F, P;
+    int64_t O;
+    const int32_t *fi, *pi;
+    int32_t *pt_ptr, *pt_obs, *cam_ptr, *cam_obs;
+    int64_t *head;
+    int32_t cam_span, chunk;
+    int64_t n_pairs;
+    int32_t *pair_o, *pair_o2, *pair_p;
+    int32_t *seg_ids, *seg_chunk_ptr;
+    int32_t *chunk_seg, *chunk_begin, *chunk_end;
+} mm_ba_index;
+int mm_ba_index_bounds(int F, int cam_span, int64_t n_pairs, int chunk, int64_t *seg_cap, int64_t *chunk_cap);
+size_t mm_ba_index_workspace_bytes(mm_ctx *ctx, const mm_ba_index *ix, int stage);
+int mm_ba_index_build(mm_ctx *ctx, const mm_ba_index *ix, int stage, void *ws0 , size_t ws0_bytes,
+                      void *ws1 , size_t ws1_bytes);
 size_t mm_multi_dot_workspace_bytes(void);
 int mm_multi_dot(mm_ctx *ctx, int k, const double *const *a, const double *const *b, int64_t n, int64_t split,
                  double *out, void *ws, size_t ws_bytes);
diff --git a/meatmodeler_amd/_lib.py b/meatmodeler_amd/_lib.py
--- a/meatmodeler_amd/_lib.py
+++ b/meatmodeler_amd/_lib.py
@@ -28,6 +28,14 @@
                 ("cam_span", C.c_int32), ("reserved", C.c_int32), ("n_seg", C.c_int64), ("seg_ids", vp),
                 ("seg_chunk_ptr", vp), ("n_chunks", C.c_int64), ("chunk_seg", vp), ("chunk_begin", vp),
                 ("chunk_end", vp), ("pair_o", vp), ("pair_o2", vp), ("pair_p", vp)]
+
+
+class BAIndex(C.Structure):
+    _fields_ = [("F", C.c_int32), ("P", C.c_int32), ("O", C.c_int64), ("fi", vp), ("pi", vp),
+                ("pt_ptr", vp), ("pt_obs", vp), ("cam_ptr", vp), ("cam_obs", vp), ("head", vp),
+                ("cam_span", C.c_int32), ("chunk", C.c_int32), ("n_pairs", C.c_int64),
+                ("pair_o", vp), ("pair_o2", vp), ("pair_p", vp), ("seg_ids", vp), ("seg_chunk_ptr", vp),
+                ("chunk_seg", vp), ("chunk_begin", vp), ("chunk_end", vp)]
 
 
 class BAFixed(C.Structure):
@@ -89,6 +97,9 @@
                                      vp, C.c_size_t]),
     "mm_bf_knn2_hamming": (C.c_int, [vp, vp, C.c_int, vp, C.c_int, vp, vp, vp, C.c_size_t]),
     "mm_ratio_filter_batched": (C.c_int, [vp, vp, vp, vp, C.c_int, C.c_int, C.c_double, vp, vp]),
+    "mm_bf_match_ratio_workspace_bytes": (C.c_size_t, [C.c_int, C.c_int, C.c_int]),
+    "mm_bf_match_ratio_batched": (C.c_int, [vp, vp, vp, C.c_int, C.c_size_t, vp, vp, C.c_int, C.c_size_t, C.c_int,
+                                            C.c_double, vp, vp, vp, C.c_size_t]),
     "mm_orb_workspace_bytes": (C.c_size_t, [C.c_int, C.c_int, C.c_int, C.POINTER(OrbParams)]),
     "mm_orb_detect_compute": (C.c_int, [vp, vp, C.c_int, C.c_int, C.c_int, C.c_int, C.POINTER(OrbParams), vp, vp,
                                         C.c_size_t, vp, vp, vp, vp, vp, vp]),
@@ -115,6 +126,9 @@
     "mm_ba_schur_workspace_bytes": (C.c_size_t, [C.POINTER(BAProblem)]),
     "mm_ba_pairs_count": (C.c_int, [vp, C.POINTER(BAProblem), vp, vp]),
     "mm_ba_pairs_emit": (C.c_int, [vp, C.POINTER(BAProblem), vp, C.c_int, vp, vp, vp]),
+    "mm_ba_index_bounds": (C.c_int, [C.c_int, C.c_int, C.c_int64, C.c_int, c_i64p, c_i64p]),
+    "mm_ba_index_workspace_bytes": (C.c_size_t, [vp, C.POINTER(BAIndex), C.c_int]),
+    "mm_ba_index_build": (C.c_int, [vp, C.POINTER(BAIndex), C.c_int, vp, C.c_size_t, vp, C.c_size_t]),
     "mm_ba_schur_solve": (C.c_int, [vp, C.POINTER(BAProblem), vp, vp, vp, vp, vp, vp, vp, vp, vp, C.c_int, vp, vp,
                                     C.c_size_t, vp, C.c_size_t, C.c_int, C.c_int, c_i64p, c_i64p]),
     "mm_multi_dot_workspace_bytes": (C.c_size_t, []),
diff --git a/meatmodeler_amd/csrc/ba_index.hip b/meatmodeler_amd/csrc/ba_index.hip
--- /dev/null
+++ b/meatmodeler_amd/csrc/ba_index.hip
@@ -0,0 +1,307 @@
+#include <cstring>
+#include "mm_common.h"
+#include <rocprim/rocprim.hpp>
+
+namespace {
+
+constexpr int HEAD_SPAN = 0, HEAD_PAIRS = 1, HEAD_BAD_RANGE = 2, HEAD_NOT_POINT_MAJOR = 3, HEAD_SEG = 4, HEAD_CHUNKS = 5;
+
+__device__ __forceinline__ bool idx_ok(const int64_t *head) { return head[HEAD_BAD_RANGE] == 0 && head[HEAD_NOT_POINT_MAJOR] == 0; }
+
+__global__ __launch_bounds__(256) void idx_validate_kernel(const int32_t *__restrict__ fi, const int32_t *__restrict__ pi,
+                                                           int64_t O, int F, int P, int64_t *__restrict__ head) {
+    const int64_t o = (int64_t)blockIdx.x * 256 + threadIdx.x;
+    bool bad = false, unsorted = false;
+    if (o < O) {
+        const int f = fi[o], p = pi[o];
+        bad = f < 0 || f >= F || p < 0 || p >= P;
+        unsorted = o > 0 && pi[o - 1] > p;
+    }
+    if (__ballot(bad) != 0 && (threadIdx.x & 63) == 0) head[HEAD_BAD_RANGE] = 1;
+    if (__ballot(unsorted) != 0 && (threadIdx.x & 63) == 0) head[HEAD_NOT_POINT_MAJOR] = 1;
+}
+
+__global__ __launch_bounds__(256) void idx_ptr_kernel(const int32_t *__restrict__ keys, int64_t n, int nbins,
+                                                      int32_t *__restrict__ ptr, int32_t *__restrict__ identity,
+                                                      const int64_t *__restrict__ head) {
+    if (!idx_ok(head)) return;
+    const int64_t i = (int64_t)blockIdx.x * 256 + threadIdx.x;
+    if (i >= n) return;
+    const int k = keys[i];
+    const int lo = i == 0 ? 0 : keys[i - 1] + 1;
+    for (int b = lo; b <= k; ++b) ptr[b] = (int32_t)i;
+    if (i == n - 1)
+        for (int b = k + 1; b <= nbins; ++b) ptr[b] = (int32_t)n;
+    if (identity) identity[i] = (int32_t)i;
+}
+
+__global__ __launch_bounds__(256) void idx_count_kernel(const int32_t *__restrict__ fi, const int32_t *__restrict__ pi,
+                                                        const int32_t *__restrict__ pt_ptr, int64_t O,
+                                                        int32_t *__restrict__ cnt, int32_t *__restrict__ span_out,
+                                                        const int64_t *__restrict__ head) {
+    if (!idx_ok(head)) return;
+    const int64_t o = (int64_t)blockIdx.x * 256 + threadIdx.x;
+    int dmax = 0;
+    if (o < O) {
+        const int f = fi[o], p = pi[o];
+        int c = 0;
+        for (int e = pt_ptr[p]; e < pt_ptr[p + 1]; ++e) {
+            const int d = f - fi[e];
+            c += d >= 0;
+            dmax = max(dmax, d);
+        }
+        cnt[o] = c;
+    }
+    for (int off = 32; off > 0; off >>= 1) dmax = max(dmax, __shfl_down(dmax, off, 64));
+    if ((threadIdx.x & 63) == 0 && dmax > __hip_atomic_load(span_out, __ATOMIC_RELAXED, __HIP_MEMORY_SCOPE_AGENT)) atomicMax(span_out, dmax);
+}
+
+__global__ void idx_head0_kernel(const int32_t *__restrict__ cnt, const int64_t *__restrict__ offs, int64_t O,
+                                 const int32_t *__restrict__ span, int64_t *__restrict__ head) {
+    if (!idx_ok(head)) return;
+    head[HEAD_SPAN] = *span;
+    head[HEAD_PAIRS] = offs[O - 1] + cnt[O - 1];
+}
+
+__global__ __launch_bounds__(256) void idx_emit_kernel(const int32_t *__restrict__ fi, const int32_t *__restrict__ pi,
+                                                       const int32_t *__restrict__ pt_ptr, int64_t O,
+                                                       const int64_t *__restrict__ offs, int span, int64_t n_pairs,
+                                                       int32_t *__restrict__ key, uint64_t *__restrict__ val,
+                                                       const int64_t *__restrict__ head) {
+    if (!idx_ok(head)) return;
+    const int64_t o = (int64_t)blockIdx.x * 256 + threadIdx.x;
+    if (o >= O) return;
+    const int f = fi[o], p = pi[o];
+    int64_t w = offs[o];
+    for (int e = pt_ptr[p]; e < pt_ptr[p + 1]; ++e) {
+        const int d = f - fi[e];
+        if (d < 0) continue;
+        if (w >= n_pairs) return;
+        key[w] = f * (span + 1) + min(d, span);
+        val[w] = ((uint64_t)(uint32_t)e << 32) | (uint32_t)o;
+        ++w;
+    }
+}
+
+__global__ __launch_bounds__(256) void idx_unpack_kernel(const uint64_t *__restrict__ val, const int32_t *__restrict__ pi,
+                                                         int64_t n_pairs, int64_t O, int32_t *__restrict__ pair_o,
+                                                         int32_t *__restrict__ pair_o2, int32_t *__restrict__ pair_p) {
+    const int64_t i = (int64_t)blockIdx.x * 256 + threadIdx.x;
+    if (i >= n_pairs) return;
+    const uint64_t v = val[i];
+    const uint32_t o = (uint32_t)v, o2 = (uint32_t)(v >> 32);
+    pair_o[i] = (int32_t)o;
+    pair_o2[i] = (int32_t)o2;
+    pair_p[i] = pi[min((int64_t)o, O - 1)];
+}
+
+__global__ __launch_bounds__(256) void idx_segcount_kernel(const int32_t *__restrict__ counts, const int32_t *__restrict__ n_seg,
+                                                           int64_t seg_cap, int chunk, int32_t *__restrict__ pairs_of,
+                                                           int32_t *__restrict__ chunks_of) {
+    const int64_t s = (int64_t)blockIdx.x * 256 + threadIdx.x;
+    if (s > seg_cap) return;
+    const int c = s < *n_seg ? counts[s] : 0;
+    pairs_of[s] = c;
+    chunks_of[s] = (c + chunk - 1) / chunk;
+}
+
+__global__ __launch_bounds__(256) void idx_chunks_kernel(const int32_t *__restrict__ n_seg_dev, const int32_t *__restrict__ seg_lo,
+                                                         const int32_t *__restrict__ pairs_of,
+                                                         const int32_t *__restrict__ seg_chunk_ptr, int chunk, int64_t chunk_cap,
+                                                         int32_t *__restrict__ chunk_seg, int32_t *__restrict__ chunk_begin,
+                                                         int32_t *__restrict__ chunk_end, int64_t *__restrict__ head) {
+    const int64_t s = ((int64_t)blockIdx.x * 256 + threadIdx.x) >> 6;
+    const int lane = threadIdx.x & 63;
+    const int n_seg = *n_seg_dev;
+    if (s == 0 && lane == 0) {
+        head[HEAD_SEG] = n_seg;
+        head[HEAD_CHUNKS] = seg_chunk_ptr[n_seg];
+    }
+    if (s >= n_seg) return;
+    const int lo = seg_lo[s], hi = lo + pairs_of[s];
+    const int64_t c0 = seg_chunk_ptr[s], c1 = seg_chunk_ptr[s + 1];
+    for (int64_t c = c0 + lane; c < c1 && c < chunk_cap; c += 64) {
+        const int b = lo + chunk * (int)(c - c0);
+        chunk_seg[c] = (int32_t)s;
+        chunk_begin[c] = b;
+        chunk_end[c] = min(b + chunk, hi);
+    }
+}
+
+int bits_for(int64_t n_values) {
+    int b = 1;
+    while (b < 63 && ((int64_t)1 << b) < n_values) ++b;
+    return b;
+}
+
+struct Carve {
+    size_t at = 0;
+    size_t take(size_t bytes) {
+        const size_t o = at;
+        at += mm_align_up(bytes ? bytes : 1, 256);
+        return o;
+    }
+};
+struct Ws0 {
+    size_t keys, cnt, offs, span, tmp, tmp_bytes, total;
+};
+struct Ws1 {
+    size_t key, val, key_s, val_s, counts, n_seg, pairs_of, chunks_of, seg_lo, tmp, tmp_bytes, total;
+};
+
+hipError_t ws0_layout(int F, int64_t O, hipStream_t st, Ws0 &w) {
+    size_t t_sort = 0, t_scan = 0;
+    hipError_t e = rocprim::radix_sort_pairs(nullptr, t_sort, (const int32_t *)nullptr, (int32_t *)nullptr, (const int32_t *)nullptr,
+                                             (int32_t *)nullptr, (size_t)O, 0u, (unsigned)bits_for(F), st);
+    if (e != hipSuccess) return e;
+    e = rocprim::exclusive_scan(nullptr, t_scan, (const int32_t *)nullptr, (int64_t *)nullptr, (int64_t)0, (size_t)O,
+                                rocprim::plus<int64_t>(), st);
+    if (e != hipSuccess) return e;
+    Carve c;
+    w.keys = c.take((size_t)O * 4);
+    w.cnt = c.take((size_t)O * 4);
+    w.offs = c.take((size_t)O * 8);
+    w.span = c.take(4);
+    w.tmp_bytes = t_sort > t_scan ? t_sort : t_scan;
+    w.tmp = c.take(w.tmp_bytes);
+    w.total = c.at;
+    return hipSuccess;
+}
+
+hipError_t ws1_layout(int64_t n_pairs, int64_t seg_cap, int key_bits, hipStream_t st, Ws1 &w) {
+    size_t t_sort = 0, t_rle = 0, t_scan = 0;
+    hipError_t e = rocprim::radix_sort_pairs(nullptr, t_sort, (const int32_t *)nullptr, (int32_t *)nullptr, (const uint64_t *)nullptr,
+                                             (uint64_t *)nullptr, (size_t)n_pairs, 0u, (unsigned)key_bits, st);
+    if (e != hipSuccess) return e;
+    e = rocprim::run_length_encode(nullptr, t_rle, (const int32_t *)nullptr, (size_t)n_pairs, (int32_t *)nullptr, (int32_t *)nullptr,
+                                   (int32_t *)nullptr, st);
+    if (e != hipSuccess) return e;
+    e = rocprim::exclusive_scan(nullptr, t_scan, (const int32_t *)nullptr, (int32_t *)nullptr, (int32_t)0, (size_t)seg_cap + 1,
+                                rocprim::plus<int32_t>(), st);
+    if (e != hipSuccess) return e;
+    Carve c;
+    w.key = c.take((size_t)n_pairs * 4);
+    w.val = c.take((size_t)n_pairs * 8);
+    w.key_s = c.take((size_t)n_pairs * 4);
+    w.val_s = c.take((size_t)n_pairs * 8);
+    w.counts = c.take((size_t)seg_cap * 4);
+    w.n_seg = c.take(4);
+    w.pairs_of = c.take((size_t)(seg_cap + 1) * 4);
+    w.chunks_of = c.take((size_t)(seg_cap + 1) * 4);
+    w.seg_lo = c.take((size_t)(seg_cap + 1) * 4);
+    w.tmp_bytes = t_sort > t_rle ? t_sort : t_rle;
+    if (t_scan > w.tmp_bytes) w.tmp_bytes = t_scan;
+    w.tmp = c.take(w.tmp_bytes);
+    w.total = c.at;
+    return hipSuccess;
+}
+
+bool index_args_ok(const mm_ba_index *ix) {
+    return ix && ix->F > 0 && ix->P > 0 && ix->O > 0 && ix->O < 0x7fffffffLL && ix->fi && ix->pi && ix->head;
+}
+bool band_ok(const mm_ba_index *ix) {
+    return ix->cam_span >= 0 && ix->cam_span < ix->F && (int64_t)ix->F * (ix->cam_span + 1) < 0x80000000LL && ix->n_pairs > 0 &&
+           ix->n_pairs < 0x7fffffffLL && ix->chunk >= 64 && ix->chunk % 64 == 0;
+}
+
+}
+
+extern "C" {
+
+int mm_ba_index_bounds(int F, int cam_span, int64_t n_pairs, int chunk, int64_t *seg_cap, int64_t *chunk_cap) {
+    if (F <= 0 || cam_span < 0 || n_pairs < 0 || chunk <= 0 || !seg_cap || !chunk_cap) return MM_ERR_ARG;
+    const int64_t keys = (int64_t)F * ((int64_t)cam_span + 1);
+    *seg_cap = n_pairs < keys ? n_pairs : keys;
+    *chunk_cap = *seg_cap + n_pairs / chunk;
+    return MM_OK;
+}
+
+size_t mm_ba_index_workspace_bytes(mm_ctx *ctx, const mm_ba_index *ix, int stage) {
+    if (!ctx || !index_args_ok(ix)) return 0;
+    if (stage == 0) {
+        Ws0 w;
+        return ws0_layout(ix->F, ix->O, ctx->stream, w) == hipSuccess ? w.total : 0;
+    }
+    if (stage != 1 || !band_ok(ix)) return 0;
+    int64_t seg_cap, chunk_cap;
+    mm_ba_index_bounds(ix->F, ix->cam_span, ix->n_pairs, ix->chunk, &seg_cap, &chunk_cap);
+    Ws1 w;
+    return ws1_layout(ix->n_pairs, seg_cap, bits_for((int64_t)ix->F * (ix->cam_span + 1)), ctx->stream, w) == hipSuccess ? w.total : 0;
+}
+
+int mm_ba_index_build(mm_ctx *ctx, const mm_ba_index *ix, int stage, void *ws0, size_t ws0_bytes, void *ws1, size_t ws1_bytes) {
+    if (!ctx) return MM_ERR_ARG;
+    if (!index_args_ok(ix) || !ix->pt_ptr || !ix->pt_obs || !ix->cam_ptr || !ix->cam_obs || !ws0 || ((uintptr_t)ws0 & 15))
+        return mm_fail(ctx, MM_ERR_ARG, "mm_ba_index_build: bad argument");
+    const int64_t O = ix->O;
+    const unsigned gO = (unsigned)((O + 255) / 256);
+    hipStream_t st = ctx->stream;
+    Ws0 w0;
+    MM_HIP(ctx, ws0_layout(ix->F, O, st, w0));
+    if (ws0_bytes < w0.total) return mm_fail(ctx, MM_ERR_WORKSPACE, "mm_ba_index_build: stage 0 workspace too small");
+    uint8_t *b0 = (uint8_t *)ws0;
+    int32_t *keys = (int32_t *)(b0 + w0.keys), *cnt = (int32_t *)(b0 + w0.cnt), *span = (int32_t *)(b0 + w0.span);
+    int64_t *offs = (int64_t *)(b0 + w0.offs);
+    if (stage == 0) {
+        MM_HIP(ctx, hipMemsetAsync(ix->head, 0, 8 * sizeof(int64_t), st));
+        MM_HIP(ctx, hipMemsetAsync(span, 0, sizeof(int32_t), st));
+        MM_LAUNCH(ctx, "idx_validate_kernel", idx_validate_kernel, dim3(gO), dim3(256), 0, ix->fi, ix->pi, O, ix->F, ix->P, ix->head);
+        MM_LAUNCH(ctx, "idx_ptr_kernel", idx_ptr_kernel, dim3(gO), dim3(256), 0, ix->pi, O, ix->P, ix->pt_ptr, ix->pt_obs,
+                  (const int64_t *)ix->head);
+        size_t tb = w0.tmp_bytes;
+        MM_HIP(ctx, rocprim::radix_sort_pairs((void *)(b0 + w0.tmp), tb, ix->fi, keys, (const int32_t *)ix->pt_obs, ix->cam_obs,
+                                              (size_t)O, 0u, (unsigned)bits_for(ix->F), st));
+        MM_LAUNCH(ctx, "idx_ptr_kernel", idx_ptr_kernel, dim3(gO), dim3(256), 0, (const int32_t *)keys, O, ix->F, ix->cam_ptr,
+                  (int32_t *)nullptr, (const int64_t *)ix->head);
+        MM_LAUNCH(ctx, "idx_count_kernel", idx_count_kernel, dim3(gO), dim3(256), 0, ix->fi, ix->pi, (const int32_t *)ix->pt_ptr, O,
+                  cnt, span, (const int64_t *)ix->head);
+        tb = w0.tmp_bytes;
+        MM_HIP(ctx, rocprim::exclusive_scan((void *)(b0 + w0.tmp), tb, (const int32_t *)cnt, offs, (int64_t)0, (size_t)O,
+                                            rocprim::plus<int64_t>(), st));
+        MM_LAUNCH(ctx, "idx_head0_kernel", idx_head0_kernel, dim3(1), dim3(1), 0, (const int32_t *)cnt, (const int64_t *)offs, O,
+                  (const int32_t *)span, ix->head);
+        return MM_OK;
+    }
+    if (stage != 1) return mm_fail(ctx, MM_ERR_ARG, "mm_ba_index_build: stage must be 0 or 1");
+    if (!band_ok(ix) || !ix->pair_o || !ix->pair_o2 || !ix->pair_p || !ix->seg_ids || !ix->seg_chunk_ptr || !ix->chunk_seg ||
+        !ix->chunk_begin || !ix->chunk_end || !ws1 || ((uintptr_t)ws1 & 15))
+        return mm_fail(ctx, MM_ERR_ARG, "mm_ba_index_build: bad stage 1 argument");
+    int64_t seg_cap, chunk_cap;
+    mm_ba_index_bounds(ix->F, ix->cam_span, ix->n_pairs, ix->chunk, &seg_cap, &chunk_cap);
+    const int key_bits = bits_for((int64_t)ix->F * (ix->cam_span + 1));
+    Ws1 w1;
+    MM_HIP(ctx, ws1_layout(ix->n_pairs, seg_cap, key_bits, st, w1));
+    if (ws1_bytes < w1.total) return mm_fail(ctx, MM_ERR_WORKSPACE, "mm_ba_index_build: stage 1 workspace too small");
+    uint8_t *b1 = (uint8_t *)ws1;
+    int32_t *key = (int32_t *)(b1 + w1.key), *key_s = (int32_t *)(b1 + w1.key_s), *counts = (int32_t *)(b1 + w1.counts);
+    int32_t *n_seg = (int32_t *)(b1 + w1.n_seg), *pairs_of = (int32_t *)(b1 + w1.pairs_of), *chunks_of = (int32_t *)(b1 + w1.chunks_of);
+    int32_t *seg_lo = (int32_t *)(b1 + w1.seg_lo);
+    uint64_t *val = (uint64_t *)(b1 + w1.val), *val_s = (uint64_t *)(b1 + w1.val_s);
+    const int64_t n = ix->n_pairs;
+    const unsigned gN = (unsigned)((n + 255) / 256);
+    MM_HIP(ctx, hipMemsetAsync(key, 0, (size_t)n * 4, st));
+    MM_HIP(ctx, hipMemsetAsync(val, 0, (size_t)n * 8, st));
+    MM_LAUNCH(ctx, "idx_emit_kernel", idx_emit_kernel, dim3(gO), dim3(256), 0, ix->fi, ix->pi, (const int32_t *)ix->pt_ptr, O,
+              (const int64_t *)offs, ix->cam_span, n, key, val, (const int64_t *)ix->head);
+    size_t tb = w1.tmp_bytes;
+    MM_HIP(ctx, rocprim::radix_sort_pairs((void *)(b1 + w1.tmp), tb, (const int32_t *)key, key_s, (const uint64_t *)val, val_s, (size_t)n,
+                                          0u, (unsigned)key_bits, st));
+    MM_LAUNCH(ctx, "idx_unpack_kernel", idx_unpack_kernel, dim3(gN), dim3(256), 0, (const uint64_t *)val_s, ix->pi, n, O, ix->pair_o,
+              ix->pair_o2, ix->pair_p);
+    tb = w1.tmp_bytes;
+    MM_HIP(ctx, rocprim::run_length_encode((void *)(b1 + w1.tmp), tb, (const int32_t *)key_s, (size_t)n, ix->seg_ids, counts, n_seg, st));
+    MM_LAUNCH(ctx, "idx_segcount_kernel", idx_segcount_kernel, dim3((unsigned)((seg_cap + 1 + 255) / 256)), dim3(256), 0,
+              (const int32_t *)counts, (const int32_t *)n_seg, seg_cap, ix->chunk, pairs_of, chunks_of);
+    tb = w1.tmp_bytes;
+    MM_HIP(ctx, rocprim::exclusive_scan((void *)(b1 + w1.tmp), tb, (const int32_t *)pairs_of, seg_lo, (int32_t)0, (size_t)seg_cap + 1,
+                                        rocprim::plus<int32_t>(), st));
+    tb = w1.tmp_bytes;
+    MM_HIP(ctx, rocprim::exclusive_scan((void *)(b1 + w1.tmp), tb, (const int32_t *)chunks_of, ix->seg_chunk_ptr, (int32_t)0,
+                                        (size_t)seg_cap + 1, rocprim::plus<int32_t>(), st));
+    MM_LAUNCH(ctx, "idx_chunks_kernel", idx_chunks_kernel, dim3((unsigned)((seg_cap * 64 + 255) / 256)), dim3(256), 0,
+              (const int32_t *)n_seg, (const int32_t *)seg_lo, (const int32_t *)pairs_of, (const int32_t *)ix->seg_chunk_ptr, ix->chunk,
+              chunk_cap, ix->chunk_seg, ix->chunk_begin, ix->chunk_end, ix->head);
+    return MM_OK;
+}
+
+}
diff --git a/meatmodeler_amd/csrc/bf_match.hip b/meatmodeler_amd/csrc/bf_match.hip
--- a/meatmodeler_amd/csrc/bf_match.hip
+++ b/meatmodeler_amd/csrc/bf_match.hip
@@ -294,6 +294,43 @@
     if (threadIdx.x == 0) m_out[pair] = base_s;
 }
 
+template <bool CODES>
+__global__ __launch_bounds__(256) void match_compact_kernel(const int32_t *__restrict__ idx,
+                                                            const int32_t *__restrict__ dist,
+                                                            const int32_t *__restrict__ nq_dev, int nq_cap,
+                                                            double threshold, int32_t *__restrict__ pairs,
+                                                            int32_t *__restrict__ m_out) {
+    __shared__ int wave_cnt[2][4];
+    const int pair = blockIdx.x;
+    const int nq = nq_dev ? max(min(nq_dev[pair], nq_cap), 0) : nq_cap;
+    const int lane = threadIdx.x & 63, wave = threadIdx.x >> 6;
+    int2 *__restrict__ out = reinterpret_cast<int2 *>(pairs) + (size_t)pair * nq_cap;
+    int base = 0, par = 0;
+    for (int q0 = 0; q0 < nq; q0 += 256, par ^= 1) {
+        const int qi = q0 + threadIdx.x;
+        int ti = -1;
+        if (qi < nq) {
+            if constexpr (CODES) {
+                ti = idx[(size_t)pair * nq_cap + qi];
+            } else {
+                const size_t o = ((size_t)pair * nq_cap + qi) * 2;
+                const int d0 = dist[o], d1 = dist[o + 1];
+                if ((d0 >= 0) && (d1 >= 0) && ((double)d0 < threshold * (double)d1)) ti = idx[o];
+            }
+        }
+        const bool keep = ti >= 0;
+        const unsigned long long m = __ballot(keep);
+        if (lane == 0) wave_cnt[par][wave] = __builtin_popcountll(m);
+        __syncthreads();
+        const int c0 = wave_cnt[par][0], c1 = wave_cnt[par][1], c2 = wave_cnt[par][2], c3 = wave_cnt[par][3];
+        const int off = base + (wave > 0 ? c0 : 0) + (wave > 1 ? c1 : 0) + (wave > 2 ? c2 : 0);
+        if (keep) out[off + __builtin_popcountll(m & ((1ull << lane) - 1ull))] = make_int2(qi, ti);
+        base += c0 + c1 + c2 + c3;
+    }
+    for (int j = base + (int)threadIdx.x; j < nq_cap; j += 256) out[j] = make_int2(-1, -1);
+    if (threadIdx.x == 0) m_out[pair] = base;
+}
+
 typedef int bf_v4i __attribute__((ext_vector_type(4)));
 typedef int bf_v16i __attribute__((ext_vector_type(16)));
 constexpr int MF_TT = 32;
@@ -510,6 +547,13 @@
     return r;
 }
 
+__device__ __forceinline__ bf_v4i bf_fp4x32_planes(uint32_t bits) {
+    bf_v4i r;
+#pragma unroll
+    for (int k = 0; k < 4; ++k) r[k] = (int)(((bits << (3 - k)) & 0x88888888u) | 0x22222222u);
+    return r;
+}
+
 __global__ __launch_bounds__(256) void bf_expand_fp4_kernel(const uint8_t *__restrict__ t, int nt_cap, size_t t_stride, int ntp,
                                                             int n_pairs, uint8_t *__restrict__ out) {
     const size_t g = (size_t)blockIdx.x * 256 + threadIdx.x;
@@ -757,11 +801,11 @@
 #ifdef MM_BF_CLOCK
 __device__ long long g_bf_clock[2 * 4096];
 #endif
-template <int WAVES, bool PIPE>
+template <int WAVES, bool PIPE, bool RATIO>
 __global__ __launch_bounds__(BF_THREADS, WAVES) void bf_knn2_fp4min_kernel(
     const uint8_t *__restrict__ q, const int32_t *__restrict__ nq_dev, int nq_cap, size_t q_stride,
-    const uint8_t *__restrict__ tx, const uint8_t *__restrict__ tpk, size_t t_stride, const int32_t *__restrict__ nt_dev,
-    int nt_cap, int ntp, int32_t *__restrict__ idx, int32_t *__restrict__ dist, int qtiles, int n_pairs) {
+    const uint8_t *__restrict__ tpk, size_t t_stride, const int32_t *__restrict__ nt_dev,
+    int nt_cap, int32_t *__restrict__ idx, int32_t *__restrict__ dist, int qtiles, int n_pairs, double threshold) {
     __shared__ __attribute__((aligned(16))) uint8_t tile[3][MF_TT][F4_PITCH];
     const int xcd = blockIdx.x & 7, slot = blockIdx.x >> 3;
     const int grp = slot / qtiles;
@@ -791,7 +835,7 @@
         const uint32_t w[8] = {lo.x, lo.y, lo.z, lo.w, hi.x, hi.y, hi.z, hi.w};
 #pragma unroll
         for (int j = 0; j < 4; ++j) {
-            const bf_v4i e = bf_fp4x32(~(h ? w[2 * j + 1] : w[2 * j]));
+            const bf_v4i e = bf_fp4x32_planes(~(h ? w[2 * j + 1] : w[2 * j]));
             B4[u][j] = e;
         }
     }
@@ -800,13 +844,14 @@
     for (int i = 0; i < 16; ++i) cinit[i] = 12582912.0f + 262144.0f + (float)(8 * (i >> 2) + 4 * h + (i & 3));
     uint32_t b0[2] = {BF_NONE, BF_NONE}, b1[2] = {BF_NONE, BF_NONE};
     const int ntiles = (nt + MF_TT - 1) / MF_TT;
-    const uint8_t *txp = tx + (size_t)pair * ntp * 128;
+    const uint8_t *tp = tpk + (size_t)pair * t_stride;
     const int e0 = threadIdx.x;
-    bf_v4i ra, rb, rc;
+    uint32_t ra, rb, rc;
     auto fetch = [&](int tt, auto set) __attribute__((always_inline)) {
         constexpr int S = decltype(set)::value;
         if (tt < ntiles) {
-            const bf_v4i v = reinterpret_cast<const bf_v4i *>(txp + (size_t)tt * MF_TT * 128)[e0];
+            const uint32_t v = tt * MF_TT + (e0 >> 3) < nt_cap
+                                   ? reinterpret_cast<const uint32_t *>(tp + (size_t)tt * MF_TT * 32)[e0] : 0u;
             if constexpr (S == 0) ra = v;
             if constexpr (S == 1) rb = v;
             if constexpr (S == 2) rc = v;
@@ -815,9 +860,9 @@
     auto commit = [&](int buf, auto set) __attribute__((always_inline)) {
         constexpr int S = decltype(set)::value;
         bf_v4i *d = reinterpret_cast<bf_v4i *>(&tile[buf][e0 >> 3][(e0 & 7) * 16]);
-        if constexpr (S == 0) *d = ra;
-        if constexpr (S == 1) *d = rb;
-        if constexpr (S == 2) *d = rc;
+        if constexpr (S == 0) *d = bf_fp4x32_planes(ra);
+        if constexpr (S == 1) *d = bf_fp4x32_planes(rb);
+        if constexpr (S == 2) *d = bf_fp4x32_planes(rc);
     };
     bf_v16f acc1_prev;
     bf_v4i A4[4];
@@ -926,7 +971,6 @@
         book(acc0, (uint32_t)nfull * MF_TT, 0, std::true_type{}, dead_from);
         book(acc1, (uint32_t)nfull * MF_TT, 1, std::true_type{}, dead_from);
     }
-    const uint8_t *tp = tpk + (size_t)pair * t_stride;
 #pragma unroll
     for (int u = 0; u < 2; ++u) {
         const int qi = qbase + 64 * wv + 32 * u + c;
@@ -963,11 +1007,17 @@
         top2_insert(o0, b0[u], b1[u]);
         top2_insert(o1, b0[u], b1[u]);
         if (h == 0 && qi < nq) {
-            const size_t o = ((size_t)pair * nq_cap + qi) * 2;
-            idx[o] = b0[u] == BF_NONE ? -1 : (int32_t)(b0[u] & 0xFFFFu);
-            idx[o + 1] = b1[u] == BF_NONE ? -1 : (int32_t)(b1[u] & 0xFFFFu);
-            dist[o] = b0[u] == BF_NONE ? -1 : (int32_t)(b0[u] >> 22);
-            dist[o + 1] = b1[u] == BF_NONE ? -1 : (int32_t)(b1[u] >> 22);
+            if constexpr (RATIO) {
+                const bool keep = b0[u] != BF_NONE && b1[u] != BF_NONE &&
+                                  (double)(int32_t)(b0[u] >> 22) < threshold * (double)(int32_t)(b1[u] >> 22);
+                idx[(size_t)pair * nq_cap + qi] = keep ? (int32_t)(b0[u] & 0xFFFFu) : -1;
+            } else {
+                const size_t o = ((size_t)pair * nq_cap + qi) * 2;
+                idx[o] = b0[u] == BF_NONE ? -1 : (int32_t)(b0[u] & 0xFFFFu);
+                idx[o + 1] = b1[u] == BF_NONE ? -1 : (int32_t)(b1[u] & 0xFFFFu);
+                dist[o] = b0[u] == BF_NONE ? -1 : (int32_t)(b0[u] >> 22);
+                dist[o + 1] = b1[u] == BF_NONE ? -1 : (int32_t)(b1[u] >> 22);
+            }
         }
     }
 #ifdef MM_BF_CLOCK
@@ -992,6 +1042,11 @@
     const int v = bf_variant(n_pairs, nq_cap);
     return (v == 200 || v == 300 || v == 310 || v == 314) && nt_cap >= 64 && nt_cap < 65536;
 }
+bool bf_fp4min(int n_pairs, int nq_cap) {
+    const int v = bf_variant(n_pairs, nq_cap);
+    return v == 310 || v == 314;
+}
+bool bf_fused(int n_pairs, int nq_cap, int nt_cap) { return bf_use_mfma(n_pairs, nq_cap, nt_cap) && bf_fp4min(n_pairs, nq_cap); }
 int bf_ntp(int nt_cap) { return (nt_cap + MF_TT - 1) / MF_TT * MF_TT; }
 
 int bf_choose_splits(int n_pairs, int nq_cap, int nt_cap) {
@@ -1020,19 +1075,24 @@
 extern "C" {
 
 size_t mm_bf_workspace_bytes(int n_pairs, int nq_cap, int nt_cap) {
-    if (n_pairs > 0 && nq_cap > 0 && bf_use_mfma(n_pairs, nq_cap, nt_cap))
+    if (n_pairs > 0 && nq_cap > 0 && bf_use_mfma(n_pairs, nq_cap, nt_cap)) {
+        if (bf_fp4min(n_pairs, nq_cap)) return 256;
         return mm_align_up((size_t)n_pairs * bf_ntp(nt_cap) * (bf_variant(n_pairs, nq_cap) >= 300 ? 128 : 256), 256);
+    }
     int s = bf_choose_splits(n_pairs, nq_cap, nt_cap);
     if (s == 1) return 256;
     return mm_align_up((size_t)n_pairs * s * nq_cap * 2 * sizeof(uint32_t), 256);
 }
 
-int mm_bf_knn2_batched(mm_ctx *ctx, const uint8_t *q, const int32_t *nq, int nq_cap, size_t q_set_stride,
-                       const uint8_t *t, const int32_t *nt, int nt_cap, size_t t_set_stride, int n_pairs,
-                       int32_t *idx, int32_t *dist, void *ws, size_t ws_bytes) {
-    if (!ctx) return MM_ERR_ARG;
+}
+
+namespace {
+
+int bf_knn2_run(mm_ctx *ctx, const uint8_t *q, const int32_t *nq, int nq_cap, size_t q_set_stride, const uint8_t *t,
+                const int32_t *nt, int nt_cap, size_t t_set_stride, int n_pairs, int32_t *idx, int32_t *dist, void *ws,
+                size_t ws_bytes, const double *ratio) {
     if (n_pairs == 0 || nq_cap == 0) return MM_OK;
-    if (!q || (!t && nt_cap > 0) || !idx || !dist || n_pairs < 0 || nq_cap < 0 || nt_cap < 0)
+    if (!q || (!t && nt_cap > 0) || !idx || (!dist && !ratio) || n_pairs < 0 || nq_cap < 0 || nt_cap < 0)
         return mm_fail(ctx, MM_ERR_ARG, "mm_bf_knn2_batched: bad argument");
     if (nt_cap >= (1 << BF_IDX_BITS)) return mm_fail(ctx, MM_ERR_ARG, "mm_bf_knn2_batched: nt_cap must be < 2^20");
     if (((uintptr_t)q | (uintptr_t)t | q_set_stride | t_set_stride) & 15)
@@ -1046,22 +1106,25 @@
             return mm_fail(ctx, MM_ERR_WORKSPACE, "mm_bf_knn2_batched: workspace too small or misaligned");
         const int ntp = bf_ntp(nt_cap);
         const dim3 grid((nq_cap + BF_THREADS - 1) / BF_THREADS, 1, n_pairs);
+        if (bf_fp4min(n_pairs, nq_cap)) {
+            const int qtiles = (int)grid.x;
+            const dim3 grid_x(8u * (unsigned)((n_pairs + 7) / 8) * grid.x);
+            const double thr = ratio ? *ratio : 0.0;
+#define BF_GO_MIN(W, P, R)                                                                                                \
+    MM_LAUNCH(ctx, "bf_knn2_fp4min_kernel", (bf_knn2_fp4min_kernel<W, P, R>), grid_x, dim3(BF_THREADS), 0, q, nq, nq_cap, \
+              q_set_stride, t, t_set_stride, nt, nt_cap, idx, dist, qtiles, n_pairs, thr)
+            if (bf_variant(n_pairs, nq_cap) == 310) {
+                if (ratio) BF_GO_MIN(3, true, true); else BF_GO_MIN(3, true, false);
+            } else {
+                if (ratio) BF_GO_MIN(4, false, true); else BF_GO_MIN(4, false, false);
+            }
+#undef BF_GO_MIN
+            return MM_OK;
+        }
         if (bf_variant(n_pairs, nq_cap) >= 300) {
             const size_t chunks = (size_t)n_pairs * ntp * 8;
             MM_LAUNCH(ctx, "bf_expand_kernel", bf_expand_fp4_kernel, dim3((unsigned)((chunks + 255) / 256)), dim3(256), 0, t, nt_cap,
                       t_set_stride, ntp, n_pairs, (uint8_t *)ws);
-            const int qtiles = (int)grid.x;
-            const dim3 grid_x(8u * (unsigned)((n_pairs + 7) / 8) * grid.x);
-            if (bf_variant(n_pairs, nq_cap) == 310) {
-                MM_LAUNCH(ctx, "bf_knn2_fp4min_kernel", (bf_knn2_fp4min_kernel<3, true>), grid_x, dim3(BF_THREADS), 0, q, nq, nq_cap, q_set_stride,
-                          (const uint8_t *)ws, t, t_set_stride, nt, nt_cap, ntp, idx, dist, qtiles, n_pairs);
-                return MM_OK;
-            }
-            if (bf_variant(n_pairs, nq_cap) == 314) {
-                MM_LAUNCH(ctx, "bf_knn2_fp4min_kernel", (bf_knn2_fp4min_kernel<4, false>), grid_x, dim3(BF_THREADS), 0, q, nq, nq_cap, q_set_stride,
-                          (const uint8_t *)ws, t, t_set_stride, nt, nt_cap, ntp, idx, dist, qtiles, n_pairs);
-                return MM_OK;
-            }
             MM_LAUNCH(ctx, "bf_knn2_fp4_kernel", bf_knn2_fp4_kernel, grid, dim3(BF_THREADS), 0, q, nq, nq_cap, q_set_stride,
                       (const uint8_t *)ws, nt, nt_cap, ntp, idx, dist);
             return MM_OK;
@@ -1114,6 +1177,60 @@
     return MM_OK;
 }
 
+struct BfMatchWs {
+    size_t knn, idx, dist, total;
+};
+BfMatchWs bf_match_ws(int n_pairs, int nq_cap, int nt_cap) {
+    BfMatchWs w;
+    w.knn = mm_align_up(mm_bf_workspace_bytes(n_pairs, nq_cap, nt_cap), 256);
+    const size_t rows = (size_t)max(n_pairs, 0) * (size_t)max(nq_cap, 0);
+    const bool fused = n_pairs > 0 && nq_cap > 0 && bf_fused(n_pairs, nq_cap, nt_cap);
+    const size_t one = mm_align_up(rows * (fused ? 1 : 2) * sizeof(int32_t), 256);
+    w.idx = w.knn;
+    w.dist = fused ? w.idx : w.idx + one;
+    w.total = w.dist + one;
+    return w;
+}
+
+}
+
+extern "C" {
+
+int mm_bf_knn2_batched(mm_ctx *ctx, const uint8_t *q, const int32_t *nq, int nq_cap, size_t q_set_stride,
+                       const uint8_t *t, const int32_t *nt, int nt_cap, size_t t_set_stride, int n_pairs,
+                       int32_t *idx, int32_t *dist, void *ws, size_t ws_bytes) {
+    if (!ctx) return MM_ERR_ARG;
+    return bf_knn2_run(ctx, q, nq, nq_cap, q_set_stride, t, nt, nt_cap, t_set_stride, n_pairs, idx, dist, ws, ws_bytes, nullptr);
+}
+
+size_t mm_bf_match_ratio_workspace_bytes(int n_pairs, int nq_cap, int nt_cap) {
+    return bf_match_ws(n_pairs, nq_cap, nt_cap).total;
+}
+
+int mm_bf_match_ratio_batched(mm_ctx *ctx, const uint8_t *q, const int32_t *nq, int nq_cap, size_t q_set_stride,
+                              const uint8_t *t, const int32_t *nt, int nt_cap, size_t t_set_stride, int n_pairs,
+                              double threshold, int32_t *pairs, int32_t *m_out, void *ws, size_t ws_bytes) {
+    if (!ctx) return MM_ERR_ARG;
+    if (n_pairs == 0) return MM_OK;
+    if (n_pairs < 0 || nq_cap < 0 || nt_cap < 0 || !m_out || (!pairs && nq_cap > 0))
+        return mm_fail(ctx, MM_ERR_ARG, "mm_bf_match_ratio_batched: bad argument");
+    const BfMatchWs w = bf_match_ws(n_pairs, nq_cap, nt_cap);
+    if (!ws || ws_bytes < w.total || ((uintptr_t)ws & 15))
+        return mm_fail(ctx, MM_ERR_WORKSPACE, "mm_bf_match_ratio_batched: workspace too small or misaligned");
+    int32_t *idx = (int32_t *)((uint8_t *)ws + w.idx), *dist = (int32_t *)((uint8_t *)ws + w.dist);
+    const bool fused = nq_cap > 0 && bf_fused(n_pairs, nq_cap, nt_cap);
+    const int rc = bf_knn2_run(ctx, q, nq, nq_cap, q_set_stride, t, nt, nt_cap, t_set_stride, n_pairs, idx, dist, ws, w.knn,
+                               fused ? &threshold : nullptr);
+    if (rc != MM_OK) return rc;
+    if (fused)
+        MM_LAUNCH(ctx, "match_compact_kernel", match_compact_kernel<true>, dim3(n_pairs), dim3(256), 0, idx, (const int32_t *)nullptr, nq, nq_cap,
+                  threshold, pairs, m_out);
+    else
+        MM_LAUNCH(ctx, "match_compact_kernel", match_compact_kernel<false>, dim3(n_pairs), dim3(256), 0, idx, dist, nq, nq_cap,
+                  threshold, pairs, m_out);
+    return MM_OK;
+}
+
 int mm_bf_knn2_hamming(mm_ctx *ctx, const uint8_t *q, int nq, const uint8_t *t, int nt, int32_t *idx, int32_t *dist,
                        void *ws, size_t ws_bytes) {
     return mm_bf_knn2_batched(ctx, q, nullptr, nq, 0, t, nullptr, nt, 0, 1, idx, dist, ws, ws_bytes);
diff --git a/meatmodeler_amd/ops.py b/meatmodeler_amd/ops.py
--- a/meatmodeler_amd/ops.py
+++ b/meatmodeler_amd/ops.py
@@ -58,6 +58,26 @@
         return pairs, m
     ctx.check(lib.mm_ratio_filter_batched(ctx.h, ptr(_i32(idx)), ptr(_i32(dist)), ptr(nq), nq_cap, n_pairs,
                                           float(threshold), ptr(pairs), ptr(m)), "mm_ratio_filter_batched")
+    return pairs, m
+
+
+def bf_match_ratio_batched(q, t, nq=None, nt=None, threshold=0.75, ctx=None):
+    ctx = ctx or default_context()
+    assert q.dtype == torch.uint8 and t.dtype == torch.uint8 and q.shape[-1] == 32 and t.shape[-1] == 32
+    assert q.stride(-1) == 1 and q.stride(-2) == 32 and t.stride(-1) == 1 and t.stride(-2) == 32
+    n_pairs, nq_cap, nt_cap = q.shape[0], q.shape[1], t.shape[1]
+    assert t.shape[0] == n_pairs
+    pairs = torch.empty((n_pairs, nq_cap, 2), dtype=torch.int32, device=q.device)
+    m = torch.empty(n_pairs, dtype=torch.int32, device=q.device)
+    if n_pairs == 0:
+        return pairs, m
+    wsb = lib.mm_bf_match_ratio_workspace_bytes(n_pairs, nq_cap, nt_cap)
+    ws = torch.empty(wsb, dtype=torch.uint8, device=q.device)
+    qs = q.stride(0) if n_pairs > 1 else 0
+    ts = t.stride(0) if n_pairs > 1 else 0
+    ctx.check(lib.mm_bf_match_ratio_batched(ctx.h, ptr(q), ptr(nq), nq_cap, qs, ptr(t), ptr(nt), nt_cap, ts, n_pairs,
+                                            float(threshold), ptr(pairs), ptr(m), ptr(ws), wsb),
+              "mm_bf_match_ratio_batched")
     return pairs, m
 
 
@@ -274,7 +294,8 @@
 
 class BADevice:
 
-    def __init__(self, K, fi, pi, obs, F, P, device, ctx=None, pairs=True, max_band_span=192, fixed_cams=None):
+    def __init__(self, K, fi, pi, obs, F, P, device, ctx=None, pairs=True, max_band_span=192, fixed_cams=None,
+                 native_index=True):
         self.ctx = ctx or default_context()
         self._mdot = None
         dev = device
@@ -300,6 +321,101 @@
                 self.fixed_cams = fixed_cams.contiguous()
                 self.fx = _lib.BAFixed(self.F_fixed, 0, ptr(self.fixed_cams))
         F_all = F + self.F_fixed
+        self.cam_span = 0
+        self.max_band_span = int(max_band_span)
+        self._slabs, self._slab_src = None, None
+        self.n_pairs = 0
+        self.overlap = os.environ.get("MM_SCHUR_OVERLAP", "0") != "0"
+        self.index_build = "torch"
+        if native_index and O and F > 0 and P > 0 and not self.F_fixed and self._build_index_native(pairs):
+            self.index_build = "native"
+        else:
+            self._build_index_torch(pairs, F_all)
+        self._ws = torch.empty(2048 * 8, dtype=torch.uint8, device=dev)
+        self._cost2 = torch.zeros(1, dtype=torch.float64, device=dev)
+        self._S = None
+        self._schur_ws = None
+        self._chol_ws = None
+
+    @staticmethod
+    def _chunk_pairs():
+        return max(64, int(os.environ.get("MM_SCHUR_CHUNK", "512")) // 64 * 64)
+
+    @property
+    def slabs(self):
+        if self._slabs is None and self._slab_src is not None:
+            seg_ids, seg_chunk_ptr = self._slab_src
+            self._slab_src = None
+            self._set_slabs(seg_ids.to(torch.int64), seg_chunk_ptr.to(torch.int64))
+        return self._slabs
+
+    def _set_slabs(self, seg_ids, seg_chunk_ptr):
+        n_slabs = 8
+        cps = -(-self.F // n_slabs)
+        if cps >= 16:
+            seg_cam = seg_ids // (self.cam_span + 1)
+            bounds = torch.arange(n_slabs + 1, dtype=torch.int64, device=self.device) * cps
+            sseg = torch.searchsorted(seg_cam, bounds)
+            schunk = seg_chunk_ptr[sseg]
+            self._slabs = (n_slabs, cps, np.ascontiguousarray(sseg.cpu().numpy(), np.int64),
+                           np.ascontiguousarray(schunk.cpu().numpy(), np.int64))
+
+    def _build_index_native(self, pairs):
+        F, P, O, dev = self.F, self.P, self.O, self.device
+        i32 = dict(dtype=torch.int32, device=dev)
+        pt_ptr, pt_obs = torch.empty(P + 1, **i32), torch.empty(O, **i32)
+        cam_ptr, cam_obs = torch.empty(F + 1, **i32), torch.empty(O, **i32)
+        head = torch.empty(8, dtype=torch.int64, device=dev)
+        ix = _lib.BAIndex(F, P, O, ptr(self.fi), ptr(self.pi), ptr(pt_ptr), ptr(pt_obs), ptr(cam_ptr), ptr(cam_obs), ptr(head),
+                          0, self._chunk_pairs(), 0, None, None, None, None, None, None, None, None)
+        ws0b = lib.mm_ba_index_workspace_bytes(self.ctx.h, C.byref(ix), 0)
+        if not ws0b:
+            raise _lib.MMError("mm_ba_index_workspace_bytes: no workspace size for stage 0")
+        ws0 = torch.empty(ws0b, dtype=torch.uint8, device=dev)
+        self.ctx.check(lib.mm_ba_index_build(self.ctx.h, C.byref(ix), 0, ptr(ws0), ws0b, None, 0), "mm_ba_index_build")
+        span, n, bad_range, not_point_major = head[:4].tolist()
+        if bad_range:
+            raise ValueError("frame / point index out of range")
+        if not_point_major:
+            return False
+        self.pt_ptr, self.pt_obs, self.cam_ptr, self.cam_obs = pt_ptr, pt_obs, cam_ptr, cam_obs
+        self.cam_span = int(span)
+        self.pb = BAProblem(F, P, O, ptr(self.K), ptr(self.fi), ptr(self.pi), ptr(self.obs),
+                            ptr(self.pt_ptr), ptr(self.pt_obs), ptr(self.cam_ptr), ptr(self.cam_obs),
+                            self.cam_span, 0, 0, None, None, 0, None, None, None, None, None, None)
+        if pairs and self.cam_span <= self.max_band_span and self.cam_span < F and F * (self.cam_span + 1) < 2 ** 31:
+            n = int(n)
+            seg_cap, chunk_cap = C.c_int64(0), C.c_int64(0)
+            lib.mm_ba_index_bounds(F, self.cam_span, n, ix.chunk, C.byref(seg_cap), C.byref(chunk_cap))
+            seg_cap, chunk_cap = seg_cap.value, chunk_cap.value
+            pair_o, pair_o2, pair_p = torch.empty(n, **i32), torch.empty(n, **i32), torch.empty(n, **i32)
+            seg_ids, seg_chunk_ptr = torch.empty(seg_cap, **i32), torch.empty(seg_cap + 1, **i32)
+            chunk_seg, chunk_begin, chunk_end = (torch.empty(chunk_cap, **i32) for _ in range(3))
+            ix.cam_span, ix.n_pairs = self.cam_span, n
+            ix.pair_o, ix.pair_o2, ix.pair_p = ptr(pair_o), ptr(pair_o2), ptr(pair_p)
+            ix.seg_ids, ix.seg_chunk_ptr = ptr(seg_ids), ptr(seg_chunk_ptr)
+            ix.chunk_seg, ix.chunk_begin, ix.chunk_end = ptr(chunk_seg), ptr(chunk_begin), ptr(chunk_end)
+            ws1b = lib.mm_ba_index_workspace_bytes(self.ctx.h, C.byref(ix), 1)
+            if not ws1b:
+                raise _lib.MMError("mm_ba_index_workspace_bytes: no workspace size for stage 1")
+            ws1 = torch.empty(ws1b, dtype=torch.uint8, device=dev)
+            self.ctx.check(lib.mm_ba_index_build(self.ctx.h, C.byref(ix), 1, ptr(ws0), ws0b, ptr(ws1), ws1b), "mm_ba_index_build")
+            n_seg, n_chunks = head[4:6].tolist()
+            self.pair_o, self.pair_o2, self.pair_p = pair_o, pair_o2, pair_p
+            self.seg_ids, self.seg_chunk_ptr = seg_ids[:n_seg], seg_chunk_ptr[:n_seg + 1]
+            self.chunk_seg, self.chunk_begin, self.chunk_end = chunk_seg[:n_chunks], chunk_begin[:n_chunks], chunk_end[:n_chunks]
+            self.n_pairs = n
+            self.pb.n_seg = n_seg
+            self.pb.n_chunks = n_chunks
+            self.pb.seg_ids, self.pb.seg_chunk_ptr = ptr(self.seg_ids), ptr(self.seg_chunk_ptr)
+            self.pb.chunk_seg, self.pb.chunk_begin, self.pb.chunk_end = ptr(self.chunk_seg), ptr(self.chunk_begin), ptr(self.chunk_end)
+            self.pb.pair_o, self.pb.pair_o2, self.pb.pair_p = ptr(self.pair_o), ptr(self.pair_o2), ptr(self.pair_p)
+            self._slab_src = (self.seg_ids, self.seg_chunk_ptr)
+        return True
+
+    def _build_index_torch(self, pairs, F_all):
+        F, P, O, dev = self.F, self.P, self.O, self.device
+        max_band_span = self.max_band_span
         i64 = dict(dtype=torch.int64, device=dev)
         if O:
             lim = torch.stack([self.fi.min(), self.fi.max(), self.pi.min(), self.pi.max(),
@@ -326,14 +442,9 @@
             self.cam_obs = torch.sort(self.fi, stable=True)[1].to(torch.int32)
         else:
             self.cam_obs = torch.zeros(0, dtype=torch.int32, device=dev)
-        self.cam_span = 0
-        self.max_band_span = int(max_band_span)
-        self.slabs = None
-        self.overlap = os.environ.get("MM_SCHUR_OVERLAP", "0") != "0"
         self.pb = BAProblem(F, P, O, ptr(self.K), ptr(self.fi), ptr(self.pi), ptr(self.obs),
                             ptr(self.pt_ptr), ptr(self.pt_obs), ptr(self.cam_ptr), ptr(self.cam_obs),
                             0, 0, 0, None, None, 0, None, None, None, None, None, None)
-        self.n_pairs = 0
         pair_pb, free_idx, O_pairs = self.pb, None, O
         if O and self.F_fixed:
             free_idx = torch.nonzero(self.fi < F).reshape(-1)
@@ -371,7 +482,7 @@
                 seg_ids, counts = torch.unique_consecutive(key_s, return_counts=True)
                 seg_hi = torch.cumsum(counts, 0)
                 seg_lo = seg_hi - counts
-                CH = max(64, int(os.environ.get("MM_SCHUR_CHUNK", "512")) // 64 * 64)
+                CH = self._chunk_pairs()
                 cntc = (counts + (CH - 1)) // CH
                 first_hi = torch.cumsum(cntc, 0)
                 first = first_hi - cntc
@@ -391,20 +502,7 @@
                 self.pb.pair_o, self.pb.pair_o2 = ptr(self.pair_o), ptr(self.pair_o2)
                 self.pair_p = self.pi[self.pair_o.long()].contiguous()
                 self.pb.pair_p = ptr(self.pair_p)
-                n_slabs = 8
-                cps = -(-F // n_slabs)
-                if cps >= 16:
-                    seg_cam = seg_ids.to(torch.int64) // (self.cam_span + 1)
-                    bounds = torch.arange(n_slabs + 1, **i64) * cps
-                    sseg = torch.searchsorted(seg_cam, bounds)
-                    schunk = torch.cat([first, first_hi[-1:]])[sseg]
-                    self.slabs = (n_slabs, cps, np.ascontiguousarray(sseg.cpu().numpy(), np.int64),
-                                  np.ascontiguousarray(schunk.cpu().numpy(), np.int64))
-        self._ws = torch.empty(2048 * 8, dtype=torch.uint8, device=dev)
-        self._cost2 = torch.zeros(1, dtype=torch.float64, device=dev)
-        self._S = None
-        self._schur_ws = None
-        self._chol_ws = None
+                self._set_slabs(seg_ids.to(torch.int64), torch.cat([first, first_hi[-1:]]))
 
     def residual(self, cams, pts, want_res=False, cost_out=None):
         res = torch.empty((self.O, 2), dtype=torch.float64, device=self.device) if want_res else None
@@ -506,7 +604,7 @@
         if self._chol_ws is None:
             self._chol_ws = torch.empty(lib.mm_chol_workspace_bytes(n), dtype=torch.uint8, device=self.device)
         hb = int(min(half_bandwidth, n))
-        if self.slabs is not None and self.overlap:
+        if self.overlap and self.slabs is not None:
             ns, cps, sseg, schunk = self.slabs
             a_seg, a_chunk = sseg.ctypes.data_as(_lib.c_i64p), schunk.ctypes.data_as(_lib.c_i64p)
         else:
diff --git a/meatmodeler_amd/pipeline.py b/meatmodeler_amd/pipeline.py
--- a/meatmodeler_amd/pipeline.py
+++ b/meatmodeler_amd/pipeline.py
@@ -65,9 +65,8 @@
                     torch.zeros(0, dtype=torch.int32, device=self.device))
         q = desc[pair_lo:pair_hi]
         t = desc[pair_lo + 1:pair_hi + 1]
-        idx, dist = ops.bf_knn2_batched(q, t, n[pair_lo:pair_hi].contiguous(), n[pair_lo + 1:pair_hi + 1].contiguous(),
-                                        self.ctx)
-        return ops.ratio_filter_batched(idx, dist, self.ratio, n[pair_lo:pair_hi].contiguous(), self.ctx)
+        return ops.bf_match_ratio_batched(q, t, n[pair_lo:pair_hi].contiguous(), n[pair_lo + 1:pair_hi + 1].contiguous(),
+                                          self.ratio, self.ctx)
 
     def verify(self, det, pairs, m, pair_lo=0, **params):
         n = pairs.shape[0]
```

Measured after the change: 9259 billion descriptor pairs/s (match stage) (median of 6 runs). 8.2% higher.
